# yashkant/sam-textvqa

Hardware: AMD Instinct MI355X
Metric: training samples/sec, SA-M4C c=3 synthetic batch (higher is better)
Workload: dtype bf16; 1 GPU; SA-M4C c=3 full train step (fwd + masked BCE + bwd + clip 0.25 + Adam + LR), T=20 + 100 obj + 50 OCR + 12 dec = 182 tokens, 768-d, 12 heads, MMT n,n,s,s,s,s + TextBert 3 layers + input encoders + classifier(V=5000)/pointer net, dropout 0.1 on, bf16 MFMA compute, fp32 master weights/Adam; global_batch=64, per_gpu_batch=64, seq_len=182, parallelism=dp1

## Files before the change

### include/sam_hip.h

```cpp
#ifndef SAM_HIP_H
#define SAM_HIP_H
#include <stdint.h>
#ifdef __cplusplus
extern "C" {
#endif

#define SAM_ERR_ARG (-1)
#define SAM_ERR_UNSUPPORTED (-2)

int sam_abi_version(void);
const char* sam_build_digest(void);
const char* sam_last_error(void);
int sam_device_info(int* cu_count, int* lds_per_cu_bytes, char* arch, int arch_len);
int sam_set_cu_reserve(int n);
int sam_get_cu_reserve(void);
int sam_debug_cu_hog(int blocks, double microseconds, void* stream);

int sam_attn_words_per_row(int N);
int sam_pack_masks_u8(const int64_t* question_mask, int T, const int64_t* obj_mask, int No, const int64_t* ocr_mask, int Nc, int B, uint8_t* key_valid,
                      uint8_t* q8, uint8_t* ocr8, void* stream);
int sam_mask_bits_prefix_lm(const uint8_t* key_valid, int B, int n_enc, int n_dec, int NW, uint32_t* out, void* stream);
int sam_mask_bits_from_additive(const float* mask, int B, int N, int NW, uint32_t* out, void* stream);
int sam_mask_bits_spatial(const uint32_t* base, const int8_t* adj, int B, int N, int NW, int T, int n_oo, int R, int H,
                          unsigned quadrant_bits, uint32_t* out, void* stream);

int sam_mask_bits_from_int8_bhnn(const int8_t* rel, const uint32_t* base, int B, int H, int N, int NW, uint32_t* out, void* stream);

int sam_spatial_relation_tensor(const double* boxes, int B, int N, int context, double distance_threshold, int8_t* out, void* stream);

int sam_attn_fwd(const void* qkv, const uint32_t* allow, int64_t allow_stride_b, int64_t allow_stride_h, int B, int N, int H,
                 int head_dim, float scale, float p_drop, uint64_t seed, uint64_t offset, void* out, float* lse2,
                 uint32_t* keep, void* stream);
int sam_attn_fwd_rows(const void* qkv, const uint32_t* allow, int64_t allow_stride_b, int64_t allow_stride_h, int B, int N, int H,
                      int head_dim, float scale, int q_begin, void* out, float* lse2, void* stream);
int sam_attn_fwd_dec(const void* qkv_enc, const void* qkv_dec, const uint32_t* allow, int64_t allow_stride_b, int64_t allow_stride_h, int B, int N, int n_dec,
                     int H, int head_dim, float scale, void* out_dec, void* stream);
int sam_attn_fwd_dec_shared(const void* qkv_enc, const void* qkv_dec, const uint32_t* allow, int64_t allow_stride_b, int64_t allow_stride_h, int B, int group,
                            int N, int n_dec, int H, int head_dim, float scale, void* out_dec, void* stream);
int sam_attn_dec_row(const void* qkv_enc, const void* qkv_dec, const uint32_t* allow, int64_t allow_stride_b, int64_t allow_stride_h, int B, int group, int N,
                     int n_dec, int t, int H, int head_dim, float scale, void* out, int64_t ldo, void* stream);
int sam_attn_fwd_train(const void* qkv, const uint32_t* allow, int64_t allow_stride_b, int64_t allow_stride_h, int B, int N, int H,
                       int head_dim, float scale, float p_drop, uint64_t seed, uint64_t offset, void* out, void* out_lo, float* lse2,
                       uint32_t* keep, void* stream);
int sam_attn_bwd_fused(const void* dout, const void* qkv, const void* out, const void* out_lo, const float* lse2, const uint32_t* allow,
                       int64_t allow_stride_b, int64_t allow_stride_h, const uint32_t* keep, int B, int N, int H, int head_dim,
                       float scale, float p_drop, void* dqkv, void* stream);
int sam_attn_bwd_fused_max_n(void);
int sam_attn_bwd(const void* dout, const void* qkv, const float* lse2, const uint32_t* allow, int64_t allow_stride_b,
                 int64_t allow_stride_h, const uint32_t* keep, int B, int N, int H, int head_dim, float scale, float p_drop,
                 void* dqkv, float* delta_ws, void* stream);

enum { SAM_EPI_NONE = 0, SAM_EPI_BIAS = 1, SAM_EPI_BIAS_GELU = 2, SAM_EPI_BIAS_DROPOUT_RES = 3, SAM_EPI_DGELU = 4, SAM_EPI_BIAS_GELU_GRAD = 5, SAM_EPI_MUL_AUX = 6,
       SAM_EPI_BIAS_RELU = 7 };
typedef struct sam_ln_fuse {
  const float* gamma; const float* beta; float eps;
  void* y; int64_t ldy;
  float* mean; float* rstd;
  int32_t done;
  float* xws; int64_t xws_bytes;
} sam_ln_fuse;
int64_t sam_gemm_ln_ws_bytes(int M, int N);
typedef struct sam_gemm_desc {
  int32_t M, N, K;
  int32_t a_kcontig, b_kcontig;
  int32_t c_is_f32, accumulate, epilogue;
  const void* A; int64_t lda;
  const void* B; int64_t ldb;
  void* C; int64_t ldc;
  const float* bias;
  const void* residual; int64_t ldr;
  void* aux_out; const void* aux_in; int64_t ld_aux;
  float p_drop; uint64_t seed, offset;
  int32_t split_k;
  float* bias_grad;
  float* ws; int64_t ws_bytes;
  int32_t force_tile;
  int32_t defer_reduce;
  int32_t split_k_used;
  sam_ln_fuse* ln;
} sam_gemm_desc;
int sam_gemm_bf16(const sam_gemm_desc* d, void* stream);
int sam_gemm_bf16_grouped(const sam_gemm_desc* descs, int count, void* stream);
int64_t sam_gemm_grouped_ws_bytes(const sam_gemm_desc* descs, int count);
int sam_gemm_splitk_reduce(const float* ws, int split_k, int M, int N, float* C, int64_t ldc, float* bias_grad, void* stream);

int sam_layernorm_fwd(const void* x, int x_is_f32, int64_t ldx, const float* gamma, const float* beta, float eps, int M, int D, void* y,
                      int64_t ldy, float* mean, float* rstd, void* stream);
int64_t sam_layernorm_bwd_ws_bytes(int D);
int sam_layernorm_bwd(const void* dy, int64_t ldd, const void* x, int x_is_f32, int64_t ldx, const float* mean, const float* rstd,
                      const float* gamma, int M, int D, void* dx, void* dx_dropped, int64_t ldo, float p_drop, uint64_t seed, uint64_t offset,
                      float* dgamma, float* dbeta, float* dbias, int accumulate, float* ws, void* stream);
typedef struct sam_ln_finalize_item {
  const float* ws; int32_t rows; int32_t accumulate;
  float* dgamma; float* dbeta; float* dbias;
} sam_ln_finalize_item;
int sam_layernorm_bwd_partial_rows(int M);
int sam_layernorm_bwd_finalize_batch(const sam_ln_finalize_item* items, int count, int D, void* stream);
int64_t sam_colsum_ws_bytes(int N);
int sam_colsum_bf16(const void* x, int64_t ldx, int M, int N, float* out, int accumulate, float* ws, void* stream);
int sam_add_dropout_bf16(const void* a, int64_t lda, const void* b, int64_t ldb, void* out, int64_t ldo, int M, int D, float p_drop, uint64_t seed,
                         uint64_t offset, void* stream);

int sam_bce_loss(const float* fixed_scores, int64_t ld_fixed, const float* ocr_scores, int64_t ld_ocr, const float* targets, int64_t ld_t,
                 const float* loss_mask, int R, int V, int No, float grad_scale, const float* global_count, float* loss, void* d_fixed,
                 int64_t ld_dfixed, float* d_ocr, int64_t ld_docr, void* stream);

int sam_ptr_scores_fwd(const void* q, const void* k, const uint8_t* ocr_mask, int B, int S, int No, int D, float scale, float* out,
                       int64_t ld_out_b, int64_t ld_out_s, void* stream);
int sam_ptr_scores_bwd(const float* dscores, int64_t ld_b, int64_t ld_s, const void* q, const void* k, int B, int S, int No, int D, float scale,
                       void* dq, void* dk, void* stream);

int sam_embedding_bwd(const void* dy, int64_t ldd, const int64_t* idx, int T, int D, int rows, int64_t padding_idx, float* grad, int64_t ldg, uint8_t* touched,
                      void* stream);
int sam_embedding_bwd_sorted(const void* dy, int64_t ldd, const int64_t* idx_sorted, int T, int D, int rows, int64_t padding_idx, float* grad, int64_t ldg,
                             uint8_t* touched, void* stream);

int sam_l2norm_pack_bf16(const float* x, int64_t ldx, int M, int D, int normalize, float eps, void* out, int64_t ldo, int col0, int zero_upto,
                         void* stream);
int sam_embed_sum_fwd(const void* table, int64_t ld_table, const int64_t* ids, int table_rows, const float* pos, int64_t ld_pos, int S,
                      const float* tt, int64_t ld_tt, const uint8_t* type_ids, int n_types, int R, int D, float* out, int64_t ldo, void* stream);
int64_t sam_embed_sum_bwd_ws_bytes(int S, int n_types, int D);
int sam_embed_sum_bwd(const void* d, int64_t ldd, int R, int D, int S, const uint8_t* type_ids, int n_types, float* d_pos, int64_t ld_pos,
                      float* d_tt, int64_t ld_tt, float* ws, void* stream);
int sam_gather2_add_fwd(const void* ans, int64_t ld_ans, int V, const void* ocr, int64_t ld_ocr, int n_ocr, const int64_t* inds, int B, int S, int D,
                        const void* emb, int64_t ld_emb, float p_drop, uint64_t seed, uint64_t offset, void* out, int64_t ldo, void* stream);
int sam_gather2_add_bwd(const void* dy, int64_t ldd, int V, int n_ocr, const int64_t* inds, int B, int S, int D, float* d_ans, int64_t ld_dans,
                        float* d_ocr, int64_t ld_docr, float p_drop, uint64_t seed, uint64_t offset, void* d_emb, int64_t ld_demb, void* stream);

int sam_input_encoder_fwd(const void* za, int64_t ldza, const float* bbox, int64_t ldbox, const void* wb, int64_t ldw, const float* bias_b,
                          const float* gamma_a, const float* beta_a, const float* gamma_b, const float* beta_b, float eps, int R, int D, float p_drop,
                          uint64_t seed, uint64_t offset, void* out, int64_t ldo, float* stats, void* stream);
int64_t sam_input_encoder_bwd_ws_bytes(int R, int D);
int sam_input_encoder_bwd(const void* dy, int64_t ldd, const void* za, int64_t ldza, const float* bbox, int64_t ldbox, const void* wb, int64_t ldw,
                          const float* bias_b, const float* gamma_a, const float* gamma_b, const float* stats, int R, int D, float p_drop, uint64_t seed,
                          uint64_t offset, void* dza, int64_t ldo, float* dgamma_a, float* dbeta_a, float* dgamma_b, float* dbeta_b, float* dbias_b, float* dwb,
                          int64_t ldgw, int accumulate, float* ws, void* stream);

typedef struct sam_sparse_rows { int64_t lo, hi; int32_t row_len; const uint8_t* touched; } sam_sparse_rows;
int64_t sam_sumsq_ws_bytes(void);
int sam_sumsq_f32(const float* g, int64_t n, const sam_sparse_rows* sparse, float* out, float* ws, void* stream);
int sam_adam_step(float* p, float* g, float* m, float* v, void* p_bf16, int64_t n, const int64_t* seg_end, const float* seg_lr, int nseg,
                  float beta1, float beta2, float eps, int64_t step, const float* gnorm_sq, float max_norm, const sam_sparse_rows* sparse, void* stream);
int sam_adam_step_dev(float* p, float* g, float* m, float* v, void* p_bf16, int64_t n, const int64_t* seg_end, int nseg, float beta1, float beta2,
                      float eps, const float* dev_sched, const float* gnorm_sq, float max_norm, const sam_sparse_rows* sparse, void* stream);
int sam_adam_step_range(float* p, float* g, float* m, float* v, void* p_bf16, int64_t n, const int64_t* seg_end, int nseg, float beta1, float beta2,
                        float eps, const float* dev_sched, const float* gnorm_sq, float max_norm, const sam_sparse_rows* sparse, int64_t lo, int64_t hi,
                        int zero_grad, const int32_t* gate, int max_blocks, void* stream);
typedef struct sam_lr_schedule {
  double base_lr[8]; int32_t nseg;
  int64_t warmup_iters; double warmup_factor;
  int32_t n_decay; int64_t decay_iters[4]; double lr_decay;
  double beta1, beta2;
} sam_lr_schedule;
int sam_step_advance(unsigned long long* rng_state, uint64_t offset_stride, int64_t* step_counter, const sam_lr_schedule* sched, float* dev_sched,
                     void* stream);
int sam_cast_f32_to_bf16(const float* x, void* y, int64_t n, void* stream);

int sam_greedy_pick(const float* fixed_scores, int64_t ld_fixed, const float* ocr_scores, int64_t ld_ocr, int R, int S, int V, int No, int64_t* prev_inds,
                    void* stream);
int sam_beam_step(const float* fixed_scores, int64_t ld_fixed, const float* ocr_scores, int64_t ld_ocr, int B, int K, int S, int V, int No, int eos, int t,
                  int32_t* ctl, float* cum, uint8_t* done, int64_t* seqs, int64_t* prev_pos, void* stream);
int64_t sam_beam_step_ws_bytes(int B, int K);
// ... 68 lines not shown
```

### sam-textvqa_amd/_capi.py

```python
import ctypes as C
import os

_PKG = os.path.dirname(os.path.abspath(__file__))
LIB_PATH = os.path.join(_PKG, "lib", "libsam_hip.so")

_vp, _i, _i64, _u64, _f, _u = C.c_void_p, C.c_int, C.c_int64, C.c_uint64, C.c_float, C.c_uint

class LnFuse(C.Structure):
    _fields_ = [("gamma", _vp), ("beta", _vp), ("eps", _f), ("y", _vp), ("ldy", _i64), ("mean", _vp), ("rstd", _vp), ("done", C.c_int32),
                ("xws", _vp), ("xws_bytes", _i64)]


class GemmDesc(C.Structure):
    _fields_ = [("M", C.c_int32), ("N", C.c_int32), ("K", C.c_int32),
                ("a_kcontig", C.c_int32), ("b_kcontig", C.c_int32),
                ("c_is_f32", C.c_int32), ("accumulate", C.c_int32), ("epilogue", C.c_int32),
                ("A", _vp), ("lda", _i64), ("B", _vp), ("ldb", _i64), ("C", _vp), ("ldc", _i64),
                ("bias", _vp), ("residual", _vp), ("ldr", _i64),
                ("aux_out", _vp), ("aux_in", _vp), ("ld_aux", _i64),
                ("p_drop", _f), ("seed", _u64), ("offset", _u64), ("split_k", C.c_int32), ("bias_grad", _vp), ("ws", _vp), ("ws_bytes", _i64), ("force_tile", C.c_int32),
                ("defer_reduce", C.c_int32), ("split_k_used", C.c_int32), ("ln", C.POINTER(LnFuse))]


EPI_NONE, EPI_BIAS, EPI_BIAS_GELU, EPI_BIAS_DROPOUT_RES, EPI_DGELU, EPI_BIAS_GELU_GRAD, EPI_MUL_AUX, EPI_BIAS_RELU = range(8)
AUX_MUL, AUX_ADD = 0, 1

SIGNATURES = {
    "sam_attn_fwd": [_vp, _vp, _i64, _i64, _i, _i, _i, _i, _f, _f, _u64, _u64, _vp, _vp, _vp, _vp],
    "sam_attn_fwd_rows": [_vp, _vp, _i64, _i64, _i, _i, _i, _i, _f, _i, _vp, _vp, _vp],
    "sam_attn_bwd": [_vp, _vp, _vp, _vp, _i64, _i64, _vp, _i, _i, _i, _i, _f, _f, _vp, _vp, _vp],
    "sam_attn_words_per_row": [_i],
    "sam_attn_fwd_train": [_vp, _vp, _i64, _i64, _i, _i, _i, _i, _f, _f, _u64, _u64, _vp, _vp, _vp, _vp, _vp],
    "sam_attn_bwd_fused": [_vp, _vp, _vp, _vp, _vp, _vp, _i64, _i64, _vp, _i, _i, _i, _i, _f, _f, _vp, _vp],
    "sam_attn_bwd_fused_max_n": [],
    "sam_mask_bits_prefix_lm": [_vp, _i, _i, _i, _i, _vp, _vp],
    "sam_mask_bits_from_additive": [_vp, _i, _i, _i, _vp, _vp],
    "sam_mask_bits_spatial": [_vp, _vp, _i, _i, _i, _i, _i, _i, _i, _u, _vp, _vp],
    "sam_abi_version": [],
    "sam_mask_bits_from_int8_bhnn": [_vp, _vp, _i, _i, _i, _i, _vp, _vp],
    "sam_spatial_relation_tensor": [_vp, _i, _i, _i, C.c_double, _vp, _vp],
    "sam_gemm_bf16": [C.POINTER(GemmDesc), _vp],
    "sam_gemm_splitk_reduce": [_vp, _i, _i, _i, _vp, _i64, _vp, _vp],
    "sam_gemm_bf16_grouped": [C.POINTER(GemmDesc), _i, _vp],
    "sam_gemm_grouped_ws_bytes": [C.POINTER(GemmDesc), _i],
    "sam_layernorm_fwd": [_vp, _i, _i64, _vp, _vp, _f, _i, _i, _vp, _i64, _vp, _vp, _vp],
    "sam_layernorm_bwd": [_vp, _i64, _vp, _i, _i64, _vp, _vp, _vp, _i, _i, _vp, _vp, _i64, _f, _u64, _u64, _vp, _vp, _vp, _i, _vp, _vp],
    "sam_layernorm_bwd_ws_bytes": [_i],
    "sam_layernorm_bwd_partial_rows": [_i],
    "sam_layernorm_bwd_finalize_batch": [C.c_void_p, _i, _i, _vp],
    "sam_colsum_ws_bytes": [_i],
    "sam_colsum_bf16": [_vp, _i64, _i, _i, _vp, _i, _vp, _vp],
    "sam_bce_loss": [_vp, _i64, _vp, _i64, _vp, _i64, _vp, _i, _i, _i, _f, _vp, _vp, _vp, _i64, _vp, _i64, _vp],
    "sam_ptr_scores_fwd": [_vp, _vp, _vp, _i, _i, _i, _i, _f, _vp, _i64, _i64, _vp],
    "sam_ptr_scores_bwd": [_vp, _i64, _i64, _vp, _vp, _i, _i, _i, _i, _f, _vp, _vp, _vp],
    "sam_embedding_bwd": [_vp, _i64, _vp, _i, _i, _i, _i64, _vp, _i64, _vp, _vp],
    "sam_embedding_bwd_sorted": [_vp, _i64, _vp, _i, _i, _i, _i64, _vp, _i64, _vp, _vp],
    "sam_l2norm_pack_bf16": [_vp, _i64, _i, _i, _i, _f, _vp, _i64, _i, _i, _vp],
    "sam_embed_sum_fwd": [_vp, _i64, _vp, _i, _vp, _i64, _i, _vp, _i64, _vp, _i, _i, _i, _vp, _i64, _vp],
    "sam_embed_sum_bwd_ws_bytes": [_i, _i, _i],
    "sam_embed_sum_bwd": [_vp, _i64, _i, _i, _i, _vp, _i, _vp, _i64, _vp, _i64, _vp, _vp],
    "sam_gather2_add_fwd": [_vp, _i64, _i, _vp, _i64, _i, _vp, _i, _i, _i, _vp, _i64, _f, _u64, _u64, _vp, _i64, _vp],
    "sam_gather2_add_bwd": [_vp, _i64, _i, _i, _vp, _i, _i, _i, _vp, _i64, _vp, _i64, _f, _u64, _u64, _vp, _i64, _vp],
    "sam_sumsq_ws_bytes": [],
    "sam_sumsq_f32": [_vp, _i64, C.c_void_p, _vp, _vp, _vp],
    "sam_adam_step": [_vp, _vp, _vp, _vp, _vp, _i64, C.POINTER(_i64), C.POINTER(_f), _i, _f, _f, _f, _i64, _vp, _f, C.c_void_p, _vp],
    "sam_adam_step_dev": [_vp, _vp, _vp, _vp, _vp, _i64, C.POINTER(_i64), _i, _f, _f, _f, _vp, _vp, _f, C.c_void_p, _vp],
    "sam_adam_step_range": [_vp, _vp, _vp, _vp, _vp, _i64, C.POINTER(_i64), _i, _f, _f, _f, _vp, _vp, _f, C.c_void_p, _i64, _i64, _i, _vp, _i, _vp],
    "sam_cast_f32_to_bf16": [_vp, _vp, _i64, _vp],
    "sam_pack_masks_u8": [_vp, _i, _vp, _i, _vp, _i, _i, _vp, _vp, _vp, _vp],
    "sam_add_dropout_bf16": [_vp, _i64, _vp, _i64, _vp, _i64, _i, _i, _f, _u64, _u64, _vp],
    "sam_set_rng_state": [_vp],
    "sam_step_advance": [_vp, _u64, _vp, C.c_void_p, _vp, _vp],
    "sam_input_encoder_fwd": [_vp, _i64, _vp, _i64, _vp, _i64, _vp, _vp, _vp, _vp, _vp, _f, _i, _i, _f, _u64, _u64, _vp, _i64, _vp, _vp],
    "sam_input_encoder_bwd_ws_bytes": [_i, _i],
    "sam_input_encoder_bwd": [_vp, _i64, _vp, _i64, _vp, _i64, _vp, _i64, _vp, _vp, _vp, _vp, _i, _i, _f, _u64, _u64, _vp, _i64, _vp, _vp, _vp, _vp, _vp, _vp, _i64, _i, _vp, _vp],
    "sam_attn_fwd_dec": [_vp, _vp, _vp, _i64, _i64, _i, _i, _i, _i, _i, _f, _vp, _vp],
    "sam_attn_fwd_dec_shared": [_vp, _vp, _vp, _i64, _i64, _i, _i, _i, _i, _i, _i, _f, _vp, _vp],
    "sam_attn_dec_row": [_vp, _vp, _vp, _i64, _i64, _i, _i, _i, _i, _i, _i, _i, _f, _vp, _i64, _vp],
    "sam_greedy_pick": [_vp, _i64, _vp, _i64, _i, _i, _i, _i, _vp, _vp],
    "sam_beam_step": [_vp, _i64, _vp, _i64, _i, _i, _i, _i, _i, _i, _i, _vp, _vp, _vp, _vp, _vp, _vp],
    "sam_beam_step_split": [_vp, _i64, _vp, _i64, _i, _i, _i, _i, _i, _i, _i, _vp, _vp, _vp, _vp, _vp, _vp, _vp],
    "sam_beam_step_ws_bytes": [_i, _i],
    "sam_greedy_decode_ws_bytes": [_i, _i, _i],
    "sam_copy_blocks": [C.c_void_p, _i, _vp],
    "sam_ge_u8": [_vp, _i64, _i64, _vp, _vp],
    "sam_greedy_decode_steps": [C.c_void_p, _vp, _i64, _vp],
    "sam_gemm_ln_ws_bytes": [_i, _i],
    "sam_attn_probs": [_vp, _vp, _i64, _i64, _vp, _vp, _vp, _i, _i, _i, _i, _f, _f, _vp, _vp],
    "sam_rowvec_bf16": [_i, _vp, _i64, _vp, _i64, _vp, _vp, _i64, _i64, _i, _vp],
    "sam_set_cu_reserve": [_i],
    "sam_get_cu_reserve": [],
    "sam_debug_cu_hog": [_i, C.c_double, _vp],
    "sam_aux_pair_fwd": [_vp, _vp, _vp, _vp, _i, _i, _i, _vp, _vp],
    "sam_aux_pair_bwd_ws_bytes": [_i, _i],
    "sam_aux_pair_bwd": [_vp, _vp, _vp, _vp, _i, _i, _i, _vp, _vp, _vp, _vp, _i, _vp, _i64, _vp],
    "sam_l2norm_pack_from_bf16": [_vp, _i64, _i, _i, _i, _f, _vp, _i64, _i, _i, _vp],
    "sam_fc7_bwd_rows": [_vp, _i64, _vp, _i64, _i, _i, _i, _f, _vp, _i64, _vp],
    "sam_answer_sample": [_vp, _vp, _vp, _vp, _vp, _vp, _vp, _vp, _i, _i, _i, _i, _i, _i, _i, _u64, _vp, _i64, _vp, _vp, _i64, _vp, _vp, _vp, _vp, _vp],
    "sam_bce_loss_table": [_vp, _i64, _vp, _i64, _vp, _vp, _vp, _vp, _vp, _vp, _vp, _vp, _i, _i, _i, _i, _i, _vp, _vp, _i, _i, _i, _f, _vp, _vp, _vp, _i64, _vp, _i64,
                           _vp, _vp],
}
NO_STATUS = {"sam_set_rng_state", "sam_get_cu_reserve", "sam_gemm_ln_ws_bytes", "sam_layernorm_bwd_partial_rows", "sam_gemm_grouped_ws_bytes", "sam_attn_words_per_row", "sam_attn_bwd_fused_max_n", "sam_abi_version", "sam_layernorm_bwd_ws_bytes", "sam_colsum_ws_bytes", "sam_sumsq_ws_bytes", "sam_embed_sum_bwd_ws_bytes", "sam_input_encoder_bwd_ws_bytes", "sam_greedy_decode_ws_bytes", "sam_beam_step_ws_bytes", "sam_aux_pair_bwd_ws_bytes"}
RET_I64 = {"sam_gemm_grouped_ws_bytes", "sam_gemm_ln_ws_bytes", "sam_layernorm_bwd_ws_bytes", "sam_colsum_ws_bytes", "sam_sumsq_ws_bytes", "sam_embed_sum_bwd_ws_bytes", "sam_input_encoder_bwd_ws_bytes", "sam_greedy_decode_ws_bytes", "sam_beam_step_ws_bytes", "sam_aux_pair_bwd_ws_bytes"}

# ... 109 lines not shown
```

### sam-textvqa_amd/autograd.py

```python
import math
import os

import torch
from torch.autograd import Function

from . import _capi as capi
from . import ops, parallel, torchops
from .params import FlatParams, flat_of

BF16 = torch.bfloat16


class DropoutClock:

    def __init__(self):
        self.seed = 0x5A4D3443
        self.offset = 0

    def manual_seed(self, seed):
        self.seed, self.offset = int(seed) & 0xFFFFFFFFFFFFFFFF, 0

    def next(self):
        self.offset += 1
        return self.seed, self.offset
# ... 543 lines not shown
                pass
        cls.late = []


def defer_mmt_pairs_active():
    return os.environ.get("SAM_DEFER_MMT_WGRAD", "2") not in ("0", "1")


def wgrad_late_enabled():
    return os.environ.get("SAM_WGRAD_LATE", "1") != "0"


def wgrad_merge_enabled():
    return os.environ.get("SAM_WGRAD_MERGE_TB", "1") != "0"


def defer_wgrad_enabled():
    return os.environ.get("SAM_DEFER_TB_WGRAD", "1") != "0"


class EncoderLayerFn(Function):

    @staticmethod
    def forward(ctx, x, anchor, layer, allow, batch, p_attn, p_hid):
        att, so, inter, out = layer.attention.self, layer.attention.output, layer.intermediate, layer.output
        wqkv, bqkv, _, _ = _fused_qkv(att)
        heads = att.num_attention_heads
        scale = 1.0 / math.sqrt(att.attention_head_size)
        seeds = [dropout_clock.next() for _ in range(3)]
        ctx.layer, ctx.batch, ctx.p_attn, ctx.p_hid, ctx.seeds, ctx.scale = layer, batch, p_attn, p_hid, seeds, scale
        if coarse_ops_active() and x.dtype == BF16 and x.dim() == 2 and x.stride(1) == 1:
            outs = torchops.ns().encoder_layer_fwd(x, allow, _layer_params(layer), batch, heads, scale, p_attn, p_hid, [v for sd in seeds for v in sd],
                                                   so.LayerNorm.variance_epsilon, out.LayerNorm.variance_epsilon)
            ctx.save_for_backward(*outs[1:], allow)
            ctx.coarse = True
            return outs[0]
        ctx.coarse = False
        qkv = ops.gemm(x, wqkv, epilogue=capi.EPI_BIAS, bias=bqkv)
        fused_bwd = x.shape[0] // batch <= ops.attn_bwd_fused_max_n() and os.environ.get("SAM_ATTN_BWD_FUSED", "1") != "0"
        if fused_bwd:
            ctxv, lse2, keep, ctx_lo = ops.attn_fwd(qkv, allow, batch, heads, scale, p_attn, *seeds[0], want_residual=True)
        else:
            (ctxv, lse2, keep), ctx_lo = ops.attn_fwd(qkv, allow, batch, heads, scale, p_attn, *seeds[0]), None
        z1, a, mean1, rstd1 = ops.gemm_ln(ctxv, _w(so.dense.weight), so.LayerNorm.weight, so.LayerNorm.bias, so.LayerNorm.variance_epsilon,
                                          epilogue=capi.EPI_BIAS_DROPOUT_RES, bias=so.dense.bias, residual=x, p_drop=p_hid, seed=seeds[1][0], offset=seeds[1][1])
        pre = torch.empty((x.shape[0], inter.dense.weight.shape[0]), dtype=BF16, device=x.device)
        h = ops.gemm(a, _w(inter.dense.weight), epilogue=capi.EPI_BIAS_GELU_GRAD, bias=inter.dense.bias, aux_out=pre)
        z2, y, mean2, rstd2 = ops.gemm_ln(h, _w(out.dense.weight), out.LayerNorm.weight, out.LayerNorm.bias, out.LayerNorm.variance_epsilon,
                                          epilogue=capi.EPI_BIAS_DROPOUT_RES, bias=out.dense.bias, residual=a, p_drop=p_hid, seed=seeds[2][0], offset=seeds[2][1])
        ctx.save_for_backward(x, qkv, ctxv, lse2, keep, z1, mean1, rstd1, a, pre, h, z2, mean2, rstd2, allow, ctx_lo)
        return y

    @staticmethod
    def backward(ctx, dy):
        layer, p_hid, seeds = ctx.layer, ctx.p_hid, ctx.seeds
        att, so, inter, out = layer.attention.self, layer.attention.output, layer.intermediate, layer.output
        acc = not getattr(layer, "_sam_grad_fresh", False)
        layer._sam_grad_fresh = False
        defer = bool(getattr(layer, "_sam_defer_wgrad", False)) and defer_wgrad_enabled()
        if ctx.coarse:
            *saved, allow = ctx.saved_tensors
            if defer:
                dx, dy2, dpre, dy1, dqkv = torchops.ns().encoder_layer_bwd_nowgrad(dy, saved, allow, _layer_params(layer), _layer_grads(layer), ctx.batch,
                                                                                   att.num_attention_heads, ctx.scale, ctx.p_attn, p_hid,
                                                                                   [v for sd in seeds for v in sd], bool(ctx.needs_input_grad[0]), acc)
                _, _, dwqkv, dbqkv = _fused_qkv(att)
                x_, ctx_, a_, h_ = saved[0], saved[2], saved[8], saved[10]
                DeferredWgrads.add(layer, [(dy2, h_, out.dense.weight.grad, None), (dpre, a_, inter.dense.weight.grad, inter.dense.bias.grad),
                                           (dy1, ctx_, so.dense.weight.grad, None), (dqkv, x_, dwqkv, dbqkv)], acc)
            else:
                dx = torchops.ns().encoder_layer_bwd(dy, saved, allow, _layer_params(layer), _layer_grads(layer), ctx.batch, att.num_attention_heads, ctx.scale,
                                                     ctx.p_attn, p_hid, [v for sd in seeds for v in sd], bool(ctx.needs_input_grad[0]), acc)
                region_done(getattr(layer, "_sam_region_id", None))
            return (dx if ctx.needs_input_grad[0] else None), None, None, None, None, None, None
        x, qkv, ctxv, lse2, keep, z1, mean1, rstd1, a, pre, h, z2, mean2, rstd2, allow, ctx_lo = ctx.saved_tensors
        wqkv, _, dwqkv, dbqkv = _fused_qkv(att)
        if dy.dtype != BF16 or not dy.is_contiguous():
            dy = dy.to(BF16).contiguous()
        dz2, dy2 = ops.layernorm_bwd(dy, z2, mean2, rstd2, out.LayerNorm.weight, out.LayerNorm.weight.grad, out.LayerNorm.bias.grad,
                                     dbias=out.dense.bias.grad, want_dropped=True, p_drop=p_hid, seed=seeds[2][0], offset=seeds[2][1], accumulate=acc, may_defer=True)
        wgrads = [(dy2, h, out.dense.weight.grad, None)]
        dpre = ops.gemm(dy2, _w(out.dense.weight), b_kcontig=False, epilogue=capi.EPI_MUL_AUX, aux_in=pre)
        wgrads.append((dpre, a, inter.dense.weight.grad, inter.dense.bias.grad))
        da = ops.gemm(dpre, _w(inter.dense.weight), b_kcontig=False, epilogue=capi.EPI_BIAS_DROPOUT_RES, residual=dz2)
        dz1, dy1 = ops.layernorm_bwd(da, z1, mean1, rstd1, so.LayerNorm.weight, so.LayerNorm.weight.grad, so.LayerNorm.bias.grad,
                                     dbias=so.dense.bias.grad, want_dropped=True, p_drop=p_hid, seed=seeds[1][0], offset=seeds[1][1], accumulate=acc, may_defer=True)
        wgrads.append((dy1, ctxv, so.dense.weight.grad, None))
        dctx = ops.gemm(dy1, _w(so.dense.weight), b_kcontig=False)
        dqkv = ops.attn_bwd(dctx, qkv, lse2, allow, keep, ctx.batch, att.num_attention_heads, ctx.scale, ctx.p_attn, out=ctxv, out_lo=ctx_lo)
        wgrads.append((dqkv, x, dwqkv, dbqkv))
        if defer:
            DeferredWgrads.add(layer, wgrads, acc)
        else:
            ops.wgrad_grouped(wgrads, accumulate=acc)
        dx = ops.gemm(dqkv, wqkv, b_kcontig=False, epilogue=capi.EPI_BIAS_DROPOUT_RES, residual=dz1) if ctx.needs_input_grad[0] else None
        if not defer:
            region_done(getattr(layer, "_sam_region_id", None))
        return dx, None, None, None, None, None, None


def _rows_bf16(t):
    x2 = t.reshape(-1, t.shape[-1])
    if x2.dtype != BF16 or x2.stride(1) != 1 or x2.stride(0) % 8 or x2.data_ptr() % 16:
        x2 = x2.to(BF16).contiguous()
    return x2


class DenseDropoutResLnFn(Function):

    @staticmethod
    def forward(ctx, x, residual, mod, p_drop):
        dense, ln = mod.dense, mod.LayerNorm
        n, k = dense.weight.shape
        if n % 8 or k % 8:
            raise capi.SamHipError("%s: hidden sizes must be multiples of 8 (got %d -> %d)" % (type(mod).__name__, k, n))
        x2, r2 = _rows_bf16(x), _rows_bf16(residual)
        seed = dropout_clock.next()
        z, y, mean, rstd = ops.gemm_ln(x2, _w(dense.weight), ln.weight, ln.bias, ln.variance_epsilon, epilogue=capi.EPI_BIAS_DROPOUT_RES, bias=dense.bias,
                                       residual=r2, p_drop=p_drop, seed=seed[0], offset=seed[1])
        ctx.save_for_backward(x2, z, mean, rstd)
        ctx.mod, ctx.p_drop, ctx.seed, ctx.shapes = mod, p_drop, seed, (x.shape, x.dtype, residual.shape, residual.dtype)
        return y.view(*residual.shape[:-1], n)

    @staticmethod
    def backward(ctx, dy):
        x2, z, mean, rstd = ctx.saved_tensors
        dense, ln = ctx.mod.dense, ctx.mod.LayerNorm
        xs, xd, rs, rd = ctx.shapes
        dy2 = _rows_bf16(dy)
        dz, dyd = ops.layernorm_bwd(dy2, z, mean, rstd, ln.weight, ln.weight.grad, ln.bias.grad, dbias=dense.bias.grad, want_dropped=True, p_drop=ctx.p_drop,
                                    seed=ctx.seed[0], offset=ctx.seed[1], accumulate=True)
        ops.gemm(dyd, x2, a_kcontig=False, b_kcontig=False, out=dense.weight.grad, accumulate=True, split_k=-1)
        dx = ops.gemm(dyd, _w(dense.weight), b_kcontig=False).view(xs).to(xd) if ctx.needs_input_grad[0] else None
        return dx, (dz.view(rs).to(rd) if ctx.needs_input_grad[1] else None), None, None


class DenseGeluFn(Function):

    @staticmethod
    def forward(ctx, x, mod, want_grad):
        dense = mod.dense
        n, k = dense.weight.shape
        if n % 8 or k % 8:
            raise capi.SamHipError("BertIntermediate: sizes must be multiples of 8 (got %d -> %d)" % (k, n))
        x2 = _rows_bf16(x)
        dact = torch.empty((x2.shape[0], n), dtype=BF16, device=x2.device) if want_grad else None
        h = ops.gemm(x2, _w(dense.weight), epilogue=capi.EPI_BIAS_GELU_GRAD, bias=dense.bias, aux_out=dact)
        if want_grad:
            ctx.save_for_backward(x2, dact)
        ctx.mod, ctx.shape, ctx.dtype = mod, x.shape, x.dtype
        return h.view(*x.shape[:-1], n)

    @staticmethod
    def backward(ctx, dy):
        x2, dact = ctx.saved_tensors
        dense = ctx.mod.dense
        dpre = ops.rowvec("mul", _rows_bf16(dy), dact)
        ops.gemm(dpre, x2, a_kcontig=False, b_kcontig=False, out=dense.weight.grad, accumulate=True, split_k=-1, bias_grad=dense.bias.grad)
        dx = ops.gemm(dpre, _w(dense.weight), b_kcontig=False).view(ctx.shape).to(ctx.dtype) if ctx.needs_input_grad[0] else None
        return dx, None, None


def coarse_ops_active():
    return torchops.enabled() and capi.profiler is None


def _layer_params(layer):
    c = getattr(layer, "_sam_coarse_params", None)
    if c is None:
# ... 185 lines not shown
```

### sam-textvqa_amd/csrc/common.h

```cpp
#pragma once
#include <hip/hip_runtime.h>
#include <stdint.h>

typedef unsigned short bf16_t;
typedef __attribute__((ext_vector_type(8))) short bf16x8;
typedef __attribute__((ext_vector_type(4))) short s16x4;
typedef __attribute__((ext_vector_type(4))) float f32x4;
typedef __attribute__((ext_vector_type(2))) __bf16 hw_bf16x2;
typedef __attribute__((ext_vector_type(2))) float f32x2;

#define SAM_OK 0
#define SAM_ERR_ARG (-1)
#define SAM_ERR_UNSUPPORTED (-2)

extern "C" void sam_set_error(const char* fmt, ...);
extern "C" const unsigned long long* sam_get_rng_state(void);

#define SAM_REQUIRE(cond, ...)                    \
  do {                                            \
    if (!(cond)) {                                \
      sam_set_error(__VA_ARGS__);                 \
      return SAM_ERR_ARG;                         \
    }                                             \
  } while (0)

#define SAM_LAUNCH_CHECK()                                                       \
  do {                                                                           \
    hipError_t e_ = hipGetLastError();                                           \
    if (e_ != hipSuccess) {                                                      \
      sam_set_error("%s:%d launch failed: %s", __FILE__, __LINE__, hipGetErrorString(e_)); \
      return (int)e_;                                                            \
    }                                                                            \
  } while (0)

__device__ __forceinline__ float bf2f(bf16_t h) { return __uint_as_float(((unsigned)h) << 16); }
__device__ __forceinline__ unsigned pack_bf16x2(float lo, float hi) {
  f32x2 f = {lo, hi};
  return __builtin_bit_cast(unsigned, __builtin_convertvector(f, hw_bf16x2));
}
__device__ __forceinline__ bf16_t f2bf(float f) { return (bf16_t)(pack_bf16x2(f, 0.f) & 0xffffu); }
__device__ __forceinline__ float bf_lo(unsigned u) { return __uint_as_float(u << 16); }
__device__ __forceinline__ float bf_hi(unsigned u) { return __uint_as_float(u & 0xffff0000u); }

__device__ __forceinline__ s16x4 lds_read_tr16(const void* p) {
  return __builtin_amdgcn_ds_read_tr16_b64_v4i16((__attribute__((address_space(3))) s16x4*)p);
}
__device__ __forceinline__ bf16x8 cat4(s16x4 a, s16x4 b) {
  bf16x8 r;
  r[0] = a[0]; r[1] = a[1]; r[2] = a[2]; r[3] = a[3];
  r[4] = b[0]; r[5] = b[1]; r[6] = b[2]; r[7] = b[3];
  return r;
}

__device__ __forceinline__ float xgroup_max(float v) {
  auto a = __builtin_amdgcn_permlane16_swap(__float_as_uint(v), __float_as_uint(v), false, false);
  v = fmaxf(__uint_as_float(a[0]), __uint_as_float(a[1]));
  auto b = __builtin_amdgcn_permlane32_swap(__float_as_uint(v), __float_as_uint(v), false, false);
  return fmaxf(__uint_as_float(b[0]), __uint_as_float(b[1]));
}
__device__ __forceinline__ float xgroup_sum(float v) {
  auto a = __builtin_amdgcn_permlane16_swap(__float_as_uint(v), __float_as_uint(v), false, false);
  v = __uint_as_float(a[0]) + __uint_as_float(a[1]);
  auto b = __builtin_amdgcn_permlane32_swap(__float_as_uint(v), __float_as_uint(v), false, false);
  return __uint_as_float(b[0]) + __uint_as_float(b[1]);
}
__device__ __forceinline__ unsigned xgroup_or(unsigned v) {
  auto a = __builtin_amdgcn_permlane16_swap(v, v, false, false);
  v = a[0] | a[1];
  auto b = __builtin_amdgcn_permlane32_swap(v, v, false, false);
  return b[0] | b[1];
}
__device__ __forceinline__ float wave_sum_v(float v) {
  auto h = __builtin_amdgcn_permlane32_swap(__float_as_uint(v), __float_as_uint(v), false, false);
  v = __uint_as_float(h[0]) + __uint_as_float(h[1]);
  auto r = __builtin_amdgcn_permlane16_swap(__float_as_uint(v), __float_as_uint(v), false, false);
  v = __uint_as_float(r[0]) + __uint_as_float(r[1]);
  v += __int_as_float(__builtin_amdgcn_update_dpp(0, __float_as_int(v), 0x128, 0xf, 0xf, false));
  int t = __builtin_amdgcn_update_dpp(0, __float_as_int(v), 0x104, 0xf, 0x5, false);
  t = __builtin_amdgcn_update_dpp(t, __float_as_int(v), 0x114, 0xf, 0xa, false);
  v += __int_as_float(t);
  v += __int_as_float(__builtin_amdgcn_update_dpp(0, __float_as_int(v), 0x4E, 0xf, 0xf, false));
  v += __int_as_float(__builtin_amdgcn_update_dpp(0, __float_as_int(v), 0xB1, 0xf, 0xf, false));
  return v;
}

__device__ __forceinline__ void rng_resolve(const unsigned long long* st, unsigned& seed_lo, unsigned& seed_hi, unsigned& off_lo, unsigned& off_hi) {
  if (st) {
    const unsigned long long s = st[0], o = st[1] + (((unsigned long long)off_hi << 32) | off_lo);
    if (s) { seed_lo = (unsigned)s; seed_hi = (unsigned)(s >> 32); }
    off_lo = (unsigned)o; off_hi = (unsigned)(o >> 32);
  }
}

struct u32x4 { unsigned x, y, z, w; };
__device__ __forceinline__ unsigned mix32(unsigned x) {
  x ^= x >> 16; x *= 0x7feb352du; x ^= x >> 15; x *= 0x846ca68bu; x ^= x >> 16;
  return x;
}
__device__ __forceinline__ unsigned dropout_row_key(unsigned row, unsigned off_lo, unsigned off_hi, unsigned seed_lo, unsigned seed_hi) {
// ... 72 lines not shown
```

### sam-textvqa_amd/csrc/gemm.hip

```cpp
#include "gemm_common.h"
#include <stdlib.h>

using namespace samgemm;
namespace {

__device__ __forceinline__ int kc_off(int row, int chunk) { return row * 128 + ((chunk ^ ((row >> 1) & 7)) << 4); }
__device__ __forceinline__ int ks_swz(int krow) { return ((krow & 3) | (((krow >> 3) & 1) << 2)) << 1; }
template <int C>
__device__ __forceinline__ int ks_off(int krow, int chunk) { return krow * (2 * C) + ((chunk ^ (ks_swz(krow) & (C / 8 - 1))) << 4); }

template <bool KC, int R, int NT>
__device__ __forceinline__ void load_tile(uint4 (&r)[R * 8 / NT], const bf16_t* base, int64_t ld, int row0, int rows, int k0, int K, int tid) {
#pragma unroll
  for (int j = 0; j < R * 8 / NT; ++j) {
    const int c = tid + NT * j;
    r[j] = make_uint4(0, 0, 0, 0);
    if (KC) {
      const int row = row0 + (c >> 3), k = k0 + (c & 7) * 8;
      if (row < rows && k < K) r[j] = *reinterpret_cast<const uint4*>(base + (int64_t)row * ld + k);
    } else {
      const int k = k0 + c / (R / 8), col = row0 + (c % (R / 8)) * 8;
      if (k < K && col < rows) r[j] = *reinterpret_cast<const uint4*>(base + (int64_t)k * ld + col);
    }
  }
// ... 471 lines not shown
  g.count = count;
  int total = 0;
  static int bm_env = -1;
  if (bm_env < 0) { const char* e = getenv("SAM_WGRAD_TILE_M"); bm_env = e ? atoi(e) : 0; }
  const int bm = bm_env == 256 ? 256 : 128;
  for (int q = 0; q < count; ++q) {
    const sam_gemm_desc* d = descs + q;
    SAM_REQUIRE(!d->a_kcontig && !d->b_kcontig && d->c_is_f32 && d->epilogue == SAM_EPI_NONE && (d->split_k == 0 || d->split_k == 1),
                "sam_gemm_bf16_grouped: problem %d is not a plain fp32 wgrad-layout GEMM", q);
    SAM_REQUIRE(d->M > 0 && d->N > 0 && d->K > 0 && d->A && d->B && d->C, "sam_gemm_bf16_grouped: problem %d is empty", q);
    SAM_REQUIRE(d->M % 8 == 0 && d->N % 8 == 0 && d->lda % 8 == 0 && d->ldb % 8 == 0 && d->ldc % 4 == 0, "sam_gemm_bf16_grouped: problem %d: M, N, lda, ldb must be multiples of 8", q);
    SAM_REQUIRE(((uintptr_t)d->A % 16 == 0) && ((uintptr_t)d->B % 16 == 0) && ((uintptr_t)d->C % 16 == 0), "sam_gemm_bf16_grouped: problem %d: operands must be 16-byte aligned", q);
    if (q >= SAM_MAX_GROUP) continue;
    GemmArgs& a = g.a[q];
    a.M = d->M; a.N = d->N; a.K = d->K;
    a.A = (const bf16_t*)d->A; a.lda = d->lda; a.B = (const bf16_t*)d->B; a.ldb = d->ldb; a.C = d->C; a.ldc = d->ldc;
    a.accumulate = d->accumulate ? 1 : 0;
    a.inv_keep = 1.0f;
    a.tiles_m = (d->M + bm - 1) / bm; a.tiles_n = (d->N + 127) / 128;
    { static int gm = -1; if (gm < 0) { const char* e = getenv("SAM_GEMM_GROUP_M_WGRAD"); gm = e ? atoi(e) : 0; }
      a.group_m = gm > 0 ? gm : (gm == 0 && a.tiles_n > a.tiles_m ? a.tiles_m : 1); }
    a.split_k = 1;
    a.bias_grad = d->bias_grad;
    g.start[q] = total;
    total += (a.tiles_m * a.tiles_n + 7) / 8 * 8;
  }
  if (count <= SAM_MAX_GROUP) g.start[count] = total;
  {
    static int use8 = -1;
    if (use8 < 0) { const char* e = getenv("SAM_GEMM8W"); use8 = e ? atoi(e) : 1; }
    SAM_REQUIRE(ft == 0 || ft == 128 || ft == 1256 || ft == 12448, "sam_gemm_bf16_grouped: force_tile must be 0, 128, 1256 or 12448");
    static int use12 = -1;
    if (use12 < 0) { const char* e = getenv("SAM_GEMM12W"); use12 = e ? atoi(e) : 0; }
    if ((use12 && ft == 0) || ft == 12448) {
      const int rc = gemm12w_grouped(descs, count, (hipStream_t)stream);
      if (rc == SAM_OK) return SAM_OK;
      SAM_REQUIRE(rc == SAM_ERR_UNSUPPORTED && ft != 12448, "sam_gemm_bf16_grouped: the loader-wave grouped kernel cannot run this problem set (fewer deep tiles than CUs, K %% 64, workspace)");
    }
    if ((use8 && ft == 0) || ft == 1256) {
      const int rc = gemm8w_grouped(descs, count, (hipStream_t)stream);
      if (rc == SAM_OK) return SAM_OK;
      SAM_REQUIRE(rc == SAM_ERR_UNSUPPORTED && ft != 1256, "sam_gemm_bf16_grouped: the 8-wave grouped kernel cannot run this problem set (K %% 64, workspace, tile count)");
    }
  }
  if (count > SAM_MAX_GROUP) {
    for (int q0 = 0; q0 < count; q0 += SAM_MAX_GROUP) {
      const int rc = grouped_impl(descs + q0, count - q0 < SAM_MAX_GROUP ? count - q0 : SAM_MAX_GROUP, stream, ft);
      if (rc != SAM_OK) return rc;
    }
    return SAM_OK;
  }
  static bool once = false;
  if (!once) {
    hipFuncSetAttribute(reinterpret_cast<const void*>(gemm_group_kernel<128, 128, 2, 2, false, false, SAM_EPI_NONE, float>), hipFuncAttributeMaxDynamicSharedMemorySize, 2 * (128 + 128) * BK * 2);
    hipFuncSetAttribute(reinterpret_cast<const void*>(gemm_group_kernel<256, 128, 4, 2, false, false, SAM_EPI_NONE, float>), hipFuncAttributeMaxDynamicSharedMemorySize, 2 * (256 + 128) * BK * 2);
    once = true;
  }
  if (bm == 256)
    gemm_group_kernel<256, 128, 4, 2, false, false, SAM_EPI_NONE, float><<<dim3(total), dim3(512), (size_t)2 * (256 + 128) * BK * 2, (hipStream_t)stream>>>(g);
  else
    gemm_group_kernel<128, 128, 2, 2, false, false, SAM_EPI_NONE, float><<<dim3(total), dim3(256), (size_t)2 * (128 + 128) * BK * 2, (hipStream_t)stream>>>(g);
  SAM_LAUNCH_CHECK();
  return SAM_OK;
}

extern "C" int64_t sam_gemm_grouped_ws_bytes(const sam_gemm_desc* descs, int count) {
  if (!descs || count < 1 || count > SAM_MAX_GROUP8) return 0;
  int tiles = 0;
  for (int q = 0; q < count; ++q) tiles += ((descs[q].M + 255) / 256) * ((descs[q].N + 255) / 256);
  const int64_t a = gemm8w_ws_bytes(tiles), b = gemm12w_ws_bytes(descs, count);
  return a > b ? a : b;
}

extern "C" int64_t sam_gemm_ln_ws_bytes(int M, int N) { return (M > 0 && N > 0) ? gemm_ln_ws_bytes(M, N) : 0; }

extern "C" int sam_gemm_splitk_reduce(const float* ws, int split_k, int M, int N, float* C, int64_t ldc, float* bias_grad, void* stream) {
  SAM_REQUIRE(ws && C && split_k >= 1 && M > 0 && N > 0 && N % 4 == 0 && ldc % 4 == 0, "sam_gemm_splitk_reduce: bad arguments");
  const int64_t mn4 = (int64_t)M * N / 4;
  splitk_reduce_kernel<<<dim3((unsigned)min((int64_t)2048, (mn4 + 255) / 256)), dim3(256), 0, (hipStream_t)stream>>>(ws, split_k, M, N, C, ldc, bias_grad);
  SAM_LAUNCH_CHECK();
  return SAM_OK;
}

extern "C" int sam_gemm_bf16(const sam_gemm_desc* d, void* stream) {
  SAM_REQUIRE(d, "sam_gemm_bf16: null descriptor");
  if (d->ln) d->ln->done = 0;
  SAM_REQUIRE(d->M > 0 && d->N > 0 && d->K > 0, "sam_gemm_bf16: empty problem %dx%dx%d", d->M, d->N, d->K);
  SAM_REQUIRE(d->A && d->B && d->C, "sam_gemm_bf16: null operand");
  SAM_REQUIRE(d->N % 8 == 0 && d->lda % 8 == 0 && d->ldb % 8 == 0 && d->ldc % 4 == 0, "sam_gemm_bf16: N, lda, ldb must be multiples of 8 (N=%d lda=%lld ldb=%lld)", d->N, (long long)d->lda, (long long)d->ldb);
  SAM_REQUIRE(!d->a_kcontig || d->K % 8 == 0, "sam_gemm_bf16: K must be a multiple of 8 for k-contiguous A (K=%d)", d->K);
  SAM_REQUIRE(!d->b_kcontig || d->K % 8 == 0, "sam_gemm_bf16: K must be a multiple of 8 for k-contiguous B (K=%d)", d->K);
  SAM_REQUIRE(d->a_kcontig || d->M % 8 == 0, "sam_gemm_bf16: M must be a multiple of 8 for k-strided A (M=%d)", d->M);
  SAM_REQUIRE(((uintptr_t)d->A % 16 == 0) && ((uintptr_t)d->B % 16 == 0) && ((uintptr_t)d->C % 16 == 0), "sam_gemm_bf16: operands must be 16-byte aligned");
  SAM_REQUIRE(!d->accumulate || d->c_is_f32, "sam_gemm_bf16: accumulate needs an fp32 C");
  SAM_REQUIRE(d->p_drop >= 0.f && d->p_drop < 1.f, "sam_gemm_bf16: p_drop out of range");
  GemmArgs a = {};
  a.M = d->M; a.N = d->N; a.K = d->K;
  a.A = (const bf16_t*)d->A; a.lda = d->lda; a.B = (const bf16_t*)d->B; a.ldb = d->ldb; a.C = d->C; a.ldc = d->ldc;
  a.bias = d->bias; a.residual = (const bf16_t*)d->residual; a.ldr = d->ldr;
  a.aux_out = (bf16_t*)d->aux_out; a.aux_in = (const bf16_t*)d->aux_in; a.ld_aux = d->ld_aux;
  a.accumulate = d->accumulate;
  a.thr16 = dropout_thr16(d->p_drop);
  a.inv_keep = a.thr16 ? 1.0f / (1.0f - (float)a.thr16 / 65536.0f) : 1.0f;
  a.seed_lo = (unsigned)d->seed; a.seed_hi = (unsigned)(d->seed >> 32); a.off_lo = (unsigned)d->offset; a.off_hi = (unsigned)(d->offset >> 32);
  a.rng_state = sam_get_rng_state();
  a.split_k = 1;
  { static int gm = -1; if (gm < 0) { const char* e = getenv("SAM_GEMM_GROUP_M"); gm = e ? atoi(e) : 0; } a.group_m = gm > 0 ? gm : (d->split_k != 0 && d->split_k != 1 ? 1 : 8); }
  a.bias_grad = d->bias_grad;
  a.ws = d->ws;
  a.defer_reduce = d->defer_reduce;
  a.split_used = const_cast<int32_t*>(&d->split_k_used);
  SAM_REQUIRE(!d->bias_grad || (!d->a_kcontig && !d->b_kcontig), "sam_gemm_bf16: bias_grad is a wgrad-layout (0,0) feature");
  if (d->epilogue == SAM_EPI_BIAS_GELU) SAM_REQUIRE(d->aux_out && d->ld_aux % 4 == 0, "sam_gemm_bf16: BIAS_GELU needs aux_out");
  if (d->epilogue == SAM_EPI_BIAS_GELU_GRAD) SAM_REQUIRE(!d->aux_out || d->ld_aux % 4 == 0, "sam_gemm_bf16: BIAS_GELU_GRAD: ld_aux must be a multiple of 4");

  if (d->epilogue == SAM_EPI_DGELU || d->epilogue == SAM_EPI_MUL_AUX) SAM_REQUIRE(d->aux_in && d->ld_aux % 4 == 0, "sam_gemm_bf16: DGELU / MUL_AUX need aux_in");
  if (d->epilogue == SAM_EPI_BIAS_DROPOUT_RES) SAM_REQUIRE(!d->residual || d->ldr % 4 == 0, "sam_gemm_bf16: bad residual ld");
  int want_split = (d->split_k == 1) ? 0 : d->split_k;
  hipStream_t st = (hipStream_t)stream;
  if (want_split != 0 && !(d->c_is_f32 && d->epilogue == SAM_EPI_NONE && d->accumulate)) {
    SAM_REQUIRE(!d->accumulate && !d->bias_grad, "sam_gemm_bf16: split_k with an epilogue cannot accumulate / reduce a bias gradient");
    SAM_REQUIRE(d->ws && ((uintptr_t)d->ws % 16 == 0), "sam_gemm_bf16: split_k needs a 16-byte aligned workspace");
    int S = want_split < 0 ? pick_epilogue_split(d->M, d->N, d->K, d->ws_bytes) : want_split;
    if (S > (d->K + BK - 1) / BK) S = (d->K + BK - 1) / BK;
    S = no_empty_split((d->K + BK - 1) / BK, S);
    SAM_REQUIRE((int64_t)S * d->M * d->N * (int64_t)sizeof(float) <= d->ws_bytes || S <= 1, "sam_gemm_bf16: workspace too small for split_k=%d", S);
    if (S > 1) {
      GemmArgs g = a;
      g.bias = nullptr; g.residual = nullptr; g.aux_out = nullptr; g.aux_in = nullptr; g.thr16 = 0; g.accumulate = 0;
      g.tiles_m = (d->M + 63) / 64; g.tiles_n = (d->N + 63) / 64; g.split_k = S; g.group_m = 1; g.defer_reduce = 1; g.bias_grad = nullptr;
      const int lay2 = (d->a_kcontig ? 2 : 0) | (d->b_kcontig ? 1 : 0);
      int rc = lay2 == 3 ? launch_cfg<64, 64, 2, 2, true, true, SAM_EPI_NONE, float>(g, st)
             : lay2 == 2 ? launch_cfg<64, 64, 2, 2, true, false, SAM_EPI_NONE, float>(g, st)
             : lay2 == 0 ? launch_cfg<64, 64, 2, 2, false, false, SAM_EPI_NONE, float>(g, st) : SAM_ERR_UNSUPPORTED;
      if (rc) { if (rc == SAM_ERR_UNSUPPORTED) sam_set_error("sam_gemm_bf16: no split kernel for layout (0,1)"); return rc; }
      const int e2 = d->epilogue;
      if (d->ln && e2 == SAM_EPI_BIAS_DROPOUT_RES && !d->c_is_f32 && d->N % 4 == 0 && d->N <= 2048) {
        const sam_ln_fuse* l = d->ln;
        SAM_REQUIRE(l->gamma && l->beta && l->y && l->mean && l->rstd && l->ldy >= d->N, "sam_gemm_bf16: incomplete sam_ln_fuse");
        LnFuseArgs la = {l->gamma, l->beta, l->eps, (bf16_t*)l->y, l->ldy, l->mean, l->rstd};
        const dim3 lgrid((unsigned)((d->M + 3) / 4));
        switch ((d->N / 4 + 63) / 64) {
#define SAM_LN_CASE(NC) case NC: splitk_epilogue_ln_kernel<NC><<<lgrid, dim3(256), 0, st>>>(d->ws, S, a, la); break;
          SAM_LN_CASE(1) SAM_LN_CASE(2) SAM_LN_CASE(3) SAM_LN_CASE(4) SAM_LN_CASE(5) SAM_LN_CASE(6) SAM_LN_CASE(7) SAM_LN_CASE(8)
#undef SAM_LN_CASE
        }
        SAM_LAUNCH_CHECK();
        d->ln->done = 1;
        *const_cast<int32_t*>(&d->split_k_used) = S;
        return SAM_OK;
      }
      const int64_t mn4 = (int64_t)d->M * d->N / 4;
      const dim3 grid((unsigned)min((int64_t)2048, (mn4 + 255) / 256));
#define SAM_SPLIT_EPI(E, T) splitk_epilogue_kernel<E, T><<<grid, dim3(256), 0, st>>>(d->ws, S, a)
      if (d->c_is_f32) {
        if (e2 == SAM_EPI_NONE) SAM_SPLIT_EPI(SAM_EPI_NONE, float);
        else if (e2 == SAM_EPI_BIAS) SAM_SPLIT_EPI(SAM_EPI_BIAS, float);
        else { sam_set_error("sam_gemm_bf16: fp32 output supports epilogues NONE / BIAS only"); return SAM_ERR_UNSUPPORTED; }
      } else {
        if (e2 == SAM_EPI_NONE) SAM_SPLIT_EPI(SAM_EPI_NONE, bf16_t);
        else if (e2 == SAM_EPI_BIAS) SAM_SPLIT_EPI(SAM_EPI_BIAS, bf16_t);
        else if (e2 == SAM_EPI_BIAS_GELU) SAM_SPLIT_EPI(SAM_EPI_BIAS_GELU, bf16_t);
        else if (e2 == SAM_EPI_DGELU) SAM_SPLIT_EPI(SAM_EPI_DGELU, bf16_t);
        else if (e2 == SAM_EPI_BIAS_GELU_GRAD) SAM_SPLIT_EPI(SAM_EPI_BIAS_GELU_GRAD, bf16_t);
        else if (e2 == SAM_EPI_MUL_AUX) SAM_SPLIT_EPI(SAM_EPI_MUL_AUX, bf16_t);
        else if (e2 == SAM_EPI_BIAS_DROPOUT_RES) SAM_SPLIT_EPI(SAM_EPI_BIAS_DROPOUT_RES, bf16_t);
        else if (e2 == SAM_EPI_BIAS_RELU) SAM_SPLIT_EPI(SAM_EPI_BIAS_RELU, bf16_t);
        else { sam_set_error("sam_gemm_bf16: unknown epilogue %d", e2); return SAM_ERR_UNSUPPORTED; }
      }
#undef SAM_SPLIT_EPI
      SAM_LAUNCH_CHECK();
      *const_cast<int32_t*>(&d->split_k_used) = S;
      return SAM_OK;
    }
    want_split = 0;
    *const_cast<int32_t*>(&d->split_k_used) = 1;
  }
  if (want_split != 0) {
    SAM_REQUIRE(d->c_is_f32 && d->epilogue == SAM_EPI_NONE && d->accumulate, "sam_gemm_bf16: split_k needs an fp32 C with accumulate=1 and no epilogue");
    SAM_REQUIRE(d->ws && ((uintptr_t)d->ws % 16 == 0), "sam_gemm_bf16: split_k needs a 16-byte aligned workspace");
    const int64_t per_split = ((int64_t)d->M * d->N + d->M) * (int64_t)sizeof(float);
    SAM_REQUIRE(want_split < 0 || (int64_t)want_split * per_split <= d->ws_bytes || want_split > (d->K + BK - 1) / BK,
                "sam_gemm_bf16: workspace too small for split_k=%d (%lld bytes)", d->split_k, (long long)d->ws_bytes);
  }
  if (d->ln && d->ln->xws && want_split == 0 && d->epilogue == SAM_EPI_BIAS_DROPOUT_RES && !d->c_is_f32 && d->a_kcontig && d->N % 16 == 0 &&
      d->ln->xws_bytes >= gemm_ln_ws_bytes(d->M, d->N) && ((uintptr_t)d->ln->xws % 16) == 0) {
    const char* e = getenv("SAM_GEMM_LN_FUSE");
    const int lnx = e ? atoi(e) : 0;
    const sam_ln_fuse* l = d->ln;
    if (lnx) {
      SAM_REQUIRE(l->gamma && l->beta && l->y && l->mean && l->rstd && l->ldy >= d->N && l->ldy % 4 == 0, "sam_gemm_bf16: incomplete sam_ln_fuse");
      a.ln_gamma = l->gamma; a.ln_beta = l->beta; a.ln_eps = l->eps; a.ln_y = (bf16_t*)l->y; a.ln_ldy = l->ldy; a.ln_mean = l->mean; a.ln_rstd = l->rstd;
      a.ln_ws = l->xws; a.ln_done = const_cast<int32_t*>(&l->done);
    }
  }
  const int64_t wsb = d->ws_bytes;
  const int ft = d->force_tile;
  SAM_REQUIRE(ft == 0 || ft == 64 || ft == 128 || ft == 160 || ft == 192 || ft == 256 || ft == 1192 || ft == 1256 || ft == 1448 || ft == 3192 || ft == 1128 || ft == 12192 || ft == 12448, "sam_gemm_bf16: force_tile must be 0, 64, 128, 160, 192, 256, 1128, 1192, 1256, 1448, 3192, 12192 or 12448");
  const int lay = (d->a_kcontig ? 2 : 0) | (d->b_kcontig ? 1 : 0);
  const int e = d->epilogue;
  if (lay == 3) {
    if (d->c_is_f32) {
      if (e == SAM_EPI_NONE) return launch<true, true, SAM_EPI_NONE, float>(a, st, want_split, wsb, ft);
      if (e == SAM_EPI_BIAS) return launch<true, true, SAM_EPI_BIAS, float>(a, st, want_split, wsb, ft);
    } else {
      if (e == SAM_EPI_NONE) return launch<true, true, SAM_EPI_NONE, bf16_t>(a, st, want_split, wsb, ft);
      if (e == SAM_EPI_BIAS) return launch<true, true, SAM_EPI_BIAS, bf16_t>(a, st, want_split, wsb, ft);
      if (e == SAM_EPI_BIAS_GELU) return launch<true, true, SAM_EPI_BIAS_GELU, bf16_t>(a, st, want_split, wsb, ft);
      if (e == SAM_EPI_BIAS_GELU_GRAD) return launch<true, true, SAM_EPI_BIAS_GELU_GRAD, bf16_t>(a, st, want_split, wsb, ft);
      if (e == SAM_EPI_BIAS_DROPOUT_RES) return launch<true, true, SAM_EPI_BIAS_DROPOUT_RES, bf16_t>(a, st, want_split, wsb, ft);
      if (e == SAM_EPI_BIAS_RELU) return launch<true, true, SAM_EPI_BIAS_RELU, bf16_t>(a, st, want_split, wsb, ft);
    }
  } else if (lay == 2) {
    if (!d->c_is_f32) {
      if (e == SAM_EPI_NONE) return launch<true, false, SAM_EPI_NONE, bf16_t>(a, st, want_split, wsb, ft);
      if (e == SAM_EPI_DGELU) return launch<true, false, SAM_EPI_DGELU, bf16_t>(a, st, want_split, wsb, ft);
      if (e == SAM_EPI_MUL_AUX) return launch<true, false, SAM_EPI_MUL_AUX, bf16_t>(a, st, want_split, wsb, ft);
      if (e == SAM_EPI_BIAS_DROPOUT_RES) return launch<true, false, SAM_EPI_BIAS_DROPOUT_RES, bf16_t>(a, st, want_split, wsb, ft);
    } else if (e == SAM_EPI_NONE) return launch<true, false, SAM_EPI_NONE, float>(a, st, want_split, wsb, ft);
  } else if (lay == 0) {
    if (d->c_is_f32 && e == SAM_EPI_NONE) return launch<false, false, SAM_EPI_NONE, float>(a, st, want_split, wsb, ft);
    if (!d->c_is_f32 && e == SAM_EPI_NONE) return launch<false, false, SAM_EPI_NONE, bf16_t>(a, st, want_split, wsb, ft);
  }
  sam_set_error("sam_gemm_bf16: no kernel for layout (a_kcontig=%d,b_kcontig=%d) epilogue=%d c_is_f32=%d", d->a_kcontig, d->b_kcontig, e, d->c_is_f32);
  return SAM_ERR_UNSUPPORTED;
}
```

### sam-textvqa_amd/csrc/rowops.hip

```cpp
#include "common.h"
#include <stdlib.h>
#include "sam_hip.h"

namespace {

constexpr int LN_PARTIAL_BLOCKS = 512;


template <typename T> struct Ld4;
template <> struct Ld4<bf16_t> {
  static __device__ __forceinline__ void ld(const void* p, int64_t idx, float* v) {
    const uint2 x = *reinterpret_cast<const uint2*>(reinterpret_cast<const bf16_t*>(p) + idx);
    v[0] = bf_lo(x.x); v[1] = bf_hi(x.x); v[2] = bf_lo(x.y); v[3] = bf_hi(x.y);
  }
};
template <> struct Ld4<float> {
  static __device__ __forceinline__ void ld(const void* p, int64_t idx, float* v) {
    const float4 x = *reinterpret_cast<const float4*>(reinterpret_cast<const float*>(p) + idx);
    v[0] = x.x; v[1] = x.y; v[2] = x.z; v[3] = x.w;
  }
};
__device__ __forceinline__ void st4_bf16(void* p, int64_t idx, const float* v) {
  *reinterpret_cast<uint2*>(reinterpret_cast<bf16_t*>(p) + idx) = make_uint2(pack_bf16x2(v[0], v[1]), pack_bf16x2(v[2], v[3]));
}

constexpr int LN_FWD_ROWS = 1;
template <typename InT, int NCH>
__global__ __launch_bounds__(256) void ln_fwd_kernel(const void* x, int64_t ldx, const float* gamma, const float* beta, float eps, int M, int D,
                                                     void* y, int64_t ldy, float* mean_out, float* rstd_out) {
  const int lane = threadIdx.x & 63, row0 = (blockIdx.x * 4 + (threadIdx.x >> 6)) * LN_FWD_ROWS;
  if (row0 >= M) return;
  const int nchunk = D >> 2;
  float v[LN_FWD_ROWS][NCH][4];
#pragma unroll
  for (int i = 0; i < LN_FWD_ROWS; ++i) {
    const int row = min(row0 + i, M - 1);
#pragma unroll
    for (int j = 0; j < NCH; ++j) Ld4<InT>::ld(x, (int64_t)row * ldx + 4 * min(lane + 64 * j, nchunk - 1), v[i][j]);
  }
  float g4[NCH][4], b4[NCH][4];
#pragma unroll
  for (int j = 0; j < NCH; ++j) {
    const int c = min(lane + 64 * j, nchunk - 1);
    Ld4<float>::ld(gamma, 4 * c, g4[j]);
    Ld4<float>::ld(beta, 4 * c, b4[j]);
  }
#pragma unroll
  for (int i = 0; i < LN_FWD_ROWS; ++i) {
    const int row = row0 + i;
    float s = 0.f;
#pragma unroll
    for (int j = 0; j < NCH; ++j) {
      if (lane + 64 * j >= nchunk) v[i][j][0] = v[i][j][1] = v[i][j][2] = v[i][j][3] = 0.f;
      s += (v[i][j][0] + v[i][j][1]) + (v[i][j][2] + v[i][j][3]);
    }
    const float mean = wave_sum_v(s) / D;
    float q = 0.f;
#pragma unroll
    for (int j = 0; j < NCH; ++j)
      if (lane + 64 * j < nchunk)
#pragma unroll
        for (int e = 0; e < 4; ++e) { const float d = v[i][j][e] - mean; q += d * d; }
    const float rstd = 1.0f / sqrtf(wave_sum_v(q) / D + eps);
    if (row >= M) continue;
#pragma unroll
    for (int j = 0; j < NCH; ++j) {
      const int c = lane + 64 * j;
      if (c < nchunk) {
        float o[4];
#pragma unroll
        for (int e = 0; e < 4; ++e) o[e] = g4[j][e] * ((v[i][j][e] - mean) * rstd) + b4[j][e];
        st4_bf16(y, (int64_t)row * ldy + 4 * c, o);
      }
    }
    if (lane == 0) { mean_out[row] = mean; rstd_out[row] = rstd; }
  }
}

template <typename T> struct Raw4;
template <> struct Raw4<bf16_t> {
  typedef uint2 R;
  static __device__ __forceinline__ R ld(const void* p, int64_t idx) { return *reinterpret_cast<const uint2*>(reinterpret_cast<const bf16_t*>(p) + idx); }
  static __device__ __forceinline__ void expand(const R& x, float* v) { v[0] = bf_lo(x.x); v[1] = bf_hi(x.x); v[2] = bf_lo(x.y); v[3] = bf_hi(x.y); }
};
template <> struct Raw4<float> {
  typedef float4 R;
  static __device__ __forceinline__ R ld(const void* p, int64_t idx) { return *reinterpret_cast<const float4*>(reinterpret_cast<const float*>(p) + idx); }
  static __device__ __forceinline__ void expand(const R& x, float* v) { v[0] = x.x; v[1] = x.y; v[2] = x.z; v[3] = x.w; }
};

__device__ __forceinline__ void pin(unsigned& v) { asm volatile("" : "+v"(v)); }
__device__ __forceinline__ void pin(float& v) { asm volatile("" : "+v"(v)); }
__device__ __forceinline__ void pin(uint2& v) { pin(v.x); pin(v.y); }
__device__ __forceinline__ void pin(float4& v) { pin(v.x); pin(v.y); pin(v.z); pin(v.w); }

template <typename InT, int NCH, bool FULL, int MODE>
__global__ __launch_bounds__(256) void ln_bwd_kernel(const bf16_t* __restrict__ dy, int64_t ldd, const void* __restrict__ x, int64_t ldx, const float* __restrict__ mean,
                                                     const float* __restrict__ rstd, const float* __restrict__ gamma, int M, int D, bf16_t* __restrict__ dx,
                                                     bf16_t* __restrict__ dxd, int64_t ldo, unsigned thr16, float inv_keep, unsigned seed_lo, unsigned seed_hi,
                                                     unsigned off_lo, unsigned off_hi, const unsigned long long* rng_state, float* __restrict__ ws) {
  if (MODE == 2) rng_resolve(rng_state, seed_lo, seed_hi, off_lo, off_hi);
  constexpr int NS = NCH <= 3 ? 3 : (NCH == 4 ? 2 : 1);
  typedef typename Raw4<InT>::R XR;
  __shared__ float red[4][64 * 4];
  const int lane = threadIdx.x & 63, wave = __builtin_amdgcn_readfirstlane(threadIdx.x >> 6);
  const int nchunk = D >> 2;
  float ag[NCH][4], ab[NCH][4], ad[NCH][4];
#pragma unroll
  for (int j = 0; j < NCH; ++j)
#pragma unroll
    for (int e = 0; e < 4; ++e) ag[j][e] = ab[j][e] = ad[j][e] = 0.f;
  float gm[NCH][4];
#pragma unroll
  for (int j = 0; j < NCH; ++j) {
    const int c = lane + 64 * j;
    Ld4<float>::ld(gamma, 4 * min(c, nchunk - 1), gm[j]);
    if (!FULL && c >= nchunk) gm[j][0] = gm[j][1] = gm[j][2] = gm[j][3] = 0.f;
  }
  __builtin_amdgcn_sched_barrier(0);
  const DropHalfConsts hk = dropout_half_consts((lane & 1) != 0);
  const int rstride = gridDim.x * 4;
  XR xr[NS][NCH];
  uint2 dr[NS][NCH];
  float mu[NS], rs[NS];
#define LN_BWD_REQUEST(S, ROW)                                                                     \
  do {                                                                                             \
    const int row_ = min((ROW), M - 1);                                                            \
    mu[S] = mean[row_]; rs[S] = rstd[row_];                                                        \
    _Pragma("unroll") for (int j = 0; j < NCH; ++j) {                                              \
      const int c_ = FULL ? lane + 64 * j : min(lane + 64 * j, nchunk - 1);                        \
      xr[S][j] = Raw4<InT>::ld(x, (int64_t)row_ * ldx + 4 * c_);                                   \
      dr[S][j] = Raw4<bf16_t>::ld(dy, (int64_t)row_ * ldd + 4 * c_);                               \
    }                                                                                              \
  } while (0)
#define LN_BWD_SLOT(S, ROW, REQ)                                                                                                     \
  {                                                                                                                                \
    const int row = (ROW);                                                                                                         \
    float xh[NCH][4], g[NCH][4];                                                                                                   \
    float t1 = 0.f, t2 = 0.f;                                                                                                      \
    asm volatile("" ::: "memory");                                                                                                 \
    _Pragma("unroll") for (int j = 0; j < NCH; ++j) { pin(xr[S][j]); pin(dr[S][j]); }      \
    _Pragma("unroll") for (int j = 0; j < NCH; ++j) {                                                                              \
      const int c = lane + 64 * j;                                                                                                 \
      float xv[4], dv[4];                                                                                                          \
      Raw4<InT>::expand(xr[S][j], xv);                                                                                             \
      Raw4<bf16_t>::expand(dr[S][j], dv);                                                                                          \
      if (!FULL && c >= nchunk) { _Pragma("unroll") for (int e = 0; e < 4; ++e) xv[e] = dv[e] = 0.f; }                             \
      _Pragma("unroll") for (int e = 0; e < 4; ++e) {                                                                              \
        xh[j][e] = (FULL || c < nchunk) ? (xv[e] - mu[S]) * rs[S] : 0.f;                                                           \
        g[j][e] = dv[e] * gm[j][e];                                                                                                \
        t1 += g[j][e];                                                                                                             \
        t2 += g[j][e] * xh[j][e];                                                                                                  \
        ag[j][e] += dv[e] * xh[j][e];                                                                                              \
        ab[j][e] += dv[e];                                                                                                         \
      }                                                                                                                            \
    }                                                                                                                              \
    const float rsv = rs[S];                                                                                                       \
    pin(t1); pin(t2);                                                                                                              \
    if (REQ) {                                     \
      asm volatile("" ::: "memory");               \
      __builtin_amdgcn_sched_barrier(0);                                                                                           \
      LN_BWD_REQUEST(S, row + NS * rstride);                                                                                       \
      __builtin_amdgcn_sched_barrier(0);                                                                                           \
      asm volatile("" ::: "memory");                                                                                               \
    }                                                                                                                              \
    const float s1 = wave_sum_v(t1) / D, s2 = wave_sum_v(t2) / D;                                                                      \
    const unsigned rkey = MODE == 2 ? hidden_dropout_row_key((unsigned)row, off_lo, off_hi, seed_lo, seed_hi) : 0u;                \
    _Pragma("unroll") for (int j = 0; j < NCH; ++j) {                                                                              \
      const int c = lane + 64 * j;                                                                                                 \
      if (!FULL && c >= nchunk) continue;                                                                                          \
      float o[4];                                                                                                                  \
      _Pragma("unroll") for (int e = 0; e < 4; ++e) o[e] = rsv * (g[j][e] - s1 - xh[j][e] * s2);                                   \
      st4_bf16(dx, (int64_t)row * ldo + 4 * c, o);                                                                                 \
      if (MODE >= 1) {                                                                                                             \
        if (MODE == 2) {  \
          unsigned lo, hi;                                                                                                         \
          dropout_bits_half(rkey, (unsigned)(c >> 1), hk, lo, hi);                                                                 \
          o[0] = (lo & 0xffffu) >= thr16 ? o[0] * inv_keep : 0.f;                                                                  \
          o[1] = (lo >> 16) >= thr16 ? o[1] * inv_keep : 0.f;                                                                      \
          o[2] = (hi & 0xffffu) >= thr16 ? o[2] * inv_keep : 0.f;                                                                  \
          o[3] = (hi >> 16) >= thr16 ? o[3] * inv_keep : 0.f;                                                                      \
        }                                                                                                                          \
        st4_bf16(dxd, (int64_t)row * ldo + 4 * c, o);                                                                              \
      }                                                                                                                            \
      _Pragma("unroll") for (int e = 0; e < 4; ++e) ad[j][e] += o[e];                                                              \
    }                                                                                                                              \
    __builtin_amdgcn_sched_barrier(0);                                                                                             \
  }
#define LN_BWD_TRIP(R0)                                                  \
  LN_BWD_SLOT(0, (R0), true)                                             \
  if constexpr (NS > 1) LN_BWD_SLOT(1, (R0) + rstride, true)             \
  if constexpr (NS > 2) LN_BWD_SLOT(2, (R0) + 2 * rstride, true)
  const int row00 = blockIdx.x * 4 + wave;
  LN_BWD_REQUEST(0, row00);
  __builtin_amdgcn_sched_barrier(0);
  if constexpr (NS > 1) { LN_BWD_REQUEST(1, row00 + rstride); __builtin_amdgcn_sched_barrier(0); }
  if constexpr (NS > 2) { LN_BWD_REQUEST(2, row00 + 2 * rstride); __builtin_amdgcn_sched_barrier(0); }
  const int full = M / (rstride * NS);
  int r0 = row00;
  if (full > 0) {
    LN_BWD_TRIP(r0)
    r0 += NS * rstride;
    for (int t = 1; t < full; ++t, r0 += NS * rstride) { LN_BWD_TRIP(r0) }
  }
  if (r0 < M) LN_BWD_SLOT(0, r0, false)
  if constexpr (NS > 1) { if (r0 + rstride < M) LN_BWD_SLOT(1, r0 + rstride, false) }
  if constexpr (NS > 2) { if (r0 + 2 * rstride < M) LN_BWD_SLOT(2, r0 + 2 * rstride, false) }
#undef LN_BWD_TRIP
#undef LN_BWD_SLOT
#undef LN_BWD_REQUEST
#pragma unroll
  for (int which = 0; which < 3; ++which) {
#pragma unroll
    for (int j = 0; j < NCH; ++j) {
      const int c = lane + 64 * j;
      __syncthreads();
#pragma unroll
      for (int e = 0; e < 4; ++e) red[wave][lane * 4 + e] = which == 0 ? ag[j][e] : (which == 1 ? ab[j][e] : ad[j][e]);
      __syncthreads();
      if (wave == 0 && c < nchunk) {
        float o[4];
#pragma unroll
        for (int e = 0; e < 4; ++e) o[e] = red[0][lane * 4 + e] + red[1][lane * 4 + e] + red[2][lane * 4 + e] + red[3][lane * 4 + e];
        *reinterpret_cast<float4*>(ws + ((int64_t)blockIdx.x * 3 + which) * D + 4 * c) = make_float4(o[0], o[1], o[2], o[3]);
      }
    }
  }
}

struct FinalizeOuts { float* out[3]; int64_t col0[3]; };
constexpr int FIN_RL = 16;
__global__ __launch_bounds__(64 * FIN_RL) void partial_finalize_kernel(const float* ws, int nrows, int64_t stride, int ncols, FinalizeOuts o, int accumulate) {
  __shared__ float red[FIN_RL][64];
  const int cx = threadIdx.x & 63, ry = threadIdx.x >> 6, c = min((int)blockIdx.x * 64 + cx, ncols - 1);
  const float* base = ws + o.col0[blockIdx.y] + c;
  float s = 0.f;
  for (int r = ry; r < nrows; r += FIN_RL * 8) {
    float t[8];
#pragma unroll
    for (int u = 0; u < 8; ++u) t[u] = base[(int64_t)min(r + FIN_RL * u, nrows - 1) * stride];
#pragma unroll
    for (int u = 0; u < 8; ++u)
      if (r + FIN_RL * u >= nrows) t[u] = 0.f;
    s += ((t[0] + t[1]) + (t[2] + t[3])) + ((t[4] + t[5]) + (t[6] + t[7]));
  }
  red[ry][cx] = s;
  __syncthreads();
  if (ry == 0 && (int)blockIdx.x * 64 + cx < ncols) {
    float tot = 0.f;
#pragma unroll
    for (int u = 0; u < FIN_RL; ++u) tot += red[u][cx];
    float* out = o.out[blockIdx.y];
    out[c] = accumulate ? out[c] + tot : tot;
  }
}

struct FinalizeBatch { const float* ws[32]; float* out[32][3]; int nrows[32]; int accumulate[32]; int D; };
__global__ __launch_bounds__(64 * FIN_RL) void partial_finalize_batch_kernel(FinalizeBatch b) {
  __shared__ float red[FIN_RL][64];
  const int z = blockIdx.z, D = b.D;
  float* out = b.out[z][blockIdx.y];
  const int cx = threadIdx.x & 63, ry = threadIdx.x >> 6, c = min((int)blockIdx.x * 64 + cx, D - 1);
  const int nrows = b.nrows[z];
  const int64_t stride = 3 * (int64_t)D;
  const float* base = b.ws[z] + (int64_t)blockIdx.y * D + c;
  float s = 0.f;
  if (out) {
    for (int r = ry; r < nrows; r += FIN_RL * 8) {
      float t[8];
// ... 293 lines not shown
  const int64_t row = idx[t];
  if (row < 0 || row >= rows || row == padding_idx) return;
  if (touched && threadIdx.x == 0) touched[row] = 1;
  for (int c = threadIdx.x; c * 4 < D; c += 256) {
    float v[4];
    Ld4<bf16_t>::ld(dy, (int64_t)t * ldd + 4 * c, v);
    float* g = grad + row * ldg + 4 * c;
#pragma unroll
    for (int e = 0; e < 4; ++e) unsafeAtomicAdd(g + e, v[e]);
  }
}

__global__ __launch_bounds__(256) void embedding_bwd_dedup_kernel(const bf16_t* dy, int64_t ldd, const int64_t* idx, int T, int D, int rows, int64_t padding_idx, float* grad, int64_t ldg,
                                                                  unsigned char* touched) {
  const int t = blockIdx.x, tid = threadIdx.x;
  const int64_t row = idx[t];
  if (row < 0 || row >= rows || row == padding_idx) return;
  int dup = 0;
  for (int s = tid; s < t; s += 256) dup |= idx[s] == row;
  if (__syncthreads_or(dup)) return;
  if (touched && tid == 0) touched[row] = 1;
  const int nch = (D / 4 + 255) / 256;
  for (int cc = 0; cc < nch; ++cc) {
    const int c = tid + 256 * cc;
    const bool live = c * 4 < D;
    float a[4] = {0.f, 0.f, 0.f, 0.f};
    if (live) Ld4<bf16_t>::ld(dy, (int64_t)t * ldd + 4 * c, a);
    for (int base = t + 1; base < T; base += 256) {
      const int s = base + tid;
      const int hit = s < T && idx[s] == row;
      if (__syncthreads_or(hit)) {
        const int end = min(base + 256, T);
        for (int k = base; k < end; ++k)
          if (idx[k] == row && live) {
            float v[4];
            Ld4<bf16_t>::ld(dy, (int64_t)k * ldd + 4 * c, v);
#pragma unroll
            for (int e = 0; e < 4; ++e) a[e] += v[e];
          }
      }
    }
    if (live) {
      float4* g = reinterpret_cast<float4*>(grad + row * ldg + 4 * c);
      const float4 o = *g;
      *g = make_float4(o.x + a[0], o.y + a[1], o.z + a[2], o.w + a[3]);
    }
  }
}

__global__ __launch_bounds__(256) void embedding_bwd_sorted_kernel(const bf16_t* dy, int64_t ldd, const int64_t* idx, int T, int D, int rows, int64_t padding_idx, float* grad, int64_t ldg,
                                                                   unsigned char* touched) {
  const int t = blockIdx.x;
  const int64_t row = idx[t];
  if (row < 0 || row >= rows || row == padding_idx || (t > 0 && idx[t - 1] == row)) return;
  if (touched && threadIdx.x == 0) touched[row] = 1;
  int end = t + 1;
  while (end < T && idx[end] == row) ++end;
  for (int c = threadIdx.x; c * 4 < D; c += 256) {
    float a[4] = {0.f, 0.f, 0.f, 0.f};
    for (int s = t; s < end; ++s) {
      float v[4];
      Ld4<bf16_t>::ld(dy, (int64_t)s * ldd + 4 * c, v);
#pragma unroll
      for (int e = 0; e < 4; ++e) a[e] += v[e];
    }
    float4* g = reinterpret_cast<float4*>(grad + row * ldg + 4 * c);
    const float4 o = *g;
    *g = make_float4(o.x + a[0], o.y + a[1], o.z + a[2], o.w + a[3]);
  }
}

template <typename InT>
int ln_fwd_dispatch(int nch, dim3 grid, hipStream_t st, const void* x, int64_t ldx, const float* gamma, const float* beta, float eps, int M, int D,
                    void* y, int64_t ldy, float* mean, float* rstd) {
#define LN_FWD_CASE(NC) case NC: ln_fwd_kernel<InT, NC><<<grid, dim3(256), 0, st>>>(x, ldx, gamma, beta, eps, M, D, y, ldy, mean, rstd); break;
  switch (nch) { LN_FWD_CASE(1) LN_FWD_CASE(2) LN_FWD_CASE(3) LN_FWD_CASE(4) LN_FWD_CASE(5) LN_FWD_CASE(6) LN_FWD_CASE(7) LN_FWD_CASE(8) default: return SAM_ERR_UNSUPPORTED; }
#undef LN_FWD_CASE
  return SAM_OK;
}
template <typename InT>
int ln_bwd_dispatch(int nch, dim3 grid, hipStream_t st, const bf16_t* dy, int64_t ldd, const void* x, int64_t ldx, const float* mean, const float* rstd,
                    const float* gamma, int M, int D, bf16_t* dx, bf16_t* dxd, int64_t ldo, unsigned thr16, float inv_keep, uint64_t seed, uint64_t offset, float* ws) {
#define LN_BWD_LAUNCH(NC, FULL_, MODE_) ln_bwd_kernel<InT, NC, FULL_, MODE_><<<grid, dim3(256), 0, st>>>(dy, ldd, x, ldx, mean, rstd, gamma, M, D, dx, dxd, ldo, thr16, inv_keep, \
      (unsigned)seed, (unsigned)(seed >> 32), (unsigned)offset, (unsigned)(offset >> 32), sam_get_rng_state(), ws)
#define LN_BWD_CASE(NC) case NC: \
    if (D == 256 * NC) { if (mode == 2) LN_BWD_LAUNCH(NC, true, 2); else if (mode == 1) LN_BWD_LAUNCH(NC, true, 1); else LN_BWD_LAUNCH(NC, true, 0); } \
    else { if (mode == 2) LN_BWD_LAUNCH(NC, false, 2); else if (mode == 1) LN_BWD_LAUNCH(NC, false, 1); else LN_BWD_LAUNCH(NC, false, 0); } \
    break;
  const int mode = dxd ? (thr16 ? 2 : 1) : 0;
  switch (nch) { LN_BWD_CASE(1) LN_BWD_CASE(2) LN_BWD_CASE(3) LN_BWD_CASE(4) LN_BWD_CASE(5) LN_BWD_CASE(6) LN_BWD_CASE(7) LN_BWD_CASE(8) default: return SAM_ERR_UNSUPPORTED; }
#undef LN_BWD_LAUNCH
#undef LN_BWD_CASE
  return SAM_OK;
}

}

extern "C" int sam_layernorm_fwd(const void* x, int x_is_f32, int64_t ldx, const float* gamma, const float* beta, float eps, int M, int D, void* y,
                                 int64_t ldy, float* mean, float* rstd, void* stream) {
  SAM_REQUIRE(x && gamma && beta && y && mean && rstd, "sam_layernorm_fwd: null pointer");
  SAM_REQUIRE(M > 0 && D > 0 && D % 4 == 0 && D <= 2048 && ldx % 4 == 0 && ldy % 4 == 0, "sam_layernorm_fwd: need D %% 4 == 0, D <= 2048 (M=%d D=%d)", M, D);
  const int nch = (D / 4 + 63) / 64;
  const dim3 grid((M + 4 * LN_FWD_ROWS - 1) / (4 * LN_FWD_ROWS));
  int rc = x_is_f32 ? ln_fwd_dispatch<float>(nch, grid, (hipStream_t)stream, x, ldx, gamma, beta, eps, M, D, y, ldy, mean, rstd)
                    : ln_fwd_dispatch<bf16_t>(nch, grid, (hipStream_t)stream, x, ldx, gamma, beta, eps, M, D, y, ldy, mean, rstd);
  if (rc) return rc;
  SAM_LAUNCH_CHECK();
  return SAM_OK;
}

extern "C" int64_t sam_layernorm_bwd_ws_bytes(int D) { return (int64_t)LN_PARTIAL_BLOCKS * 3 * D * sizeof(float); }

extern "C" int sam_layernorm_bwd(const void* dy, int64_t ldd, const void* x, int x_is_f32, int64_t ldx, const float* mean, const float* rstd,
                                 const float* gamma, int M, int D, void* dx, void* dx_dropped, int64_t ldo, float p_drop, uint64_t seed, uint64_t offset,
                                 float* dgamma, float* dbeta, float* dbias, int accumulate, float* ws, void* stream) {
  SAM_REQUIRE(dy && x && mean && rstd && gamma && dx && dgamma && dbeta && ws, "sam_layernorm_bwd: null pointer");
  SAM_REQUIRE(M > 0 && D > 0 && D % 4 == 0 && D <= 2048 && ldx % 4 == 0 && ldd % 4 == 0 && ldo % 4 == 0, "sam_layernorm_bwd: bad shape M=%d D=%d", M, D);
  SAM_REQUIRE(p_drop >= 0.f && p_drop < 1.f, "sam_layernorm_bwd: p_drop out of range");
  SAM_REQUIRE(!dbias || dx_dropped || p_drop == 0.f, "sam_layernorm_bwd: dbias with dropout needs dx_dropped");
  const unsigned thr16 = dropout_thr16(p_drop);
  const float inv_keep = thr16 ? 1.0f / (1.0f - (float)thr16 / 65536.0f) : 1.0f;
  const int nch = (D / 4 + 63) / 64;
  const int nblk = min(LN_PARTIAL_BLOCKS, (M + 3) / 4);
  hipStream_t st = (hipStream_t)stream;
  bf16_t* dxd = (bf16_t*)dx_dropped;
  int rc = x_is_f32 ? ln_bwd_dispatch<float>(nch, dim3(nblk), st, (const bf16_t*)dy, ldd, x, ldx, mean, rstd, gamma, M, D, (bf16_t*)dx, dxd, ldo, thr16, inv_keep, seed, offset, ws)
                    : ln_bwd_dispatch<bf16_t>(nch, dim3(nblk), st, (const bf16_t*)dy, ldd, x, ldx, mean, rstd, gamma, M, D, (bf16_t*)dx, dxd, ldo, thr16, inv_keep, seed, offset, ws);
  if (rc) return rc;
  SAM_LAUNCH_CHECK();
  if (accumulate & 4) return SAM_OK;
  FinalizeOuts fo = {{dgamma, dbeta, dbias}, {0, D, 2 * (int64_t)D}};
  partial_finalize_kernel<<<dim3((D + 63) / 64, dbias ? 3 : 2), dim3(64 * FIN_RL), 0, st>>>(ws, nblk, 3 * (int64_t)D, D, fo, accumulate & 1);
  SAM_LAUNCH_CHECK();
  return SAM_OK;
}

extern "C" int sam_layernorm_bwd_partial_rows(int M) { return min(LN_PARTIAL_BLOCKS, (M + 3) / 4); }

extern "C" int sam_layernorm_bwd_finalize_batch(const sam_ln_finalize_item* items, int count, int D, void* stream) {
  SAM_REQUIRE(items && count >= 1 && D > 0 && D % 4 == 0, "sam_layernorm_bwd_finalize_batch: bad arguments");
  hipStream_t st = (hipStream_t)stream;
  for (int i0 = 0; i0 < count; i0 += 32) {
    FinalizeBatch b = {};
    const int n = min(32, count - i0);
    b.D = D;
    for (int i = 0; i < n; ++i) {
      const sam_ln_finalize_item& it = items[i0 + i];
      SAM_REQUIRE(it.ws && it.dgamma && it.dbeta && it.rows >= 1 && it.rows <= LN_PARTIAL_BLOCKS, "sam_layernorm_bwd_finalize_batch: item %d is malformed", i0 + i);
      b.ws[i] = it.ws; b.out[i][0] = it.dgamma; b.out[i][1] = it.dbeta; b.out[i][2] = it.dbias; b.nrows[i] = it.rows; b.accumulate[i] = it.accumulate & 1;
    }
    partial_finalize_batch_kernel<<<dim3((D + 63) / 64, 3, n), dim3(64 * FIN_RL), 0, st>>>(b);
    SAM_LAUNCH_CHECK();
  }
  return SAM_OK;
}

extern "C" int64_t sam_colsum_ws_bytes(int N) { return (int64_t)COLSUM_CHUNKS * N * sizeof(float); }

extern "C" int sam_colsum_bf16(const void* x, int64_t ldx, int M, int N, float* out, int accumulate, float* ws, void* stream) {
  SAM_REQUIRE(x && out && ws, "sam_colsum_bf16: null pointer");
  SAM_REQUIRE(M > 0 && N > 0 && N % 4 == 0 && ldx % 4 == 0, "sam_colsum_bf16: need N %% 4 == 0 (M=%d N=%d)", M, N);
  hipStream_t st = (hipStream_t)stream;
  colsum_partial_kernel<<<dim3((N / 4 + 255) / 256, COLSUM_CHUNKS), dim3(256), 0, st>>>((const bf16_t*)x, ldx, M, N, ws);
  FinalizeOuts fo = {{out, nullptr, nullptr}, {0, 0, 0}};
  partial_finalize_kernel<<<dim3((N + 63) / 64, 1), dim3(64 * FIN_RL), 0, st>>>(ws, COLSUM_CHUNKS, N, N, fo, accumulate);
  SAM_LAUNCH_CHECK();
  return SAM_OK;
}

extern "C" int sam_bce_loss(const float* fixed_scores, int64_t ld_fixed, const float* ocr_scores, int64_t ld_ocr, const float* targets, int64_t ld_t,
                            const float* loss_mask, int R, int V, int No, float grad_scale, const float* global_count, float* loss, void* d_fixed,
                            int64_t ld_dfixed, float* d_ocr, int64_t ld_docr, void* stream) {
  SAM_REQUIRE(fixed_scores && ocr_scores && targets && loss_mask && loss && d_fixed && d_ocr, "sam_bce_loss: null pointer");
  SAM_REQUIRE(R > 0 && V > 0 && No >= 0, "sam_bce_loss: bad shape");
  hipStream_t st = (hipStream_t)stream;
  hipError_t e = hipMemsetAsync(loss, 0, sizeof(float), st);
  if (e != hipSuccess) { sam_set_error("sam_bce_loss: memset: %s", hipGetErrorString(e)); return (int)e; }
  const bool pairs = V % 2 == 0 && No % 2 == 0 && ld_fixed % 2 == 0 && ld_ocr % 2 == 0 && ld_t % 2 == 0 && ld_dfixed % 2 == 0 && ld_docr % 2 == 0 &&
                     ((uintptr_t)fixed_scores % 8 == 0) && ((uintptr_t)ocr_scores % 8 == 0) && ((uintptr_t)targets % 8 == 0) && ((uintptr_t)d_ocr % 8 == 0) &&
                     ((uintptr_t)d_fixed % 4 == 0);
  const int per = pairs ? 2 : 1;
  const int chunks = max(1, min(min(8, 1024 / R), ((V + No + per - 1) / per + 255) / 256));
  if (pairs)
    bce_kernel<2><<<dim3(R, chunks), dim3(256), 0, st>>>(fixed_scores, ld_fixed, ocr_scores, ld_ocr, targets, ld_t, loss_mask, R, V, No, grad_scale, global_count, loss,
                                                         (bf16_t*)d_fixed, ld_dfixed, d_ocr, ld_docr);
  else
    bce_kernel<1><<<dim3(R, chunks), dim3(256), 0, st>>>(fixed_scores, ld_fixed, ocr_scores, ld_ocr, targets, ld_t, loss_mask, R, V, No, grad_scale, global_count, loss,
                                                         (bf16_t*)d_fixed, ld_dfixed, d_ocr, ld_docr);
  SAM_LAUNCH_CHECK();
  return SAM_OK;
}

extern "C" int sam_ptr_scores_fwd(const void* q, const void* k, const uint8_t* ocr_mask, int B, int S, int No, int D, float scale, float* out,
                                  int64_t ld_out_b, int64_t ld_out_s, void* stream) {
  SAM_REQUIRE(q && k && ocr_mask && out, "sam_ptr_scores_fwd: null pointer");
  SAM_REQUIRE(B > 0 && S > 0 && No > 0 && D > 0 && D % 4 == 0, "sam_ptr_scores_fwd: bad shape");
  if (S <= 16 && No <= 64 && D == 768 && ((uintptr_t)q % 16) == 0 && ((uintptr_t)k % 16) == 0)
    ptr_fwd_mfma_kernel<6><<<dim3(B), dim3(256), 0, (hipStream_t)stream>>>((const bf16_t*)q, (const bf16_t*)k, ocr_mask, S, No, D, scale, out, ld_out_b, ld_out_s);
  else
    ptr_fwd_kernel<<<dim3(B, S), dim3(256), 0, (hipStream_t)stream>>>((const bf16_t*)q, (const bf16_t*)k, ocr_mask, S, No, D, scale, out, ld_out_b, ld_out_s);
  SAM_LAUNCH_CHECK();
  return SAM_OK;
}
extern "C" int sam_ptr_scores_bwd(const float* dscores, int64_t ld_b, int64_t ld_s, const void* q, const void* k, int B, int S, int No, int D, float scale,
                                  void* dq, void* dk, void* stream) {
  SAM_REQUIRE(dscores && q && k && dq && dk, "sam_ptr_scores_bwd: null pointer");
  SAM_REQUIRE(B > 0 && S > 0 && No > 0 && D > 0 && D % 4 == 0 && S <= 256 && No <= 256, "sam_ptr_scores_bwd: bad shape (S, No <= 256)");
  ptr_bwd_kernel<<<dim3(B, S + No), dim3(256), 0, (hipStream_t)stream>>>(dscores, ld_b, ld_s, (const bf16_t*)q, (const bf16_t*)k, S, No, D,
                                                                                          scale, (bf16_t*)dq, (bf16_t*)dk);
  SAM_LAUNCH_CHECK();
  return SAM_OK;
}

extern "C" int sam_embedding_bwd(const void* dy, int64_t ldd, const int64_t* idx, int T, int D, int rows, int64_t padding_idx, float* grad, int64_t ldg, uint8_t* touched,
                                void* stream) {
// ... 175 lines not shown
```

### sam-textvqa_amd/csrc_torch/sam_torch_ops.cpp

```cpp
#include <ATen/ATen.h>
#include <c10/hip/HIPStream.h>
#include <torch/library.h>

#include <tuple>
#include <string>
#include <cstdlib>
#include <map>
#include <mutex>
#include <vector>

#include "sam_hip.h"

namespace {

using at::Tensor;
using c10::optional;

void* cur_stream() { return (void*)c10::hip::getCurrentHIPStream().stream(); }

void ok(int rc, const char* what) { TORCH_CHECK(rc == 0, what, " failed (rc=", rc, "): ", sam_last_error()); }

const Tensor& need(const Tensor& t, at::ScalarType dt, const char* name) {
  TORCH_CHECK(t.defined() && t.is_cuda(), name, " must be a GPU tensor (this package has no CPU path)");
  TORCH_CHECK(t.scalar_type() == dt, name, ": expected dtype ", dt, ", got ", t.scalar_type());
  return t;
}
void need2d(const Tensor& t, const char* name) {
  need(t, at::kBFloat16, name);
  TORCH_CHECK(t.dim() == 2 && t.stride(1) == 1, name, ": need a 2-D bf16 tensor with contiguous last dim");
}
void* p(const Tensor& t) { return t.defined() ? t.data_ptr() : nullptr; }
void* p(const optional<Tensor>& t) { return t.has_value() && t->defined() ? t->data_ptr() : nullptr; }

struct GemmOpt {
  int epilogue = SAM_EPI_NONE;
  const Tensor* bias = nullptr;
  const Tensor* residual = nullptr;
  const Tensor* aux_in = nullptr;
  Tensor* aux_out = nullptr;
  float p_drop = 0.f;
  int64_t seed = 0, offset = 0;
  bool out_f32 = false;
  sam_ln_fuse* ln = nullptr;
};

Tensor gemm(const Tensor& a, const Tensor& b, bool a_kc, bool b_kc, const GemmOpt& o) {
  need2d(a, "gemm A"); need2d(b, "gemm B");
  const int64_t M = a_kc ? a.size(0) : a.size(1), K = a_kc ? a.size(1) : a.size(0), N = b_kc ? b.size(0) : b.size(1);
  Tensor out = at::empty({M, N}, a.options().dtype(o.out_f32 ? at::kFloat : at::kBFloat16));
  sam_gemm_desc d = {};
  d.M = (int32_t)M; d.N = (int32_t)N; d.K = (int32_t)K;
  d.a_kcontig = a_kc; d.b_kcontig = b_kc; d.c_is_f32 = o.out_f32; d.epilogue = o.epilogue;
  d.A = a.data_ptr(); d.lda = a.stride(0); d.B = b.data_ptr(); d.ldb = b.stride(0); d.C = out.data_ptr(); d.ldc = out.stride(0);
  d.bias = o.bias ? (const float*)o.bias->data_ptr() : nullptr;
  if (o.residual) { d.residual = o.residual->data_ptr(); d.ldr = o.residual->stride(0); }
  if (o.aux_out) { d.aux_out = o.aux_out->data_ptr(); d.ld_aux = o.aux_out->stride(0); }
  if (o.aux_in) { d.aux_in = o.aux_in->data_ptr(); d.ld_aux = o.aux_in->stride(0); }
  d.p_drop = o.p_drop; d.seed = (uint64_t)o.seed; d.offset = (uint64_t)o.offset;
  d.ln = o.ln;
  Tensor ws;
  if (M <= 4096 && K >= 1536 && M * N <= (4 << 20)) {
    d.split_k = -1;
    const int64_t bytes = std::min<int64_t>(8 * (M * N + M) * 4, (int64_t)96 << 20);
    ws = at::empty({(bytes + 3) / 4}, a.options().dtype(at::kFloat));
    d.ws = (float*)ws.data_ptr(); d.ws_bytes = ws.numel() * 4; d.defer_reduce = 1;
  }
  ok(sam_gemm_bf16(&d, cur_stream()), "sam_gemm_bf16");
  return out;
}

std::tuple<Tensor, Tensor, Tensor> ln_fwd(const Tensor& x, const Tensor& gamma, const Tensor& beta, double eps);
std::tuple<Tensor, Tensor, Tensor, Tensor> gemm_ln(const Tensor& a, const Tensor& b, const Tensor& gamma, const Tensor& beta, double eps, GemmOpt o) {
  const int64_t M = a.size(0), N = b.size(0);
  if (N % 4 || N > 2048 || gamma.scalar_type() != at::kFloat || beta.scalar_type() != at::kFloat) {
    Tensor z = gemm(a, b, true, true, o);
    auto [y, mean, rstd] = ln_fwd(z, gamma, beta, eps);
    return {z, y, mean, rstd};
  }
  Tensor y = at::empty({M, N}, a.options()), mean = at::empty({M}, a.options().dtype(at::kFloat)), rstd = at::empty({M}, a.options().dtype(at::kFloat));
  sam_ln_fuse ln = {(const float*)gamma.data_ptr(), (const float*)beta.data_ptr(), (float)eps, y.data_ptr(), y.stride(0), (float*)mean.data_ptr(), (float*)rstd.data_ptr(), 0, nullptr, 0};
  if (M >= 2048) {
    static std::map<std::pair<int, void*>, Tensor> cache;
    const int64_t bytes = sam_gemm_ln_ws_bytes((int)M, (int)N);
    Tensor& xws = cache[{(int)a.get_device(), cur_stream()}];
    if (!xws.defined() || xws.numel() * 4 < bytes) xws = at::zeros({(bytes + 3) / 4}, a.options().dtype(at::kFloat));
    ln.xws = (float*)xws.data_ptr(); ln.xws_bytes = xws.numel() * 4;
  }
  o.ln = &ln;
  Tensor z = gemm(a, b, true, true, o);
  if (ln.done) return {z, y, mean, rstd};
  auto [y2, mean2, rstd2] = ln_fwd(z, gamma, beta, eps);
  return {z, y2, mean2, rstd2};
}

struct WgradJob { const Tensor* dy; const Tensor* x; const Tensor* dw; const Tensor* db; };
void wgrad_grouped(const std::vector<WgradJob>& jobs, bool accumulate = true) {
  sam_gemm_desc d[20] = {};
  TORCH_CHECK(jobs.size() >= 1 && jobs.size() <= 20, "wgrad_grouped: 1..20 jobs");
  for (size_t q = 0; q < jobs.size(); ++q) {
    const WgradJob& j = jobs[q];
    d[q].M = (int32_t)j.dy->size(1); d[q].N = (int32_t)j.x->size(1); d[q].K = (int32_t)j.dy->size(0);
    d[q].c_is_f32 = 1; d[q].accumulate = accumulate ? 1 : 0; d[q].epilogue = SAM_EPI_NONE;
    d[q].A = j.dy->data_ptr(); d[q].lda = j.dy->stride(0); d[q].B = j.x->data_ptr(); d[q].ldb = j.x->stride(0);
    d[q].C = j.dw->data_ptr(); d[q].ldc = j.dw->stride(0);
    d[q].bias_grad = j.db ? (float*)j.db->data_ptr() : nullptr;
  }
  {
    static std::mutex mu;
    static std::map<std::pair<int, void*>, Tensor> cache;
    const int64_t bytes = sam_gemm_grouped_ws_bytes(d, (int)jobs.size());
    std::lock_guard<std::mutex> lock(mu);
    Tensor& ws = cache[{(int)jobs[0].dy->get_device(), cur_stream()}];
    if (!ws.defined() || ws.numel() * 4 < bytes) ws = at::zeros({(bytes + 3) / 4}, jobs[0].dy->options().dtype(at::kFloat));
    d[0].ws = (float*)ws.data_ptr(); d[0].ws_bytes = ws.numel() * 4;
  }
  ok(sam_gemm_bf16_grouped(d, (int)jobs.size(), cur_stream()), "sam_gemm_bf16_grouped");
}

std::tuple<Tensor, Tensor, Tensor> attn_fwd(const Tensor& qkv, const Tensor& allow, int64_t batch, int64_t heads, double scale, double p_drop, int64_t seed,
                                            int64_t offset) {
  need2d(qkv, "qkv"); need(allow, at::kInt, "allow");
  TORCH_CHECK(allow.dim() == 4 && allow.is_contiguous(), "allow must be a contiguous int32 [B, H|1, N, NW] tensor");
  const int64_t rows = qkv.size(0), d_model = qkv.size(1) / 3, n = rows / batch;
  Tensor out = at::empty({rows, d_model}, qkv.options());
  Tensor lse2 = at::empty({batch, heads, n}, qkv.options().dtype(at::kFloat));
  Tensor keep = p_drop > 0 ? at::empty({batch, heads, n, allow.size(3)}, allow.options()) : Tensor();
  ok(sam_attn_fwd(qkv.data_ptr(), (const uint32_t*)allow.data_ptr(), allow.stride(0), allow.size(1) == 1 ? 0 : allow.stride(1), (int)batch, (int)n, (int)heads,
                  (int)(d_model / heads), (float)scale, (float)p_drop, (uint64_t)seed, (uint64_t)offset, out.data_ptr(), (float*)lse2.data_ptr(),
                  (uint32_t*)p(keep), cur_stream()),
     "sam_attn_fwd");
  return {out, lse2, keep.defined() ? keep : at::empty({0}, allow.options())};
}

std::tuple<Tensor, Tensor, Tensor, Tensor> attn_fwd_train(const Tensor& qkv, const Tensor& allow, int64_t batch, int64_t heads, double scale, double p_drop, int64_t seed,
                                                          int64_t offset) {
  need2d(qkv, "qkv"); need(allow, at::kInt, "allow");
  TORCH_CHECK(allow.dim() == 4 && allow.is_contiguous(), "allow must be a contiguous int32 [B, H|1, N, NW] tensor");
  const int64_t rows = qkv.size(0), d_model = qkv.size(1) / 3, n = rows / batch;
  Tensor out = at::empty({rows, d_model}, qkv.options());
  Tensor out_lo = at::empty({rows, d_model}, qkv.options());
  Tensor lse2 = at::empty({batch, heads, n}, qkv.options().dtype(at::kFloat));
  Tensor keep = p_drop > 0 ? at::empty({batch, heads, n, allow.size(3)}, allow.options()) : Tensor();
// ... 3 lines not shown
     "sam_attn_fwd_train");
  return {out, lse2, keep.defined() ? keep : at::empty({0}, allow.options()), out_lo};
}

static bool fused_attn_bwd_enabled(int64_t n) {
  const char* s = getenv("SAM_ATTN_BWD_FUSED");
  return !(s && s[0] == '0') && n <= sam_attn_bwd_fused_max_n();
}

Tensor attn_bwd_fused(const Tensor& dout, const Tensor& qkv, const Tensor& out, const Tensor& out_lo, const Tensor& lse2, const Tensor& allow, const Tensor& keep,
                      int64_t batch, int64_t heads, double scale, double p_drop) {
  need2d(dout, "dout"); need2d(qkv, "qkv"); need2d(out, "out"); need2d(out_lo, "out_lo"); need(lse2, at::kFloat, "lse2"); need(allow, at::kInt, "allow");
  const int64_t rows = qkv.size(0), d_model = qkv.size(1) / 3, n = rows / batch;
  Tensor dqkv = at::empty_like(qkv);
  const bool has_keep = keep.defined() && keep.numel() > 0;
  ok(sam_attn_bwd_fused(dout.data_ptr(), qkv.data_ptr(), out.data_ptr(), out_lo.data_ptr(), (const float*)lse2.data_ptr(), (const uint32_t*)allow.data_ptr(),
                        allow.stride(0), allow.size(1) == 1 ? 0 : allow.stride(1), has_keep ? (const uint32_t*)keep.data_ptr() : nullptr, (int)batch, (int)n, (int)heads,
                        (int)(d_model / heads), (float)scale, (float)p_drop, dqkv.data_ptr(), cur_stream()),
     "sam_attn_bwd_fused");
  return dqkv;
}

Tensor attn_bwd(const Tensor& dout, const Tensor& qkv, const Tensor& lse2, const Tensor& allow, const Tensor& keep, int64_t batch, int64_t heads, double scale,
                double p_drop) {
  need2d(dout, "dout"); need2d(qkv, "qkv"); need(lse2, at::kFloat, "lse2"); need(allow, at::kInt, "allow");
  const int64_t rows = qkv.size(0), d_model = qkv.size(1) / 3, n = rows / batch;
  Tensor dqkv = at::empty_like(qkv);
  Tensor delta = at::empty({batch, heads, n}, lse2.options());
  const bool has_keep = keep.defined() && keep.numel() > 0;
  ok(sam_attn_bwd(dout.data_ptr(), qkv.data_ptr(), (const float*)lse2.data_ptr(), (const uint32_t*)allow.data_ptr(), allow.stride(0),
                  allow.size(1) == 1 ? 0 : allow.stride(1), has_keep ? (const uint32_t*)keep.data_ptr() : nullptr, (int)batch, (int)n, (int)heads,
                  (int)(d_model / heads), (float)scale, (float)p_drop, dqkv.data_ptr(), (float*)delta.data_ptr(), cur_stream()),
     "sam_attn_bwd");
  return dqkv;
}

std::tuple<Tensor, Tensor, Tensor> ln_fwd(const Tensor& x, const Tensor& gamma, const Tensor& beta, double eps) {
  TORCH_CHECK(x.is_cuda() && x.dim() == 2 && x.stride(1) == 1 && (x.scalar_type() == at::kBFloat16 || x.scalar_type() == at::kFloat),
              "layernorm_fwd: need a 2-D bf16/fp32 GPU tensor with contiguous rows");
  need(gamma, at::kFloat, "gamma"); need(beta, at::kFloat, "beta");
  const int64_t m = x.size(0), d = x.size(1);
  Tensor y = at::empty({m, d}, x.options().dtype(at::kBFloat16));
  Tensor mean = at::empty({m}, x.options().dtype(at::kFloat)), rstd = at::empty({m}, x.options().dtype(at::kFloat));
  ok(sam_layernorm_fwd(x.data_ptr(), x.scalar_type() == at::kFloat, x.stride(0), (const float*)gamma.data_ptr(), (const float*)beta.data_ptr(), (float)eps, (int)m,
                       (int)d, y.data_ptr(), y.stride(0), (float*)mean.data_ptr(), (float*)rstd.data_ptr(), cur_stream()),
     "sam_layernorm_fwd");
  return {y, mean, rstd};
}

struct LnQueue {
  std::mutex mu;
  bool defer = false;
  int64_t D = 0;
  std::vector<sam_ln_finalize_item> items;
  std::vector<Tensor> keep;
};
LnQueue& ln_queue() { static LnQueue q; return q; }

std::tuple<Tensor, Tensor> ln_bwd(const Tensor& dy, const Tensor& x, const Tensor& mean, const Tensor& rstd, const Tensor& gamma, const Tensor& dgamma,
                                  const Tensor& dbeta, const Tensor* dbias, bool want_dropped, double p_drop, int64_t seed, int64_t offset, bool accumulate = true,
                                  bool may_defer = false) {
  need2d(dy, "dy");
  const int64_t m = x.size(0), d = x.size(1);
  Tensor dx = at::empty({m, d}, dy.options());
  Tensor dxd = (want_dropped && p_drop > 0) ? at::empty({m, d}, dy.options()) : Tensor();
  Tensor ws = at::empty({(sam_layernorm_bwd_ws_bytes((int)d) + 3) / 4}, dy.options().dtype(at::kFloat));
  LnQueue& q = ln_queue();
  bool defer = false;
  if (may_defer) {
    std::lock_guard<std::mutex> lock(q.mu);
    defer = q.defer && (q.items.empty() || q.D == d);
    if (defer) {
      q.D = d;
      q.items.push_back({(const float*)ws.data_ptr(), (int32_t)sam_layernorm_bwd_partial_rows((int)m), accumulate ? 1 : 0, (float*)dgamma.data_ptr(),
                         (float*)dbeta.data_ptr(), dbias ? (float*)dbias->data_ptr() : nullptr});
      q.keep.push_back(ws);
    }
  }
  ok(sam_layernorm_bwd(dy.data_ptr(), dy.stride(0), x.data_ptr(), x.scalar_type() == at::kFloat, x.stride(0), (const float*)mean.data_ptr(),
                       (const float*)rstd.data_ptr(), (const float*)gamma.data_ptr(), (int)m, (int)d, dx.data_ptr(), p(dxd), dx.stride(0), (float)p_drop,
                       (uint64_t)seed, (uint64_t)offset, (float*)dgamma.data_ptr(), (float*)dbeta.data_ptr(), dbias ? (float*)dbias->data_ptr() : nullptr,
                       (accumulate ? 1 : 0) | (defer ? 4 : 0), (float*)ws.data_ptr(), cur_stream()),
     "sam_layernorm_bwd");
  return {dx, dxd.defined() ? dxd : (want_dropped ? dx : Tensor())};
}

void set_ln_defer(bool on) {
  LnQueue& q = ln_queue();
  std::lock_guard<std::mutex> lock(q.mu);
  q.defer = on;
}

void ln_finalize_flush() {
  LnQueue& q = ln_queue();
  std::lock_guard<std::mutex> lock(q.mu);
  if (q.items.empty()) return;
  ok(sam_layernorm_bwd_finalize_batch(q.items.data(), (int)q.items.size(), (int)q.D, cur_stream()), "sam_layernorm_bwd_finalize_batch");
  q.items.clear();
  q.keep.clear();
}

void ln_finalize_clear() {
  LnQueue& q = ln_queue();
  std::lock_guard<std::mutex> lock(q.mu);
  q.items.clear();
  q.keep.clear();
  q.defer = false;
}

int64_t words_per_row(int64_t n) {
  const int nw = sam_attn_words_per_row((int)n);
  TORCH_CHECK(nw > 0, "sequence length ", n, " exceeds the fused-attention limit (384 keys)");
  return nw;
}
std::tuple<Tensor, Tensor, Tensor> pack_masks(const Tensor& q, const Tensor& o, const Tensor& c) {
  need(q, at::kLong, "question_mask"); need(o, at::kLong, "pad_obj_mask"); need(c, at::kLong, "pad_ocr_mask");
  TORCH_CHECK(q.dim() == 2 && o.dim() == 2 && c.dim() == 2 && q.is_contiguous() && o.is_contiguous() && c.is_contiguous(), "pack_masks: contiguous [B, n] masks");
  const int64_t b = q.size(0), t = q.size(1), no = o.size(1), nc = c.size(1);
  auto u8 = q.options().dtype(at::kByte);
  Tensor kv = at::empty({b, t + no + nc}, u8), q8 = at::empty({b, t}, u8), c8 = at::empty({b, nc}, u8);
  ok(sam_pack_masks_u8((const int64_t*)q.data_ptr(), (int)t, (const int64_t*)o.data_ptr(), (int)no, (const int64_t*)c.data_ptr(), (int)nc, (int)b,
                       (uint8_t*)kv.data_ptr(), (uint8_t*)q8.data_ptr(), (uint8_t*)c8.data_ptr(), cur_stream()), "sam_pack_masks_u8");
  return {kv, q8, c8};
}
Tensor mask_bits_prefix_lm(const Tensor& key_valid, int64_t n_dec) {
  need(key_valid, at::kByte, "key_valid");
  TORCH_CHECK(key_valid.dim() == 2 && key_valid.is_contiguous(), "key_valid: contiguous uint8 [B, n_enc]");
  const int64_t b = key_valid.size(0), n_enc = key_valid.size(1), n = n_enc + n_dec, nw = words_per_row(n);
  Tensor out = at::empty({b, 1, n, nw}, key_valid.options().dtype(at::kInt));
  ok(sam_mask_bits_prefix_lm((const uint8_t*)key_valid.data_ptr(), (int)b, (int)n_enc, (int)n_dec, (int)nw, (uint32_t*)out.data_ptr(), cur_stream()), "sam_mask_bits_prefix_lm");
  return out;
}
Tensor mask_bits_from_additive(const Tensor& mask) {
  need(mask, at::kFloat, "attention_mask");
  TORCH_CHECK(mask.dim() == 4 && mask.size(1) == 1 && mask.size(2) == mask.size(3) && mask.is_contiguous(), "attention_mask must be a contiguous [B,1,N,N] tensor");
  const int64_t b = mask.size(0), n = mask.size(2), nw = words_per_row(n);
  Tensor out = at::empty({b, 1, n, nw}, mask.options().dtype(at::kInt));
  ok(sam_mask_bits_from_additive((const float*)mask.data_ptr(), (int)b, (int)n, (int)nw, (uint32_t*)out.data_ptr(), cur_stream()), "sam_mask_bits_from_additive");
  return out;
}
Tensor pack_relations(const Tensor& base_bits, const Tensor& adj, int64_t n_txt, int64_t heads, int64_t quadrant_bits) {
  need(base_bits, at::kInt, "base_bits"); need(adj, at::kChar, "spatial_adj_matrix");
  TORCH_CHECK(base_bits.dim() == 4 && base_bits.is_contiguous() && adj.dim() == 4 && adj.is_contiguous(), "pack_relations: contiguous base [B,1,N,NW], adj [B,Noo,Noo,R]");
  const int64_t b = base_bits.size(0), n = base_bits.size(2), nw = base_bits.size(3);
  Tensor out = at::empty({b, heads, n, nw}, base_bits.options());
  ok(sam_mask_bits_spatial((const uint32_t*)base_bits.data_ptr(), (const int8_t*)adj.data_ptr(), (int)b, (int)n, (int)nw, (int)n_txt, (int)adj.size(1), (int)adj.size(3),
                           (int)heads, (unsigned)quadrant_bits, (uint32_t*)out.data_ptr(), cur_stream()), "sam_mask_bits_spatial");
  return out;
}
Tensor pack_relations_bhnn(const Tensor& rel, const optional<Tensor>& base_bits) {
  need(rel, at::kChar, "rel");
  TORCH_CHECK(rel.dim() == 4 && rel.size(2) == rel.size(3) && rel.is_contiguous(), "rel must be a contiguous int8 [B,H,N,N] tensor");
  const int64_t b = rel.size(0), h = rel.size(1), n = rel.size(2), nw = words_per_row(n);
  Tensor out = at::empty({b, h, n, nw}, rel.options().dtype(at::kInt));
  ok(sam_mask_bits_from_int8_bhnn((const int8_t*)rel.data_ptr(), (const uint32_t*)p(base_bits), (int)b, (int)h, (int)n, (int)nw, (uint32_t*)out.data_ptr(), cur_stream()),
     "sam_mask_bits_from_int8_bhnn");
  return out;
}

Tensor ptr_scores_fwd(const Tensor& q, const Tensor& k, const Tensor& ocr_mask, double scale) {
  need(q, at::kBFloat16, "q"); need(k, at::kBFloat16, "k"); need(ocr_mask, at::kByte, "ocr_mask");
  TORCH_CHECK(q.dim() == 3 && k.dim() == 3 && q.is_contiguous() && k.is_contiguous() && ocr_mask.is_contiguous(), "ptr_scores: contiguous q [B,S,D], k [B,No,D], mask [B,No]");
  const int64_t b = q.size(0), s = q.size(1), d = q.size(2), no = k.size(1);
  Tensor out = at::empty({b, s, no}, q.options().dtype(at::kFloat));
  ok(sam_ptr_scores_fwd(q.data_ptr(), k.data_ptr(), (const uint8_t*)ocr_mask.data_ptr(), (int)b, (int)s, (int)no, (int)d, (float)scale, (float*)out.data_ptr(), out.stride(0),
                        out.stride(1), cur_stream()), "sam_ptr_scores_fwd");
// ... 113 lines not shown
                   const Tensor& grp_off, const Tensor& grp_extra, int64_t bos, int64_t key, const optional<Tensor>& step_dev, int64_t step,
                   const optional<Tensor>& force_choice, Tensor targets, Tensor prev_inds, Tensor loss_mask, Tensor acc_mask, Tensor choice) {
  answer_sample_impl(meta, seq_len, seq_grp, step0_idx, step0_val, grp_idx, grp_off, grp_extra, bos, key, step_dev, step, force_choice, &targets, 0, prev_inds,
                     loss_mask, acc_mask, choice);
}
void answer_sample_notargets(const Tensor& meta, const Tensor& seq_len, const Tensor& seq_grp, const Tensor& step0_idx, const Tensor& step0_val,
                             const Tensor& grp_idx, const Tensor& grp_off, const Tensor& grp_extra, int64_t width, int64_t bos, int64_t key,
                             const optional<Tensor>& step_dev, int64_t step, const optional<Tensor>& force_choice, Tensor prev_inds, Tensor loss_mask,
                             Tensor acc_mask, Tensor choice) {
  answer_sample_impl(meta, seq_len, seq_grp, step0_idx, step0_val, grp_idx, grp_off, grp_extra, bos, key, step_dev, step, force_choice, nullptr, width, prev_inds,
                     loss_mask, acc_mask, choice);
}

std::tuple<Tensor, Tensor, Tensor> bce_loss_table(const Tensor& fixed, const Tensor& ocr, at::TensorList table, const Tensor& choice, const Tensor& loss_mask,
                                                  double grad_scale, const optional<Tensor>& global_count, bool want_grads, const optional<Tensor>& pred) {
  need(fixed, at::kFloat, "fixed_scores"); need(ocr, at::kFloat, "ocr_scores"); need(loss_mask, at::kFloat, "loss_mask"); need(choice, at::kInt, "choice");
  TORCH_CHECK(fixed.dim() == 2 && ocr.dim() == 2 && fixed.stride(1) == 1 && ocr.stride(1) == 1 && ocr.size(0) == fixed.size(0) && loss_mask.is_contiguous() &&
              choice.is_contiguous(), "bce_loss_table: 2-D score blocks with unit last stride, contiguous loss_mask and choice");
  TORCH_CHECK(table.size() == 8, "bce_loss_table: the answer table is eight tensors (meta, seq_len, seq_grp, step0_idx, step0_val, grp_idx, grp_off, grp_extra)");
  const Tensor &meta = table[0], &seq_len = table[1], &seq_grp = table[2], &step0_idx = table[3], &step0_val = table[4], &grp_idx = table[5], &grp_off = table[6],
               &grp_extra = table[7];
  need(meta, at::kInt, "meta"); need(seq_len, at::kInt, "seq_len"); need(seq_grp, at::kShort, "seq_grp"); need(step0_idx, at::kInt, "step0_idx");
  need(step0_val, at::kFloat, "step0_val"); need(grp_idx, at::kInt, "grp_idx"); need(grp_off, at::kInt, "grp_off"); need(grp_extra, at::kInt, "grp_extra");
  for (const Tensor& t : table) TORCH_CHECK(t.is_contiguous(), "bce_loss_table: table tensors must be contiguous");
  TORCH_CHECK(seq_grp.dim() == 3 && meta.dim() == 2 && meta.size(1) == 4, "bce_loss_table: meta [B, 4], seq_grp [B, S, L]");
  const int64_t B = seq_grp.size(0), S = seq_grp.size(1), L = seq_grp.size(2), G = grp_idx.size(-1), E = grp_extra.size(-1);
  TORCH_CHECK(meta.size(0) == B && seq_len.numel() == B * S && step0_idx.numel() == B * S && step0_val.numel() == B * S && grp_idx.numel() == B * G &&
              grp_off.numel() == B * (G + 1) && grp_extra.numel() == B * E, "bce_loss_table: table tensors of inconsistent sizes");
  const int64_t r = fixed.size(0), v = fixed.size(1), no = ocr.size(1);
  TORCH_CHECK(r == B * L && loss_mask.numel() == r && choice.numel() == B, "bce_loss_table: ", r, " score rows for a table of ", B, " x ", L, " decoding steps");
  int64_t* pr = nullptr;
  if (pred.has_value() && pred->defined()) {
    need(*pred, at::kLong, "pred");
    TORCH_CHECK(pred->is_contiguous() && pred->numel() == r, "bce_loss_table: pred int64 [R]");
    pr = (int64_t*)pred->data_ptr();
  }
  const int64_t rg = want_grads ? r : 0;
  Tensor loss = at::empty({1}, fixed.options()), d_fixed = at::empty({rg, v}, fixed.options().dtype(at::kBFloat16)), d_ocr = at::empty({rg, no}, fixed.options());
  ok(sam_bce_loss_table((const float*)fixed.data_ptr(), fixed.stride(0), (const float*)ocr.data_ptr(), ocr.stride(0), (const int32_t*)meta.data_ptr(),
                        (const int32_t*)seq_len.data_ptr(), (const int16_t*)seq_grp.data_ptr(), (const int32_t*)step0_idx.data_ptr(), (const float*)step0_val.data_ptr(),
                        (const int32_t*)grp_idx.data_ptr(), (const int32_t*)grp_off.data_ptr(), (const int32_t*)grp_extra.data_ptr(), (int)B, (int)S, (int)L, (int)G, (int)E,
                        (const int32_t*)choice.data_ptr(), (const float*)loss_mask.data_ptr(), (int)r, (int)v, (int)no, (float)grad_scale, (const float*)p(global_count),
                        (float*)loss.data_ptr(), want_grads ? d_fixed.data_ptr() : nullptr, want_grads ? d_fixed.stride(0) : 0,
                        want_grads ? (float*)d_ocr.data_ptr() : nullptr, want_grads ? d_ocr.stride(0) : 0, pr, cur_stream()), "sam_bce_loss_table");
  return {loss, d_fixed, d_ocr};
}

enum { P_WQKV, P_BQKV, P_WO, P_BO, P_LN1W, P_LN1B, P_W1, P_B1, P_W2, P_B2, P_LN2W, P_LN2B, P_COUNT };
enum { S_X, S_QKV, S_CTX, S_LSE, S_KEEP, S_Z1, S_MEAN1, S_RSTD1, S_A, S_PRE, S_H, S_Z2, S_MEAN2, S_RSTD2, S_CTXLO, S_COUNT };

std::vector<Tensor> encoder_layer_fwd(const Tensor& x, const Tensor& allow, at::TensorList params, int64_t batch, int64_t heads, double scale, double p_attn,
                                      double p_hid, at::IntArrayRef seeds, double eps1, double eps2) {
  TORCH_CHECK(params.size() == P_COUNT, "encoder_layer_fwd: expected ", (int)P_COUNT, " parameter tensors");
  TORCH_CHECK(seeds.size() == 6, "encoder_layer_fwd: seeds = (seed, offset) x 3 dropout sites");
  need2d(x, "x");
  GemmOpt o;
  o.epilogue = SAM_EPI_BIAS; o.bias = &params[P_BQKV];
  Tensor qkv = gemm(x, params[P_WQKV], true, true, o);
  Tensor ctx, lse2, keep, ctx_lo;
  if (fused_attn_bwd_enabled(x.size(0) / batch)) std::tie(ctx, lse2, keep, ctx_lo) = attn_fwd_train(qkv, allow, batch, heads, scale, p_attn, seeds[0], seeds[1]);
  else { std::tie(ctx, lse2, keep) = attn_fwd(qkv, allow, batch, heads, scale, p_attn, seeds[0], seeds[1]); ctx_lo = at::empty({0}, x.options()); }
  o = GemmOpt(); o.epilogue = SAM_EPI_BIAS_DROPOUT_RES; o.bias = &params[P_BO]; o.residual = &x; o.p_drop = (float)p_hid; o.seed = seeds[2]; o.offset = seeds[3];
  auto [z1, a, mean1, rstd1] = gemm_ln(ctx, params[P_WO], params[P_LN1W], params[P_LN1B], eps1, o);
  Tensor pre = at::empty({x.size(0), params[P_W1].size(0)}, x.options());
  o = GemmOpt(); o.epilogue = SAM_EPI_BIAS_GELU_GRAD; o.bias = &params[P_B1]; o.aux_out = &pre;
  Tensor h = gemm(a, params[P_W1], true, true, o);
  o = GemmOpt(); o.epilogue = SAM_EPI_BIAS_DROPOUT_RES; o.bias = &params[P_B2]; o.residual = &a; o.p_drop = (float)p_hid; o.seed = seeds[4]; o.offset = seeds[5];
  auto [z2, y, mean2, rstd2] = gemm_ln(h, params[P_W2], params[P_LN2W], params[P_LN2B], eps2, o);
  return {y, x, qkv, ctx, lse2, keep, z1, mean1, rstd1, a, pre, h, z2, mean2, rstd2, ctx_lo};
}

static std::vector<Tensor> encoder_layer_bwd_impl(const Tensor& dy_in, at::TensorList saved, const Tensor& allow, at::TensorList params, at::TensorList grads, int64_t batch,
                                                  int64_t heads, double scale, double p_attn, double p_hid, at::IntArrayRef seeds, bool need_dx, bool accumulate, bool defer_wgrad) {
  TORCH_CHECK(saved.size() == S_COUNT && params.size() == P_COUNT && grads.size() == P_COUNT, "encoder_layer_bwd: bad list sizes");
  Tensor dy = dy_in;
  if (dy.scalar_type() != at::kBFloat16 || !dy.is_contiguous()) dy = dy.to(at::kBFloat16).contiguous();
  const Tensor &x = saved[S_X], &qkv = saved[S_QKV], &ctx = saved[S_CTX], &lse2 = saved[S_LSE], &keep = saved[S_KEEP], &z1 = saved[S_Z1], &a = saved[S_A],
               &pre = saved[S_PRE], &h = saved[S_H], &z2 = saved[S_Z2];
  auto [dz2, dy2] = ln_bwd(dy, z2, saved[S_MEAN2], saved[S_RSTD2], params[P_LN2W], grads[P_LN2W], grads[P_LN2B], &grads[P_B2], true, p_hid, seeds[4], seeds[5], accumulate, true);
  GemmOpt o;
  o.epilogue = SAM_EPI_MUL_AUX; o.aux_in = &pre;
  Tensor dpre = gemm(dy2, params[P_W2], true, false, o);
  o = GemmOpt(); o.epilogue = SAM_EPI_BIAS_DROPOUT_RES; o.residual = &dz2;
  Tensor da = gemm(dpre, params[P_W1], true, false, o);
  auto [dz1, dy1] = ln_bwd(da, z1, saved[S_MEAN1], saved[S_RSTD1], params[P_LN1W], grads[P_LN1W], grads[P_LN1B], &grads[P_BO], true, p_hid, seeds[2], seeds[3], accumulate, true);
  Tensor dctx = gemm(dy1, params[P_WO], true, false, GemmOpt());
  Tensor dqkv = saved[S_CTXLO].numel() ? attn_bwd_fused(dctx, qkv, ctx, saved[S_CTXLO], lse2, allow, keep, batch, heads, scale, p_attn)
                                       : attn_bwd(dctx, qkv, lse2, allow, keep, batch, heads, scale, p_attn);
  const Tensor dw2 = grads[P_W2], dw1 = grads[P_W1], db1 = grads[P_B1], dwo = grads[P_WO], dwqkv = grads[P_WQKV], dbqkv = grads[P_BQKV];
  if (!defer_wgrad) wgrad_grouped({{&dy2, &h, &dw2, nullptr}, {&dpre, &a, &dw1, &db1}, {&dy1, &ctx, &dwo, nullptr}, {&dqkv, &x, &dwqkv, &dbqkv}}, accumulate);
  Tensor dx = at::empty({0}, x.options());
  if (need_dx) {
    o = GemmOpt(); o.epilogue = SAM_EPI_BIAS_DROPOUT_RES; o.residual = &dz1;
    dx = gemm(dqkv, params[P_WQKV], true, false, o);
  }
  if (defer_wgrad) return {dx, dy2, dpre, dy1, dqkv};
  return {dx};
}
Tensor encoder_layer_bwd(const Tensor& dy_in, at::TensorList saved, const Tensor& allow, at::TensorList params, at::TensorList grads, int64_t batch, int64_t heads,
                         double scale, double p_attn, double p_hid, at::IntArrayRef seeds, bool need_dx, bool accumulate) {
  return encoder_layer_bwd_impl(dy_in, saved, allow, params, grads, batch, heads, scale, p_attn, p_hid, seeds, need_dx, accumulate, false)[0];
}
std::vector<Tensor> encoder_layer_bwd_nowgrad(const Tensor& dy_in, at::TensorList saved, const Tensor& allow, at::TensorList params, at::TensorList grads, int64_t batch,
                                              int64_t heads, double scale, double p_attn, double p_hid, at::IntArrayRef seeds, bool need_dx, bool accumulate) {
  return encoder_layer_bwd_impl(dy_in, saved, allow, params, grads, batch, heads, scale, p_attn, p_hid, seeds, need_dx, accumulate, true);
}
void wgrad_grouped_op(at::TensorList dys, at::TensorList xs, at::TensorList dws, at::TensorList dbs, bool accumulate) {
  TORCH_CHECK(dys.size() == xs.size() && dys.size() == dws.size() && dys.size() == dbs.size(), "wgrad_grouped: list sizes differ");
  std::vector<WgradJob> jobs;
  for (size_t q = 0; q < dys.size(); ++q) jobs.push_back({&dys[q], &xs[q], &dws[q], dbs[q].numel() ? &dbs[q] : nullptr});
  wgrad_grouped(jobs, accumulate);
}

std::tuple<Tensor, Tensor> linear_op(const Tensor& x, const Tensor& w, const optional<Tensor>& bias, int64_t epilogue, const optional<Tensor>& residual,
                                     const optional<Tensor>& aux_in, bool want_aux_out, double p_drop, int64_t seed, int64_t offset, bool b_kcontig, bool out_f32) {
  GemmOpt o;
  o.epilogue = (int)epilogue; o.p_drop = (float)p_drop; o.seed = seed; o.offset = offset; o.out_f32 = out_f32;
  Tensor b_, r_, ai_, aux;
  if (bias.has_value() && bias->defined()) { b_ = need(*bias, at::kFloat, "bias"); o.bias = &b_; }
  if (residual.has_value() && residual->defined()) { r_ = *residual; need2d(r_, "residual"); o.residual = &r_; }
  if (aux_in.has_value() && aux_in->defined()) { ai_ = *aux_in; need2d(ai_, "aux_in"); o.aux_in = &ai_; }
  const int64_t N = b_kcontig ? w.size(0) : w.size(1);
  if (want_aux_out) { aux = at::empty({x.size(0), N}, x.options()); o.aux_out = &aux; }
  Tensor y = gemm(x, w, true, b_kcontig, o);
  return {y, want_aux_out ? aux : at::empty({0}, x.options())};
}

std::tuple<Tensor, Tensor, Tensor> layernorm_fwd_op(const Tensor& x, const Tensor& gamma, const Tensor& beta, double eps) { return ln_fwd(x, gamma, beta, eps); }

std::tuple<Tensor, Tensor, Tensor> layernorm_bwd_op(const Tensor& dy, const Tensor& x, const Tensor& mean, const Tensor& rstd, const Tensor& gamma) {
  Tensor dg = at::zeros_like(gamma), db = at::zeros_like(gamma);
  auto r = ln_bwd(dy, x, mean, rstd, gamma, dg, db, nullptr, false, 0.0, 0, 0);
  return {std::get<0>(r), dg, db};
}

}

TORCH_LIBRARY(sam_hip, m) {
  m.def("linear(Tensor x, Tensor w, Tensor? bias, int epilogue, Tensor? residual, Tensor? aux_in, bool want_aux_out, float p_drop, int seed, int offset, "
        "bool b_kcontig, bool out_f32) -> (Tensor, Tensor)");
  m.def("spatial_attn_fwd(Tensor qkv, Tensor allow, int batch, int heads, float scale, float p_drop, int seed, int offset) -> (Tensor, Tensor, Tensor)");
  m.def("spatial_attn_bwd(Tensor dout, Tensor qkv, Tensor lse2, Tensor allow, Tensor keep, int batch, int heads, float scale, float p_drop) -> Tensor");
  m.def("spatial_attn_fwd_train(Tensor qkv, Tensor allow, int batch, int heads, float scale, float p_drop, int seed, int offset) -> (Tensor, Tensor, Tensor, Tensor)");
  m.def("spatial_attn_bwd_fused(Tensor dout, Tensor qkv, Tensor out, Tensor out_lo, Tensor lse2, Tensor allow, Tensor keep, int batch, int heads, float scale, float p_drop) -> Tensor");
  m.def("layernorm_fwd(Tensor x, Tensor gamma, Tensor beta, float eps) -> (Tensor, Tensor, Tensor)");
  m.def("layernorm_bwd(Tensor dy, Tensor x, Tensor mean, Tensor rstd, Tensor gamma) -> (Tensor, Tensor, Tensor)");
  m.def("set_ln_defer(bool on) -> ()");
  m.def("ln_finalize_flush() -> ()");
  m.def("ln_finalize_clear() -> ()");
  m.def("pack_masks(Tensor question_mask, Tensor obj_mask, Tensor ocr_mask) -> (Tensor, Tensor, Tensor)");
  m.def("mask_bits_prefix_lm(Tensor key_valid, int n_dec) -> Tensor");
  m.def("mask_bits_from_additive(Tensor mask) -> Tensor");
  m.def("pack_relations(Tensor base_bits, Tensor adj, int n_txt, int heads, int quadrant_bits) -> Tensor");
  m.def("pack_relations_bhnn(Tensor rel, Tensor? base_bits) -> Tensor");
  m.def("ptr_scores(Tensor q, Tensor k, Tensor ocr_mask, float scale) -> Tensor");
  m.def("ptr_scores_bwd(Tensor dscores, Tensor q, Tensor k, float scale) -> (Tensor, Tensor)");
  m.def("bce_loss(Tensor fixed, Tensor ocr, Tensor targets, Tensor loss_mask, float grad_scale, Tensor? global_count) -> (Tensor, Tensor, Tensor)");
  m.def("sumsq(Tensor g, Tensor(a!) out, int[] sparse_region, Tensor? touched) -> ()");
  m.def("adam_step(Tensor(a!) p, Tensor(e!) g, Tensor(b!) m, Tensor(c!) v, Tensor(d!)? p_bf16, int[] seg_end, float[] seg_lr, int step, float beta1, float beta2, float eps, "
        "Tensor? gnorm_sq, float max_norm, Tensor? dev_sched, int[] sparse_region, Tensor? touched) -> ()");
  m.def("step_advance(Tensor(a!)? rng_state, int offset_stride, Tensor(b!) step_counter, float[] base_lr, int warmup_iters, float warmup_factor, int[] decay_iters, "
        "float lr_decay, float beta1, float beta2, Tensor(c!) dev_sched) -> ()");
  m.def("encoder_layer_fwd(Tensor x, Tensor allow, Tensor[] params, int batch, int heads, float scale, float p_attn, float p_hid, int[] seeds, float eps1, "
        "float eps2) -> Tensor[]");
  m.def("encoder_layer_bwd(Tensor dy, Tensor[] saved, Tensor allow, Tensor[] params, Tensor(a!)[] grads, int batch, int heads, float scale, float p_attn, "
        "float p_hid, int[] seeds, bool need_dx, bool accumulate) -> Tensor");
  m.def("encoder_layer_bwd_nowgrad(Tensor dy, Tensor[] saved, Tensor allow, Tensor[] params, Tensor(a!)[] grads, int batch, int heads, float scale, float p_attn, "
        "float p_hid, int[] seeds, bool need_dx, bool accumulate) -> Tensor[]");
// ... 45 lines not shown
```

### sam-textvqa_amd/ops.py

```python
import os

import torch

from . import _capi as capi
from . import torchops

BF16 = torch.bfloat16


class _TorchOpsProxy:
    _cache = {}

    def __getattr__(self, name):
        fn = self._cache.get(name)
        if fn is None:
            op = getattr(torchops.ns(), name)

            def fn(*a, _op=op, **kw):
                try:
                    return _op(*a, **kw)
                except capi.SamHipError:
                    raise
                except RuntimeError as e:
                    raise capi.SamHipError(str(e).split("\n")[0]) from None
# ... 139 lines not shown
def attn_fwd_dec(qkv_enc, qkv_dec, allow, batch, n, n_dec, n_heads, scale, out_dec=None, kv_group=1):
    _chk(qkv_enc, BF16, "qkv_enc"); _chk(qkv_dec, BF16, "qkv_dec"); _chk(allow, torch.int32, "allow")
    d_model = qkv_enc.shape[1] // 3
    if out_dec is None:
        out_dec = torch.empty((batch * n_dec, d_model), dtype=BF16, device=qkv_enc.device)
    sh = 0 if allow.shape[1] == 1 else allow.stride(1)
    if kv_group > 1:
        capi.call("sam_attn_fwd_dec_shared", capi.ptr(qkv_enc), capi.ptr(qkv_dec), capi.ptr(allow), allow.stride(0), sh, batch, int(kv_group), n, n_dec, n_heads,
                  d_model // n_heads, float(scale), capi.ptr(out_dec), capi.stream_handle())
        return out_dec
    capi.call("sam_attn_fwd_dec", capi.ptr(qkv_enc), capi.ptr(qkv_dec), capi.ptr(allow), allow.stride(0), sh, batch, n, n_dec, n_heads, d_model // n_heads,
              float(scale), capi.ptr(out_dec), capi.stream_handle())
    return out_dec


def greedy_pick(fixed, ocr, prev_inds):
    _chk(prev_inds, torch.int64, "prev_inds")
    r, s = prev_inds.shape
    capi.call("sam_greedy_pick", capi.ptr(fixed), fixed.stride(0), capi.ptr(ocr), ocr.stride(0), r, s, fixed.shape[1], ocr.shape[1], capi.ptr(prev_inds), capi.stream_handle())
    return prev_inds


def attn_dec_row(qkv_enc, qkv_dec, allow, batch, n, n_dec, t, n_heads, scale, kv_group=1):
    _chk(qkv_enc, BF16, "qkv_enc"); _chk(qkv_dec, BF16, "qkv_dec"); _chk(allow, torch.int32, "allow")
    d_model = qkv_enc.shape[1] // 3
    out = torch.empty((batch, d_model), dtype=BF16, device=qkv_enc.device)
    sh = 0 if allow.shape[1] == 1 else allow.stride(1)
    capi.call("sam_attn_dec_row", capi.ptr(qkv_enc), capi.ptr(qkv_dec), capi.ptr(allow), allow.stride(0), sh, batch, int(kv_group), n, n_dec, int(t), n_heads,
              d_model // n_heads, float(scale), capi.ptr(out), out.stride(0), capi.stream_handle())
    return out


def beam_step(fixed, ocr, n_samples, beam, seqs, cum, done, eos, t=0, ctl=None, prev_pos=None):
    _chk(seqs, torch.int64, "seqs"); _chk(cum, torch.float32, "cum"); _chk(done, torch.uint8, "done")
    s = seqs.shape[1]
    if beam > 1 and os.environ.get("SAM_BEAM_STEP_SPLIT", "1") != "0":
        ws = _workspace(int(capi.call("sam_beam_step_ws_bytes", int(n_samples), int(beam))), fixed.device, "beam_step")
        capi.call("sam_beam_step_split", capi.ptr(fixed), fixed.stride(0), capi.ptr(ocr), ocr.stride(0), int(n_samples), int(beam), s, fixed.shape[1], ocr.shape[1], int(eos),
                  int(t), capi.ptr(ctl), capi.ptr(cum), capi.ptr(done), capi.ptr(seqs), capi.ptr(prev_pos), capi.ptr(ws), capi.stream_handle())
        return
    capi.call("sam_beam_step", capi.ptr(fixed), fixed.stride(0), capi.ptr(ocr), ocr.stride(0), int(n_samples), int(beam), s, fixed.shape[1], ocr.shape[1], int(eos), int(t),
              capi.ptr(ctl), capi.ptr(cum), capi.ptr(done), capi.ptr(seqs), capi.ptr(prev_pos), capi.stream_handle())


_FUSED_MAX_N = None


def attn_bwd_fused_max_n():
    global _FUSED_MAX_N
    if _FUSED_MAX_N is None:
        _FUSED_MAX_N = int(capi.call("sam_attn_bwd_fused_max_n"))
    return _FUSED_MAX_N


def attn_bwd(dout, qkv, lse2, allow, keep, batch, n_heads, scale, p_drop=0.0, out=None, out_lo=None):
    _chk(dout, BF16, "dout"); _chk(qkv, BF16, "qkv")
    rows, three_d = qkv.shape
    n = rows // batch
    d_model = three_d // 3
    dqkv = torch.empty_like(qkv)
    sh = 0 if allow.shape[1] == 1 else allow.stride(1)
    bits_bytes = n_heads * n * (allow.shape[-1] * 4 * (2 if keep is not None else 1) + 8)
    if out is not None and out_lo is not None and n <= attn_bwd_fused_max_n() and os.environ.get("SAM_ATTN_BWD_FUSED", "1") != "0":
        _chk(out, BF16, "out"); _chk(out_lo, BF16, "out_lo")
        capi.call("sam_attn_bwd_fused", capi.ptr(dout), capi.ptr(qkv), capi.ptr(out), capi.ptr(out_lo), capi.ptr(lse2), capi.ptr(allow), allow.stride(0), sh,
                  capi.ptr(keep), batch, n, n_heads, d_model // n_heads, float(scale), float(p_drop), capi.ptr(dqkv), capi.stream_handle(),
                  meta=dict(kernel="attn_bwd(fused)", flops=10.0 * batch * n * n * d_model, shape=(batch, n, n_heads),
                            bytes=batch * (10 * n * d_model * 2 + bits_bytes)))
        return dqkv
    delta = torch.empty((batch, n_heads, n), dtype=torch.float32, device=qkv.device)
    capi.call("sam_attn_bwd", capi.ptr(dout), capi.ptr(qkv), capi.ptr(lse2), capi.ptr(allow), allow.stride(0), sh,
              capi.ptr(keep), batch, n, n_heads, d_model // n_heads, float(scale), float(p_drop), capi.ptr(dqkv), capi.ptr(delta),
              capi.stream_handle(),
              meta=dict(kernel="attn_bwd(dq+dkdv)", flops=10.0 * batch * n * n * d_model, shape=(batch, n, n_heads),
                        bytes=batch * (8 * n * d_model * 2 + bits_bytes)))
    return dqkv


def _dp(t):
    return None if t is None else t.data_ptr()


def gemm(a, b, *, a_kcontig=True, b_kcontig=True, m=None, n=None, k=None, out=None, out_dtype=BF16, epilogue=capi.EPI_NONE,
         bias=None, residual=None, aux_out=None, aux_in=None, accumulate=False, p_drop=0.0, seed=0, offset=0, split_k=0, bias_grad=None, force_tile=0, ln=None):
    for t, nm in ((a, "A"), (b, "B")):
        if not t.is_cuda or t.dtype != BF16 or t.dim() != 2 or t.stride(1) != 1:
            raise capi.SamHipError("gemm %s: need a 2-D bf16 GPU tensor with contiguous last dim" % nm)
    M = m if m is not None else (a.shape[0] if a_kcontig else a.shape[1])
    K = k if k is not None else (a.shape[1] if a_kcontig else a.shape[0])
    N = n if n is not None else (b.shape[0] if b_kcontig else b.shape[1])
    if out is None:
        out = torch.empty((M, N), dtype=out_dtype, device=a.device)
    d = capi.GemmDesc()
    d.M, d.N, d.K = M, N, K
    d.a_kcontig, d.b_kcontig = int(a_kcontig), int(b_kcontig)
    d.c_is_f32, d.accumulate, d.epilogue = int(out.dtype == torch.float32), int(accumulate), int(epilogue)
    d.A, d.lda, d.B, d.ldb, d.C, d.ldc = a.data_ptr(), a.stride(0), b.data_ptr(), b.stride(0), out.data_ptr(), out.stride(0)
    d.bias = _dp(bias)
    d.residual, d.ldr = _dp(residual), (residual.stride(0) if residual is not None else 0)
    d.aux_out, d.aux_in = _dp(aux_out), _dp(aux_in)
    aux = aux_out if aux_out is not None else aux_in
    d.ld_aux = aux.stride(0) if aux is not None else 0
    d.p_drop, d.seed, d.offset = float(p_drop), int(seed), int(offset)
    wgrad_split = bool(accumulate) and out.dtype == torch.float32 and epilogue == capi.EPI_NONE
    if split_k == 0 and not accumulate and bias_grad is None and force_tile == 0 and M <= 4096 and K >= 1536 and M * N <= (4 << 20):
        split_k = -1
    d.split_k, d.bias_grad, d.force_tile = int(split_k), _dp(bias_grad), int(force_tile)
    if ln is not None:
        import ctypes as C
        d.ln = C.pointer(ln)
    if split_k not in (0, 1):
        want = split_k if split_k > 0 else (32 if wgrad_split else 8)
        ws = _workspace(min(want * (M * N + M) * 4, 96 << 20), a.device, "splitk")
        d.ws, d.ws_bytes, d.defer_reduce = ws.data_ptr(), ws.numel() * 4, 1
    capi.call("sam_gemm_bf16", d, capi.stream_handle(),
              meta=dict(kernel="gemm<a_kc=%d,b_kc=%d,epi=%d,f32=%d>" % (d.a_kcontig, d.b_kcontig, d.epilogue, d.c_is_f32), flops=2.0 * M * N * K, shape=(M, N, K)))
    if d.split_k_used > 1 and wgrad_split:
        capi.call("sam_gemm_splitk_reduce", d.ws, d.split_k_used, M, N, out.data_ptr(), out.stride(0), d.bias_grad, capi.stream_handle(),
                  meta=dict(kernel="splitk_reduce", bytes=4.0 * M * N * (d.split_k_used + 2)))
    return out


def gemm_ln(a, b, gamma, beta, eps, **kw):
    m = a.shape[0] if kw.get("a_kcontig", True) else a.shape[1]
    n = b.shape[0] if kw.get("b_kcontig", True) else b.shape[1]
    if capi.profiler is not None or n % 4 or n > 2048 or gamma.dtype != torch.float32 or beta.dtype != torch.float32:
        z = gemm(a, b, **kw)
        return (z,) + tuple(layernorm_fwd(z, gamma, beta, eps))
    y = torch.empty((m, n), dtype=BF16, device=a.device)
    mean = torch.empty((m,), dtype=torch.float32, device=a.device)
    rstd = torch.empty((m,), dtype=torch.float32, device=a.device)
    ln = capi.LnFuse()
    ln.gamma, ln.beta, ln.eps, ln.y, ln.ldy, ln.mean, ln.rstd, ln.done = gamma.data_ptr(), beta.data_ptr(), float(eps), y.data_ptr(), y.stride(0), mean.data_ptr(), rstd.data_ptr(), 0
    if m >= 2048:
        xws = _ln_xws(a.device, int(capi.call("sam_gemm_ln_ws_bytes", m, n)))
        ln.xws, ln.xws_bytes = xws.data_ptr(), xws.numel() * 4
    z = gemm(a, b, ln=ln, **kw)
    if ln.done:
        return z, y, mean, rstd
    return (z,) + tuple(layernorm_fwd(z, gamma, beta, eps))


_WS = {}
_LN_XWS = {}


def _ln_xws(device, nbytes):
    key = (device, capi.stream_handle().value)
    buf = _LN_XWS.get(key)
    if buf is None or buf.numel() * 4 < nbytes:
        buf = torch.zeros((nbytes + 3) // 4, dtype=torch.float32, device=device)
        _LN_XWS[key] = buf
    return buf


def capi_ln_words():
    return 64 + 4 * 1024


def ln_xws_check():
    for buf in _LN_XWS.values():
        if int(buf[:1].view(torch.int32).item()) != 0:
            buf[:1].zero_()
            raise capi.SamHipError("LayerNorm inside the GEMM launch: a block waited in vain for the other parts of its rows (another kernel held the CUs its partners needed)")


def _workspace(nbytes, device, tag):
    key = (device, capi.stream_handle().value, tag)
    buf = _WS.get(key)
    if buf is None or buf.numel() * 4 < nbytes:
        buf = torch.empty((nbytes + 3) // 4, dtype=torch.float32, device=device)
        _WS[key] = buf
    return buf


def layernorm_fwd(x, gamma, beta, eps):
    if x.dim() != 2 or x.stride(1) != 1 or x.dtype not in (BF16, torch.float32) or not x.is_cuda:
        raise capi.SamHipError("layernorm_fwd: need a 2-D bf16/fp32 GPU tensor with contiguous rows")
    m, d = x.shape
    y = torch.empty((m, d), dtype=BF16, device=x.device)
    mean = torch.empty(m, dtype=torch.float32, device=x.device)
    rstd = torch.empty(m, dtype=torch.float32, device=x.device)
    capi.call("sam_layernorm_fwd", capi.ptr(x), int(x.dtype == torch.float32), x.stride(0), capi.ptr(gamma), capi.ptr(beta), float(eps), m, d,
              capi.ptr(y), y.stride(0), capi.ptr(mean), capi.ptr(rstd), capi.stream_handle())
    return y, mean, rstd


class LnFinalizeQueue:
    defer = False
    items = []

    @classmethod
    def flush(cls):
        if not cls.items:
            return
        by_d = {}
        for it in cls.items:
            by_d.setdefault(it[6], []).append(it)
        for d, its in by_d.items():
            arr = (capi.LnFinalizeItem * len(its))()
            for a, (ws, rows, acc, dg, db, dbias, _) in zip(arr, its):
                a.ws, a.rows, a.accumulate, a.dgamma, a.dbeta, a.dbias = ws.data_ptr(), rows, acc, dg.data_ptr(), db.data_ptr(), _dp(dbias)
            capi.call("sam_layernorm_bwd_finalize_batch", arr, len(its), d, capi.stream_handle())
        cls.items = []

    @classmethod
    def clear(cls):
        cls.items = []
        cls.defer = False


def layernorm_bwd(dy, x, mean, rstd, gamma, dgamma, dbeta, dbias=None, want_dropped=False, p_drop=0.0, seed=0, offset=0, accumulate=True, may_defer=False):
    _chk(dy, BF16, "dy")
    m, d = x.shape
    dx = torch.empty((m, d), dtype=BF16, device=x.device)
    dxd = torch.empty((m, d), dtype=BF16, device=x.device) if (want_dropped and p_drop > 0) else None
    defer = may_defer and LnFinalizeQueue.defer
    nbytes = capi.call("sam_layernorm_bwd_ws_bytes", d)
    ws = torch.empty(((nbytes + 3) // 4,), dtype=torch.float32, device=x.device) if defer else _workspace(nbytes, x.device, "ln")
    capi.call("sam_layernorm_bwd", capi.ptr(dy), dy.stride(0), capi.ptr(x), int(x.dtype == torch.float32), x.stride(0), capi.ptr(mean), capi.ptr(rstd),
              capi.ptr(gamma), m, d, capi.ptr(dx), capi.ptr(dxd), dx.stride(0), float(p_drop), int(seed), int(offset), capi.ptr(dgamma), capi.ptr(dbeta),
              capi.ptr(dbias), int(bool(accumulate)) | (4 if defer else 0), capi.ptr(ws), capi.stream_handle())
    if defer:
        LnFinalizeQueue.items.append((ws, int(capi.call("sam_layernorm_bwd_partial_rows", m)), int(bool(accumulate)), dgamma, dbeta, dbias, d))
    return dx, (dxd if dxd is not None else (dx if want_dropped else None))


def add_dropout(a, b, p_drop, seed=0, offset=0):
    for name, t in (("a", a), ("b", b)):
        if t is not None and (not t.is_cuda or t.dtype != BF16 or t.dim() != 2 or t.stride(1) != 1):
            raise capi.SamHipError("add_dropout: %s must be a bf16 [M, D] GPU tensor with unit column stride" % name)
    m, d = a.shape
    out = torch.empty((m, d), dtype=BF16, device=a.device)
    capi.call("sam_add_dropout_bf16", capi.ptr(a), a.stride(0), capi.ptr(b), 0 if b is None else b.stride(0), capi.ptr(out), out.stride(0), m, d,
              float(p_drop), int(seed), int(offset), capi.stream_handle())
    return out


def input_encoder_fwd(za, bbox, wb, bias_b, ln_a, ln_b, p_drop=0.0, seed=0, offset=0):
    _chk(za, BF16, "za")
    if not bbox.is_cuda or bbox.dtype != torch.float32 or bbox.dim() != 2 or bbox.stride(1) != 1 or bbox.shape[1] < 4:
        raise capi.SamHipError("input_encoder_fwd: bbox must be a 2-D fp32 GPU tensor with >= 4 contiguous columns")
    r, d = za.shape
    out = torch.empty((r, d), dtype=BF16, device=za.device)
    stats = torch.empty((r, 4), dtype=torch.float32, device=za.device)
    capi.call("sam_input_encoder_fwd", capi.ptr(za), za.stride(0), capi.ptr(bbox), bbox.stride(0), capi.ptr(wb), wb.stride(0), capi.ptr(bias_b), capi.ptr(ln_a.weight),
              capi.ptr(ln_a.bias), capi.ptr(ln_b.weight), capi.ptr(ln_b.bias), float(ln_a.variance_epsilon), r, d, float(p_drop), int(seed), int(offset), capi.ptr(out),
              out.stride(0), capi.ptr(stats), capi.stream_handle())
    return out, stats


def input_encoder_bwd(dy, za, bbox, wb, bias_b, ln_a, ln_b, stats, dwb, dbias_b, p_drop=0.0, seed=0, offset=0, accumulate=True):
    _chk(dy, BF16, "dy")
    r, d = za.shape
    dza = torch.empty((r, d), dtype=BF16, device=za.device)
    ws = _workspace(capi.call("sam_input_encoder_bwd_ws_bytes", r, d), za.device, "enc_in")
    capi.call("sam_input_encoder_bwd", capi.ptr(dy), dy.stride(0), capi.ptr(za), za.stride(0), capi.ptr(bbox), bbox.stride(0), capi.ptr(wb), wb.stride(0), capi.ptr(bias_b),
              capi.ptr(ln_a.weight), capi.ptr(ln_b.weight), capi.ptr(stats), r, d, float(p_drop), int(seed), int(offset), capi.ptr(dza), dza.stride(0),
              capi.ptr(ln_a.weight.grad), capi.ptr(ln_a.bias.grad), capi.ptr(ln_b.weight.grad), capi.ptr(ln_b.bias.grad), capi.ptr(dbias_b), capi.ptr(dwb), dwb.stride(0),
              int(bool(accumulate)), capi.ptr(ws), capi.stream_handle())
    return dza


def colsum(x, out, accumulate=True):
    m, n = x.shape
    ws = _workspace(capi.call("sam_colsum_ws_bytes", n), x.device, "colsum")
    capi.call("sam_colsum_bf16", capi.ptr(x), x.stride(0), m, n, capi.ptr(out), int(accumulate), capi.ptr(ws), capi.stream_handle())
    return out


def l2norm_pack(x, out, col0=0, normalize=True, zero_upto=0, eps=1e-12):
    _chk(out, BF16, "out")
    if not x.is_cuda or x.dtype != torch.float32 or x.dim() != 2:
        raise capi.SamHipError("l2norm_pack: x must be a 2-D fp32 GPU tensor")
    m, d = x.shape
    if x.stride(1) != 1 or out.stride(1) != 1 or out.shape[0] != m:
        raise capi.SamHipError("l2norm_pack: x / out must be row-major with the same number of rows")
    capi.call("sam_l2norm_pack_bf16", capi.ptr(x), x.stride(0), m, d, int(bool(normalize)), float(eps), capi.ptr(out), out.stride(0), int(col0), int(zero_upto),
              capi.stream_handle())
    return out


def embed_sum_fwd(pos, tt, rows, seq, table=None, ids=None, type_ids=None):
    d = pos.shape[1]
    out = torch.empty((rows, d), dtype=torch.float32, device=pos.device)
    capi.call("sam_embed_sum_fwd", capi.ptr(table), table.stride(0) if table is not None else 0, capi.ptr(ids), table.shape[0] if table is not None else 0,
              capi.ptr(pos), pos.stride(0), int(seq), capi.ptr(tt), tt.stride(0), capi.ptr(type_ids), tt.shape[0], rows, d, capi.ptr(out), out.stride(0),
              capi.stream_handle())
    return out


def embed_sum_bwd(d_e, seq, d_pos, d_tt, type_ids=None, n_types=1):
    _chk(d_e, BF16, "d_e")
    r, d = d_e.shape
    ws = _workspace(capi.call("sam_embed_sum_bwd_ws_bytes", int(seq), int(n_types), d), d_e.device, "embed")
    capi.call("sam_embed_sum_bwd", capi.ptr(d_e), d_e.stride(0), r, d, int(seq), capi.ptr(type_ids), int(n_types), capi.ptr(d_pos), d_pos.stride(0),
              capi.ptr(d_tt), d_tt.stride(0), capi.ptr(ws), capi.stream_handle())


def gather2_add_fwd(ans, ocr, inds, n_ocr, emb=None, p_drop=0.0, seed=0, offset=0):
    _chk(ans, BF16, "ans"); _chk(ocr, BF16, "ocr"); _chk(inds, torch.int64, "inds")
    b, s = inds.shape
    v, d = ans.shape
    out = torch.empty((b * s, d), dtype=BF16, device=ans.device)
    capi.call("sam_gather2_add_fwd", capi.ptr(ans), ans.stride(0), v, capi.ptr(ocr), ocr.stride(0), int(n_ocr), capi.ptr(inds), b, s, d, capi.ptr(emb),
              emb.stride(0) if emb is not None else 0, float(p_drop), int(seed), int(offset), capi.ptr(out), out.stride(0), capi.stream_handle())
    return out

# ... 521 lines not shown
```

Before: 10700 samples/s.

## Fuse split-K reduction of FFN input dgrad into LayerNorm backward

When the FFN intermediate dgrad GEMM uses split-K with the bias-dropout-residual epilogue, the LayerNorm backward kernel now reads the fp32 split-K partials directly, applying bias, dropout and the residual add in registers. This removes the separate split-K epilogue kernel and the bf16 round trip of the GEMM output before LayerNorm backward. The intermediate output is only stored when asked for. It adds template variants and a fallback path for unsupported shapes, and it only applies for D=768 with 2-8 splits.

Result: no change. 10740 samples/s (median of 6 runs) (+0.4%).

```diff
diff --git a/include/sam_hip.h b/include/sam_hip.h
--- a/include/sam_hip.h
+++ b/include/sam_hip.h
@@ -60,6 +60,18 @@
   float* xws; int64_t xws_bytes;
 } sam_ln_fuse;
 int64_t sam_gemm_ln_ws_bytes(int M, int N);
+typedef struct sam_ln_bwd_fuse {
+  const void* x; int64_t ldx;
+  const float* mean; const float* rstd;
+  const float* gamma;
+  void* dx; void* dx_dropped; int64_t ldo;
+  float p_drop; uint64_t seed, offset;
+  float* dgamma; float* dbeta; float* dbias;
+  int32_t accumulate;
+  float* ws;
+  int32_t store_c;
+  int32_t done;
+} sam_ln_bwd_fuse;
 typedef struct sam_gemm_desc {
   int32_t M, N, K;
   int32_t a_kcontig, b_kcontig;
@@ -78,6 +90,7 @@
   int32_t defer_reduce;
   int32_t split_k_used;
   sam_ln_fuse* ln;
+  sam_ln_bwd_fuse* ln_bwd;
 } sam_gemm_desc;
 int sam_gemm_bf16(const sam_gemm_desc* d, void* stream);
 int sam_gemm_bf16_grouped(const sam_gemm_desc* descs, int count, void* stream);
diff --git a/sam-textvqa_amd/_capi.py b/sam-textvqa_amd/_capi.py
--- a/sam-textvqa_amd/_capi.py
+++ b/sam-textvqa_amd/_capi.py
@@ -9,6 +9,12 @@
 class LnFuse(C.Structure):
     _fields_ = [("gamma", _vp), ("beta", _vp), ("eps", _f), ("y", _vp), ("ldy", _i64), ("mean", _vp), ("rstd", _vp), ("done", C.c_int32),
                 ("xws", _vp), ("xws_bytes", _i64)]
+
+
+class LnBwdFuse(C.Structure):
+    _fields_ = [("x", _vp), ("ldx", _i64), ("mean", _vp), ("rstd", _vp), ("gamma", _vp), ("dx", _vp), ("dx_dropped", _vp), ("ldo", _i64),
+                ("p_drop", _f), ("seed", _u64), ("offset", _u64), ("dgamma", _vp), ("dbeta", _vp), ("dbias", _vp), ("accumulate", C.c_int32),
+                ("ws", _vp), ("store_c", C.c_int32), ("done", C.c_int32)]
 
 
 class GemmDesc(C.Structure):
@@ -19,7 +25,8 @@
                 ("bias", _vp), ("residual", _vp), ("ldr", _i64),
                 ("aux_out", _vp), ("aux_in", _vp), ("ld_aux", _i64),
                 ("p_drop", _f), ("seed", _u64), ("offset", _u64), ("split_k", C.c_int32), ("bias_grad", _vp), ("ws", _vp), ("ws_bytes", _i64), ("force_tile", C.c_int32),
-                ("defer_reduce", C.c_int32), ("split_k_used", C.c_int32), ("ln", C.POINTER(LnFuse))]
+                ("defer_reduce", C.c_int32), ("split_k_used", C.c_int32), ("ln", C.POINTER(LnFuse)),
+                ("ln_bwd", C.POINTER(LnBwdFuse))]
 
 
 EPI_NONE, EPI_BIAS, EPI_BIAS_GELU, EPI_BIAS_DROPOUT_RES, EPI_DGELU, EPI_BIAS_GELU_GRAD, EPI_MUL_AUX, EPI_BIAS_RELU = range(8)
diff --git a/sam-textvqa_amd/autograd.py b/sam-textvqa_amd/autograd.py
--- a/sam-textvqa_amd/autograd.py
+++ b/sam-textvqa_amd/autograd.py
@@ -649,9 +649,9 @@
         wgrads = [(dy2, h, out.dense.weight.grad, None)]
         dpre = ops.gemm(dy2, _w(out.dense.weight), b_kcontig=False, epilogue=capi.EPI_MUL_AUX, aux_in=pre)
         wgrads.append((dpre, a, inter.dense.weight.grad, inter.dense.bias.grad))
-        da = ops.gemm(dpre, _w(inter.dense.weight), b_kcontig=False, epilogue=capi.EPI_BIAS_DROPOUT_RES, residual=dz2)
-        dz1, dy1 = ops.layernorm_bwd(da, z1, mean1, rstd1, so.LayerNorm.weight, so.LayerNorm.weight.grad, so.LayerNorm.bias.grad,
-                                     dbias=so.dense.bias.grad, want_dropped=True, p_drop=p_hid, seed=seeds[1][0], offset=seeds[1][1], accumulate=acc, may_defer=True)
+        dz1, dy1, _ = ops.gemm_layernorm_bwd(dpre, _w(inter.dense.weight), z1, mean1, rstd1, so.LayerNorm.weight, so.LayerNorm.weight.grad, so.LayerNorm.bias.grad,
+                                             dbias=so.dense.bias.grad, want_dropped=True, ln_p_drop=p_hid, ln_seed=seeds[1][0], ln_offset=seeds[1][1],
+                                             accumulate=acc, may_defer=True, b_kcontig=False, residual=dz2)
         wgrads.append((dy1, ctxv, so.dense.weight.grad, None))
         dctx = ops.gemm(dy1, _w(so.dense.weight), b_kcontig=False)
         dqkv = ops.attn_bwd(dctx, qkv, lse2, allow, keep, ctx.batch, att.num_attention_heads, ctx.scale, ctx.p_attn, out=ctxv, out_lo=ctx_lo)
diff --git a/sam-textvqa_amd/csrc/common.h b/sam-textvqa_amd/csrc/common.h
--- a/sam-textvqa_amd/csrc/common.h
+++ b/sam-textvqa_amd/csrc/common.h
@@ -15,6 +15,16 @@
 
 extern "C" void sam_set_error(const char* fmt, ...);
 extern "C" const unsigned long long* sam_get_rng_state(void);
+
+struct LnBwdSplitSrc {
+  const float* ws; int nsplit;
+  const float* bias; const bf16_t* residual; int64_t ldr;
+  int has_bias, has_res;
+  bf16_t* c_out; int64_t ldc;
+  unsigned thr16; float inv_keep; unsigned seed_lo, seed_hi, off_lo, off_hi;
+};
+struct sam_ln_bwd_fuse;
+int ln_bwd_from_splitk(const LnBwdSplitSrc& src, int M, int D, const sam_ln_bwd_fuse* l, hipStream_t st);
 
 #define SAM_REQUIRE(cond, ...)                    \
   do {                                            \
diff --git a/sam-textvqa_amd/csrc/gemm.hip b/sam-textvqa_amd/csrc/gemm.hip
--- a/sam-textvqa_amd/csrc/gemm.hip
+++ b/sam-textvqa_amd/csrc/gemm.hip
@@ -577,8 +577,22 @@
   return SAM_OK;
 }
 
+static int gemm_bf16_impl(const sam_gemm_desc* d, void* stream);
+
 extern "C" int sam_gemm_bf16(const sam_gemm_desc* d, void* stream) {
   SAM_REQUIRE(d, "sam_gemm_bf16: null descriptor");
+  sam_ln_bwd_fuse* l = d->ln_bwd;
+  if (l) {
+    l->done = 0;
+    SAM_REQUIRE(d->epilogue == SAM_EPI_BIAS_DROPOUT_RES && !d->c_is_f32 && !d->ln, "sam_gemm_bf16: sam_ln_bwd_fuse needs the BIAS_DROPOUT_RES epilogue, a bf16 C and no sam_ln_fuse");
+  }
+  const int rc = gemm_bf16_impl(d, stream);
+  if (rc || !l || l->done) return rc;
+  return sam_layernorm_bwd(d->C, d->ldc, l->x, 0, l->ldx, l->mean, l->rstd, l->gamma, d->M, d->N, l->dx, l->dx_dropped, l->ldo, l->p_drop, l->seed, l->offset,
+                           l->dgamma, l->dbeta, l->dbias, l->accumulate, l->ws, stream);
+}
+
+static int gemm_bf16_impl(const sam_gemm_desc* d, void* stream) {
   if (d->ln) d->ln->done = 0;
   SAM_REQUIRE(d->M > 0 && d->N > 0 && d->K > 0, "sam_gemm_bf16: empty problem %dx%dx%d", d->M, d->N, d->K);
   SAM_REQUIRE(d->A && d->B && d->C, "sam_gemm_bf16: null operand");
@@ -645,6 +659,21 @@
         *const_cast<int32_t*>(&d->split_k_used) = S;
         return SAM_OK;
       }
+      if (d->ln_bwd && e2 == SAM_EPI_BIAS_DROPOUT_RES && !d->c_is_f32) {
+        const char* ev = getenv("SAM_LN_BWD_FUSE");
+        if (!(ev && ev[0] == '0')) {
+          const LnBwdSplitSrc src = {d->ws, S, a.bias ? a.bias : d->ws, a.residual ? a.residual : (const bf16_t*)d->ws, a.residual ? a.ldr : 0,
+                                     a.bias != nullptr, a.residual != nullptr, d->ln_bwd->store_c ? (bf16_t*)d->C : nullptr, d->ldc,
+                                     a.thr16, a.inv_keep, a.seed_lo, a.seed_hi, a.off_lo, a.off_hi};
+          rc = ln_bwd_from_splitk(src, d->M, d->N, d->ln_bwd, st);
+          if (rc == SAM_OK) {
+            d->ln_bwd->done = 1;
+            *const_cast<int32_t*>(&d->split_k_used) = S;
+            return SAM_OK;
+          }
+          if (rc != SAM_ERR_UNSUPPORTED) return rc;
+        }
+      }
       const int64_t mn4 = (int64_t)d->M * d->N / 4;
       const dim3 grid((unsigned)min((int64_t)2048, (mn4 + 255) / 256));
 #define SAM_SPLIT_EPI(E, T) splitk_epilogue_kernel<E, T><<<grid, dim3(256), 0, st>>>(d->ws, S, a)
diff --git a/sam-textvqa_amd/csrc/rowops.hip b/sam-textvqa_amd/csrc/rowops.hip
--- a/sam-textvqa_amd/csrc/rowops.hip
+++ b/sam-textvqa_amd/csrc/rowops.hip
@@ -94,13 +94,71 @@
 __device__ __forceinline__ void pin(uint2& v) { pin(v.x); pin(v.y); }
 __device__ __forceinline__ void pin(float4& v) { pin(v.x); pin(v.y); pin(v.z); pin(v.w); }
 
-template <typename InT, int NCH, bool FULL, int MODE>
+struct LnBwdNoSplit {};
+template <int SPLIT> struct LnBwdSrc { typedef LnBwdSplitSrc T; };
+template <> struct LnBwdSrc<0> { typedef LnBwdNoSplit T; };
+
+template <int NCH, int SMAX, bool EXTRAS>
+__device__ __forceinline__ void ln_bwd_dy_from_partials(const LnBwdSplitSrc& sp, int row, int M, int D, int lane, unsigned seed_lo, unsigned seed_hi,
+                                                        unsigned off_lo, unsigned off_hi, uint2* dr) {
+  const int64_t MN = (int64_t)M * D;
+  const float* base = sp.ws + (int64_t)row * D + 4 * lane;
+  const bool has_res = sp.has_res != 0, has_bias = sp.has_bias != 0;
+  const bf16_t* rbase = sp.residual + (int64_t)row * sp.ldr + 4 * lane;
+  const float* bbase = sp.bias + 4 * lane;
+  float4 b[SMAX][NCH];
+  uint2 res[NCH];
+#pragma unroll
+  for (int s = 0; s < SMAX; ++s) {
+    const int sc = s < sp.nsplit ? s : 0;
+#pragma unroll
+    for (int j = 0; j < NCH; ++j) b[s][j] = *reinterpret_cast<const float4*>(base + (int64_t)sc * MN + 256 * j);
+  }
+#pragma unroll
+  for (int j = 0; j < NCH; ++j) res[j] = *reinterpret_cast<const uint2*>(rbase + 256 * j);
+#pragma unroll
+  for (int j = 0; j < NCH; ++j) {
+    const int n = 4 * (lane + 64 * j);
+    float v[4] = {b[0][j].x, b[0][j].y, b[0][j].z, b[0][j].w};
+#pragma unroll
+    for (int s = 1; s < SMAX; ++s) {
+      const bool on = s < sp.nsplit;
+      const float t0 = v[0] + b[s][j].x, t1 = v[1] + b[s][j].y, t2 = v[2] + b[s][j].z, t3 = v[3] + b[s][j].w;
+      v[0] = on ? t0 : v[0]; v[1] = on ? t1 : v[1]; v[2] = on ? t2 : v[2]; v[3] = on ? t3 : v[3];
+    }
+    if (EXTRAS) {
+      const float4 bb = *reinterpret_cast<const float4*>(bbase + 256 * j);
+      const float t0 = v[0] + bb.x, t1 = v[1] + bb.y, t2 = v[2] + bb.z, t3 = v[3] + bb.w;
+      v[0] = has_bias ? t0 : v[0]; v[1] = has_bias ? t1 : v[1]; v[2] = has_bias ? t2 : v[2]; v[3] = has_bias ? t3 : v[3];
+      const u32x4 rn = hidden_dropout_bits((unsigned)row, (unsigned)(n >> 3), off_lo, off_hi, seed_lo, seed_hi);
+      const unsigned lo = (n & 4) ? rn.z : rn.x, hi = (n & 4) ? rn.w : rn.y;
+      v[0] = (lo & 0xffffu) >= sp.thr16 ? v[0] * sp.inv_keep : 0.f;
+      v[1] = (lo >> 16) >= sp.thr16 ? v[1] * sp.inv_keep : 0.f;
+      v[2] = (hi & 0xffffu) >= sp.thr16 ? v[2] * sp.inv_keep : 0.f;
+      v[3] = (hi >> 16) >= sp.thr16 ? v[3] * sp.inv_keep : 0.f;
+    }
+    {
+      const float t0 = v[0] + bf_lo(res[j].x), t1 = v[1] + bf_hi(res[j].x), t2 = v[2] + bf_lo(res[j].y), t3 = v[3] + bf_hi(res[j].y);
+      v[0] = has_res ? t0 : v[0]; v[1] = has_res ? t1 : v[1]; v[2] = has_res ? t2 : v[2]; v[3] = has_res ? t3 : v[3];
+    }
+    dr[j] = make_uint2(pack_bf16x2(v[0], v[1]), pack_bf16x2(v[2], v[3]));
+  }
+}
+
+template <typename InT, int NCH, bool FULL, int MODE, int SPLIT = 0>
 __global__ __launch_bounds__(256) void ln_bwd_kernel(const bf16_t* __restrict__ dy, int64_t ldd, const void* __restrict__ x, int64_t ldx, const float* __restrict__ mean,
                                                      const float* __restrict__ rstd, const float* __restrict__ gamma, int M, int D, bf16_t* __restrict__ dx,
                                                      bf16_t* __restrict__ dxd, int64_t ldo, unsigned thr16, float inv_keep, unsigned seed_lo, unsigned seed_hi,
-                                                     unsigned off_lo, unsigned off_hi, const unsigned long long* rng_state, float* __restrict__ ws) {
+                                                     unsigned off_lo, unsigned off_hi, const unsigned long long* rng_state, float* __restrict__ ws,
+                                                     typename LnBwdSrc<SPLIT>::T sp) {
+  static_assert(SPLIT == 0 || FULL, "the split-K source covers full rows only");
   if (MODE == 2) rng_resolve(rng_state, seed_lo, seed_hi, off_lo, off_hi);
-  constexpr int NS = NCH <= 3 ? 3 : (NCH == 4 ? 2 : 1);
+  unsigned gseed_lo = 0, gseed_hi = 0, goff_lo = 0, goff_hi = 0;
+  if constexpr (SPLIT != 0) {
+    gseed_lo = sp.seed_lo; gseed_hi = sp.seed_hi; goff_lo = sp.off_lo; goff_hi = sp.off_hi;
+    rng_resolve(rng_state, gseed_lo, gseed_hi, goff_lo, goff_hi);
+  }
+  constexpr int NS = SPLIT != 0 ? 1 : (NCH <= 3 ? 3 : (NCH == 4 ? 2 : 1));
   typedef typename Raw4<InT>::R XR;
   __shared__ float red[4][64 * 4];
   const int lane = threadIdx.x & 63, wave = __builtin_amdgcn_readfirstlane(threadIdx.x >> 6);
@@ -130,8 +188,9 @@
     _Pragma("unroll") for (int j = 0; j < NCH; ++j) {                                              \
       const int c_ = FULL ? lane + 64 * j : min(lane + 64 * j, nchunk - 1);                        \
       xr[S][j] = Raw4<InT>::ld(x, (int64_t)row_ * ldx + 4 * c_);                                   \
-      dr[S][j] = Raw4<bf16_t>::ld(dy, (int64_t)row_ * ldd + 4 * c_);                               \
+      if constexpr (SPLIT == 0) dr[S][j] = Raw4<bf16_t>::ld(dy, (int64_t)row_ * ldd + 4 * c_);         \
     }                                                                                              \
+    if constexpr (SPLIT != 0) ln_bwd_dy_from_partials<NCH, (SPLIT & 15), (SPLIT & 16) != 0>(sp, row_, M, D, lane, gseed_lo, gseed_hi, goff_lo, goff_hi, dr[S]); \
   } while (0)
 #define LN_BWD_SLOT(S, ROW, REQ)                                                                                                     \
   {                                                                                                                                \
@@ -156,6 +215,8 @@
       }                                                                                                                            \
     }                                                                                                                              \
     const float rsv = rs[S];                                                                                                       \
+    uint2 dkeep[NCH];                                 \
+    if constexpr (SPLIT != 0) { _Pragma("unroll") for (int j = 0; j < NCH; ++j) dkeep[j] = dr[S][j]; }                             \
     pin(t1); pin(t2);                                                                                                              \
     if (REQ) {                                     \
       asm volatile("" ::: "memory");               \
@@ -185,6 +246,9 @@
       }                                                                                                                            \
       _Pragma("unroll") for (int e = 0; e < 4; ++e) ad[j][e] += o[e];                                                              \
     }                                                                                                                              \
+    if constexpr (SPLIT != 0) {                    \
+      if (sp.c_out) { _Pragma("unroll") for (int j = 0; j < NCH; ++j) *reinterpret_cast<uint2*>(sp.c_out + (int64_t)row * sp.ldc + 4 * (lane + 64 * j)) = dkeep[j]; } \
+    }                                                                                                                              \
     __builtin_amdgcn_sched_barrier(0);                                                                                             \
   }
 #define LN_BWD_TRIP(R0)                                                  \
@@ -644,7 +708,7 @@
 int ln_bwd_dispatch(int nch, dim3 grid, hipStream_t st, const bf16_t* dy, int64_t ldd, const void* x, int64_t ldx, const float* mean, const float* rstd,
                     const float* gamma, int M, int D, bf16_t* dx, bf16_t* dxd, int64_t ldo, unsigned thr16, float inv_keep, uint64_t seed, uint64_t offset, float* ws) {
 #define LN_BWD_LAUNCH(NC, FULL_, MODE_) ln_bwd_kernel<InT, NC, FULL_, MODE_><<<grid, dim3(256), 0, st>>>(dy, ldd, x, ldx, mean, rstd, gamma, M, D, dx, dxd, ldo, thr16, inv_keep, \
-      (unsigned)seed, (unsigned)(seed >> 32), (unsigned)offset, (unsigned)(offset >> 32), sam_get_rng_state(), ws)
+      (unsigned)seed, (unsigned)(seed >> 32), (unsigned)offset, (unsigned)(offset >> 32), sam_get_rng_state(), ws, LnBwdNoSplit())
 #define LN_BWD_CASE(NC) case NC: \
     if (D == 256 * NC) { if (mode == 2) LN_BWD_LAUNCH(NC, true, 2); else if (mode == 1) LN_BWD_LAUNCH(NC, true, 1); else LN_BWD_LAUNCH(NC, true, 0); } \
     else { if (mode == 2) LN_BWD_LAUNCH(NC, false, 2); else if (mode == 1) LN_BWD_LAUNCH(NC, false, 1); else LN_BWD_LAUNCH(NC, false, 0); } \
@@ -693,6 +757,38 @@
   if (accumulate & 4) return SAM_OK;
   FinalizeOuts fo = {{dgamma, dbeta, dbias}, {0, D, 2 * (int64_t)D}};
   partial_finalize_kernel<<<dim3((D + 63) / 64, dbias ? 3 : 2), dim3(64 * FIN_RL), 0, st>>>(ws, nblk, 3 * (int64_t)D, D, fo, accumulate & 1);
+  SAM_LAUNCH_CHECK();
+  return SAM_OK;
+}
+
+int ln_bwd_from_splitk(const LnBwdSplitSrc& src, int M, int D, const sam_ln_bwd_fuse* l, hipStream_t st) {
+  SAM_REQUIRE(l->x && l->mean && l->rstd && l->gamma && l->dx && l->dgamma && l->dbeta && l->ws, "sam_gemm_bf16: incomplete sam_ln_bwd_fuse");
+  SAM_REQUIRE(M > 0 && l->ldx % 4 == 0 && l->ldo % 4 == 0 && src.ldc % 4 == 0, "sam_gemm_bf16: sam_ln_bwd_fuse: bad leading dimension");
+  SAM_REQUIRE(l->p_drop >= 0.f && l->p_drop < 1.f, "sam_gemm_bf16: sam_ln_bwd_fuse: p_drop out of range");
+  SAM_REQUIRE(!l->dbias || l->dx_dropped || l->p_drop == 0.f, "sam_gemm_bf16: sam_ln_bwd_fuse: dbias with dropout needs dx_dropped");
+  const unsigned thr16 = dropout_thr16(l->p_drop);
+  const float inv_keep = thr16 ? 1.0f / (1.0f - (float)thr16 / 65536.0f) : 1.0f;
+  const int mode = l->dx_dropped ? (thr16 ? 2 : 1) : 0;
+  if (D != 768 || mode == 1 || M > 4 * LN_PARTIAL_BLOCKS || src.nsplit < 2 || src.nsplit > 8 || ((uintptr_t)src.ws % 16) != 0 || ((uintptr_t)src.residual % 8) != 0 || src.ldr % 4 != 0 ||
+      ((uintptr_t)src.bias % 16) != 0)
+    return SAM_ERR_UNSUPPORTED;
+  const int nblk = min(LN_PARTIAL_BLOCKS, (M + 3) / 4);
+#define LN_BWD_SPLIT_LAUNCH(MODE_, SPLIT_) ln_bwd_kernel<bf16_t, 3, true, MODE_, SPLIT_><<<dim3(nblk), dim3(256), 0, st>>>(nullptr, 0, l->x, l->ldx, l->mean, l->rstd, l->gamma, M, D, \
+      (bf16_t*)l->dx, (bf16_t*)l->dx_dropped, l->ldo, thr16, inv_keep, (unsigned)l->seed, (unsigned)(l->seed >> 32), (unsigned)l->offset, (unsigned)(l->offset >> 32),        \
+      sam_get_rng_state(), l->ws, src)
+  const bool extras = src.has_bias || src.thr16;
+#define LN_BWD_SPLIT_MODE(MODE_)                                                                                             \
+  do {                                                                                                                       \
+    if (src.nsplit <= 4) { if (extras) LN_BWD_SPLIT_LAUNCH(MODE_, 4 + 16); else LN_BWD_SPLIT_LAUNCH(MODE_, 4); }             \
+    else { if (extras) LN_BWD_SPLIT_LAUNCH(MODE_, 8 + 16); else LN_BWD_SPLIT_LAUNCH(MODE_, 8); }                             \
+  } while (0)
+  if (mode == 2) LN_BWD_SPLIT_MODE(2); else LN_BWD_SPLIT_MODE(0);
+#undef LN_BWD_SPLIT_MODE
+#undef LN_BWD_SPLIT_LAUNCH
+  SAM_LAUNCH_CHECK();
+  if (l->accumulate & 4) return SAM_OK;
+  FinalizeOuts fo = {{l->dgamma, l->dbeta, l->dbias}, {0, D, 2 * (int64_t)D}};
+  partial_finalize_kernel<<<dim3((D + 63) / 64, l->dbias ? 3 : 2), dim3(64 * FIN_RL), 0, st>>>(l->ws, nblk, 3 * (int64_t)D, D, fo, l->accumulate & 1);
   SAM_LAUNCH_CHECK();
   return SAM_OK;
 }
diff --git a/sam-textvqa_amd/csrc_torch/sam_torch_ops.cpp b/sam-textvqa_amd/csrc_torch/sam_torch_ops.cpp
--- a/sam-textvqa_amd/csrc_torch/sam_torch_ops.cpp
+++ b/sam-textvqa_amd/csrc_torch/sam_torch_ops.cpp
@@ -42,6 +42,7 @@
   int64_t seed = 0, offset = 0;
   bool out_f32 = false;
   sam_ln_fuse* ln = nullptr;
+  sam_ln_bwd_fuse* ln_bwd = nullptr;
 };
 
 Tensor gemm(const Tensor& a, const Tensor& b, bool a_kc, bool b_kc, const GemmOpt& o) {
@@ -57,7 +58,7 @@
   if (o.aux_out) { d.aux_out = o.aux_out->data_ptr(); d.ld_aux = o.aux_out->stride(0); }
   if (o.aux_in) { d.aux_in = o.aux_in->data_ptr(); d.ld_aux = o.aux_in->stride(0); }
   d.p_drop = o.p_drop; d.seed = (uint64_t)o.seed; d.offset = (uint64_t)o.offset;
-  d.ln = o.ln;
+  d.ln = o.ln; d.ln_bwd = o.ln_bwd;
   Tensor ws;
   if (M <= 4096 && K >= 1536 && M * N <= (4 << 20)) {
     d.split_k = -1;
@@ -227,6 +228,45 @@
                        (uint64_t)seed, (uint64_t)offset, (float*)dgamma.data_ptr(), (float*)dbeta.data_ptr(), dbias ? (float*)dbias->data_ptr() : nullptr,
                        (accumulate ? 1 : 0) | (defer ? 4 : 0), (float*)ws.data_ptr(), cur_stream()),
      "sam_layernorm_bwd");
+  return {dx, dxd.defined() ? dxd : (want_dropped ? dx : Tensor())};
+}
+
+static bool ln_bwd_fuse_enabled() {
+  const char* s = getenv("SAM_LN_BWD_FUSE");
+  return !(s && s[0] == '0');
+}
+
+std::tuple<Tensor, Tensor> gemm_ln_bwd(const Tensor& a, const Tensor& b, bool b_kc, GemmOpt o, const Tensor& x, const Tensor& mean, const Tensor& rstd, const Tensor& gamma,
+                                       const Tensor& dgamma, const Tensor& dbeta, const Tensor* dbias, bool want_dropped, double p_drop, int64_t seed, int64_t offset,
+                                       bool accumulate, bool may_defer) {
+  if (!ln_bwd_fuse_enabled() || x.scalar_type() != at::kBFloat16) {
+    Tensor dy = gemm(a, b, true, b_kc, o);
+    return ln_bwd(dy, x, mean, rstd, gamma, dgamma, dbeta, dbias, want_dropped, p_drop, seed, offset, accumulate, may_defer);
+  }
+  const int64_t m = x.size(0), d = x.size(1);
+  Tensor dx = at::empty({m, d}, x.options());
+  Tensor dxd = (want_dropped && p_drop > 0) ? at::empty({m, d}, x.options()) : Tensor();
+  Tensor ws = at::empty({(sam_layernorm_bwd_ws_bytes((int)d) + 3) / 4}, x.options().dtype(at::kFloat));
+  LnQueue& q = ln_queue();
+  bool defer = false;
+  if (may_defer) {
+    std::lock_guard<std::mutex> lock(q.mu);
+    defer = q.defer && (q.items.empty() || q.D == d);
+    if (defer) {
+      q.D = d;
+      q.items.push_back({(const float*)ws.data_ptr(), (int32_t)sam_layernorm_bwd_partial_rows((int)m), accumulate ? 1 : 0, (float*)dgamma.data_ptr(),
+                         (float*)dbeta.data_ptr(), dbias ? (float*)dbias->data_ptr() : nullptr});
+      q.keep.push_back(ws);
+    }
+  }
+  sam_ln_bwd_fuse l = {};
+  l.x = x.data_ptr(); l.ldx = x.stride(0); l.mean = (const float*)mean.data_ptr(); l.rstd = (const float*)rstd.data_ptr(); l.gamma = (const float*)gamma.data_ptr();
+  l.dx = dx.data_ptr(); l.dx_dropped = p(dxd); l.ldo = dx.stride(0);
+  l.p_drop = (float)p_drop; l.seed = (uint64_t)seed; l.offset = (uint64_t)offset;
+  l.dgamma = (float*)dgamma.data_ptr(); l.dbeta = (float*)dbeta.data_ptr(); l.dbias = dbias ? (float*)dbias->data_ptr() : nullptr;
+  l.accumulate = (accumulate ? 1 : 0) | (defer ? 4 : 0); l.ws = (float*)ws.data_ptr();
+  o.ln_bwd = &l;
+  gemm(a, b, true, b_kc, o);
   return {dx, dxd.defined() ? dxd : (want_dropped ? dx : Tensor())};
 }
 
@@ -506,8 +546,8 @@
   o.epilogue = SAM_EPI_MUL_AUX; o.aux_in = &pre;
   Tensor dpre = gemm(dy2, params[P_W2], true, false, o);
   o = GemmOpt(); o.epilogue = SAM_EPI_BIAS_DROPOUT_RES; o.residual = &dz2;
-  Tensor da = gemm(dpre, params[P_W1], true, false, o);
-  auto [dz1, dy1] = ln_bwd(da, z1, saved[S_MEAN1], saved[S_RSTD1], params[P_LN1W], grads[P_LN1W], grads[P_LN1B], &grads[P_BO], true, p_hid, seeds[2], seeds[3], accumulate, true);
+  auto [dz1, dy1] = gemm_ln_bwd(dpre, params[P_W1], false, o, z1, saved[S_MEAN1], saved[S_RSTD1], params[P_LN1W], grads[P_LN1W], grads[P_LN1B], &grads[P_BO], true, p_hid,
+                                seeds[2], seeds[3], accumulate, true);
   Tensor dctx = gemm(dy1, params[P_WO], true, false, GemmOpt());
   Tensor dqkv = saved[S_CTXLO].numel() ? attn_bwd_fused(dctx, qkv, ctx, saved[S_CTXLO], lse2, allow, keep, batch, heads, scale, p_attn)
                                        : attn_bwd(dctx, qkv, lse2, allow, keep, batch, heads, scale, p_attn);
diff --git a/sam-textvqa_amd/ops.py b/sam-textvqa_amd/ops.py
--- a/sam-textvqa_amd/ops.py
+++ b/sam-textvqa_amd/ops.py
@@ -245,7 +245,7 @@
 
 
 def gemm(a, b, *, a_kcontig=True, b_kcontig=True, m=None, n=None, k=None, out=None, out_dtype=BF16, epilogue=capi.EPI_NONE,
-         bias=None, residual=None, aux_out=None, aux_in=None, accumulate=False, p_drop=0.0, seed=0, offset=0, split_k=0, bias_grad=None, force_tile=0, ln=None):
+         bias=None, residual=None, aux_out=None, aux_in=None, accumulate=False, p_drop=0.0, seed=0, offset=0, split_k=0, bias_grad=None, force_tile=0, ln=None, ln_bwd=None):
     for t, nm in ((a, "A"), (b, "B")):
         if not t.is_cuda or t.dtype != BF16 or t.dim() != 2 or t.stride(1) != 1:
             raise capi.SamHipError("gemm %s: need a 2-D bf16 GPU tensor with contiguous last dim" % nm)
@@ -272,6 +272,9 @@
     if ln is not None:
         import ctypes as C
         d.ln = C.pointer(ln)
+    if ln_bwd is not None:
+        import ctypes as C
+        d.ln_bwd = C.pointer(ln_bwd)
     if split_k not in (0, 1):
         want = split_k if split_k > 0 else (32 if wgrad_split else 8)
         ws = _workspace(min(want * (M * N + M) * 4, 96 << 20), a.device, "splitk")
@@ -387,6 +390,39 @@
     if defer:
         LnFinalizeQueue.items.append((ws, int(capi.call("sam_layernorm_bwd_partial_rows", m)), int(bool(accumulate)), dgamma, dbeta, dbias, d))
     return dx, (dxd if dxd is not None else (dx if want_dropped else None))
+
+
+def ln_bwd_fuse_enabled():
+    return os.environ.get("SAM_LN_BWD_FUSE", "1") != "0"
+
+
+def gemm_layernorm_bwd(a, b, x, mean, rstd, gamma, dgamma, dbeta, dbias=None, want_dropped=False, ln_p_drop=0.0, ln_seed=0, ln_offset=0, accumulate=True,
+                       may_defer=False, store_dy=False, **kw):
+    if not ln_bwd_fuse_enabled() or capi.profiler is not None or x.dtype != BF16 or gamma.dtype != torch.float32:
+        dy = gemm(a, b, epilogue=capi.EPI_BIAS_DROPOUT_RES, **kw)
+        dx, dxd = layernorm_bwd(dy, x, mean, rstd, gamma, dgamma, dbeta, dbias=dbias, want_dropped=want_dropped, p_drop=ln_p_drop, seed=ln_seed, offset=ln_offset,
+                                accumulate=accumulate, may_defer=may_defer)
+        return dx, dxd, dy
+    m, d = x.shape
+    dx = torch.empty((m, d), dtype=BF16, device=x.device)
+    dxd = torch.empty((m, d), dtype=BF16, device=x.device) if (want_dropped and ln_p_drop > 0) else None
+    defer = may_defer and LnFinalizeQueue.defer
+    nbytes = capi.call("sam_layernorm_bwd_ws_bytes", d)
+    ws = torch.empty(((nbytes + 3) // 4,), dtype=torch.float32, device=x.device) if defer else _workspace(nbytes, x.device, "ln")
+    l = capi.LnBwdFuse()
+    l.x, l.ldx, l.mean, l.rstd, l.gamma = x.data_ptr(), x.stride(0), mean.data_ptr(), rstd.data_ptr(), gamma.data_ptr()
+    l.dx, l.dx_dropped, l.ldo = dx.data_ptr(), _dp(dxd), dx.stride(0)
+    l.p_drop, l.seed, l.offset = float(ln_p_drop), int(ln_seed), int(ln_offset)
+    l.dgamma, l.dbeta, l.dbias = dgamma.data_ptr(), dbeta.data_ptr(), _dp(dbias)
+    l.accumulate, l.ws, l.store_c, l.done = int(bool(accumulate)) | (4 if defer else 0), ws.data_ptr(), int(bool(store_dy)), 0
+    dy = gemm(a, b, epilogue=capi.EPI_BIAS_DROPOUT_RES, ln_bwd=l, **kw)
+    if defer:
+        LnFinalizeQueue.items.append((ws, int(capi.call("sam_layernorm_bwd_partial_rows", m)), int(bool(accumulate)), dgamma, dbeta, dbias, d))
+    gemm_layernorm_bwd.last_fused = bool(l.done)
+    return dx, (dxd if dxd is not None else (dx if want_dropped else None)), dy
+
+
+gemm_layernorm_bwd.last_fused = False
 
 
 def add_dropout(a, b, p_drop, seed=0, offset=0):
```
